# KirillKryukov/naf

Hardware: AMD Instinct MI355X
Metric: unnaf GB/s (uncompressed bases out) on 100 GB synthetic FASTA (higher is better)
Workload: dtype u8; 1 GPU; unnaf decode of a 100.0 GB synthetic-ACGT FASTA archive on one GPU (the size BASELINE.json's metric is quoted on; configs[1] at 10 GB rides along as cfg10_*), 100 records, 80-col lines; archive made in-run by the GPU ennaf; .naf 24739662224 B -> FASTA 99999995684 B, text + archive + decoded text resident in HBM; parallelism=one archive, one GPU, no data-path collective

## Files before the change

### naf_amd/csrc/ctx.h

```cpp
#pragma once
#include "common.h"
#include "../../include/naf_gpu.h"
#include <hip/hip_runtime.h>
#include <stdio.h>
#include <stdarg.h>
#include <string.h>
#include <vector>
#include <functional>
#include <string>

struct ArenaChunk { u8 *base; size_t cap, used; };

struct KTime { const char *name; hipEvent_t a, b; };

#define ZSPLIT_MAX 8
struct ZSplit { int parts; hipEvent_t ev[ZSPLIT_MAX]; u64 out_end[ZSPLIT_MAX]; int done; void *status; };
struct FlatStream { u64 q0, A; };
#define FLAT_DECODED (~0ull)
struct ZFlat { const u8 *src; const FlatStream *si; u64 nslots; const u8 *sym; void *status; bool ready;
               const u8 *tail; u64 tail_q; u32 tail_n;
               const u8 *cls; u32 n_decoded; u32 n_walk;
               struct naf_gpu_ctx *aux; hipEvent_t decoded_ev; void *later; };
struct CtxOpts { std::vector<std::pair<std::string, std::string>> kv; std::string trace; bool tracing = false; };
struct naf_gpu_ctx {
    int device = 0;
    CtxOpts *opts = nullptr;
    naf_gpu_ctx *root = nullptr;
    hipStream_t stream = nullptr;
    bool own_stream = false;
    std::vector<ArenaChunk> chunks;
    size_t high_water = 0;
    u8 *h_stage = nullptr;
    size_t h_stage_cap = 0;
    void *d_predef = nullptr;
    void *d_seqctab = nullptr;
    char err[512] = {0};
    bool timing = false;
    std::vector<KTime> ktimes;
    std::vector<hipEvent_t> ev_pool;
    size_t ev_used = 0;
    std::vector<std::string> agg_names; std::vector<float> agg_ms; std::vector<int> agg_n;
    float stream_ms[5] = { 0, 0, 0, 0, 0 };
    naf_gpu_ctx *side = nullptr;
    naf_gpu_ctx *side2 = nullptr;
    naf_gpu_ctx *side3 = nullptr;
    naf_gpu_ctx *side4 = nullptr;
    void *sides_thread = nullptr; int sides_rc = 0;
    hipEvent_t fork_ev = nullptr;
    struct ZSplit *zsplit = nullptr;
    hipEvent_t split_ev[ZSPLIT_MAX + 2] = {};
    struct ZFlat *zflat = nullptr;
    void *io_pool = nullptr;
    void *shard_state = nullptr;
    struct HostWorker *worker = nullptr;
};

void ctx_worker_start(naf_gpu_ctx *x, std::function<void()> job);
void ctx_worker_join(naf_gpu_ctx *x);
int  ctx_sides_ready(naf_gpu_ctx *c);

int  ctx_fail(naf_gpu_ctx *c, int code, const char *fmt, ...);
const char *ctx_opt(const naf_gpu_ctx *c, const char *name);
static inline bool ctx_opt_is(const naf_gpu_ctx *c, const char *name, char v) { const char *e = ctx_opt(c, name); return e && e[0] == v; }
bool ctx_tracing(const naf_gpu_ctx *c);
void ctx_trace(naf_gpu_ctx *c, const char *fmt, ...);
#define HIP_TRY(c, call) do { hipError_t e_ = (call); if (e_ != hipSuccess) return ctx_fail((c), NAF_GPU_EHIP, "%s: %s (%s:%d)", #call, hipGetErrorString(e_), __FILE__, __LINE__); } while (0)
static inline void ctx_take_error(naf_gpu_ctx *c, const char (&text)[512]) { memcpy(c->err, text, sizeof c->err); }
static inline void ctx_take_error(naf_gpu_ctx *c, const naf_gpu_ctx *from) { ctx_take_error(c, from->err); }
static inline hipError_t ctx_side_join(naf_gpu_ctx *x) { ctx_worker_join(x); return hipStreamSynchronize(x->stream); }
#define SIDE_SYNC_TRY(c, e, x) do { if ((e) != hipSuccess) return ctx_fail((c), NAF_GPU_EHIP, "%s: %s (%s:%d)", "hipStreamSynchronize(" #x "->stream)", hipGetErrorString(e), __FILE__, __LINE__); } while (0)
struct CtxJoinGuard { naf_gpu_ctx *x; ~CtxJoinGuard() { if (x) ctx_worker_join(x); } };

void  arena_reset(naf_gpu_ctx *c);
void *arena_alloc(naf_gpu_ctx *c, size_t bytes);
void  arena_settle(naf_gpu_ctx *c);
template <typename T> T *arena_new(naf_gpu_ctx *c, size_t n) { return (T *)arena_alloc(c, n * sizeof(T)); }
static inline std::vector<size_t> arena_mark(const naf_gpu_ctx *c) { std::vector<size_t> m; for (auto &ch : c->chunks) m.push_back(ch.used); return m; }
static inline void arena_release(naf_gpu_ctx *c, const std::vector<size_t> &m) { for (size_t k = 0; k < c->chunks.size(); k++) c->chunks[k].used = k < m.size() ? m[k] : 0; }

int ctx_readback(naf_gpu_ctx *c, void *h_dst, const void *d_src, size_t bytes);
int ctx_readback2(naf_gpu_ctx *c, void *h1, const void *d1, size_t n1, void *h2, const void *d2, size_t n2);
int ctx_readbackv(naf_gpu_ctx *c, int n, void *const *h, const void *const *d, const size_t *bytes);

void ktime_begin(naf_gpu_ctx *c, const char *name);
void ktime_end(naf_gpu_ctx *c);

#define LAUNCH(c, name, kern, grid, block, shmem, ...) do { \
    ktime_begin((c), name); \
    hipLaunchKernelGGL(kern, dim3(grid), dim3(block), (shmem), (c)->stream, __VA_ARGS__); \
    ktime_end((c)); } while (0)

static inline u32 cdiv(u64 a, u64 b) { return (u32)((a + b - 1) / b); }

int scan_exclusive_u64(naf_gpu_ctx *c, u64 *d_vals, size_t n, u64 *d_total);
int scan_inclusive_max_i32(naf_gpu_ctx *c, i32 *d_vals, size_t n);
int scan_inclusive_max_i64(naf_gpu_ctx *c, i64 *d_vals, size_t n);
int scan_exclusive_u64_multi(naf_gpu_ctx *c, u64 *const *arrs, int k, size_t n, u64 *const *totals);
int scan_inclusive_max_i64_multi(naf_gpu_ctx *c, i64 *const *arrs, int k, size_t n);

int zstd_decode(naf_gpu_ctx *c, const u8 *d_src, size_t src_len, int has_magic, u8 *d_dst, size_t dst_cap, size_t *out_len, const u8 *head = nullptr);
int zstd_init_tables(naf_gpu_ctx *c);
void ennaf_shard_state_free(naf_gpu_ctx *c);
void io_pool_free(naf_gpu_ctx *c);
struct EmitP;
int zstd_decode_fused_fasta(naf_gpu_ctx *c, const u8 *d_src, size_t src_len, int has_magic, size_t *out_len, const EmitP *P, u8 *text);
struct ZRange { u64 want_lo, want_hi, got_lo, got_hi; bool ranged; u8 *own_buf; };
int zstd_decode_range(naf_gpu_ctx *c, const u8 *d_src, size_t src_len, int has_magic, u8 *d_dst, size_t dst_cap, size_t *out_len, ZRange *rg, const u8 *head = nullptr);
int zstd_split_status(naf_gpu_ctx *c, const ZSplit *sp);
int zstd_flat_later(naf_gpu_ctx *c, ZFlat *zf);
void zstd_flat_drop(ZFlat *zf);
int zstd_small_batch(naf_gpu_ctx *c, int n, const u8 *const *src, const size_t *len, u8 *const *dst, const size_t *cap, bool *ok);
bool zstd_small_fits(size_t len, size_t cap);
int zstd_small_launch(naf_gpu_ctx *c, int n, const u8 *const *src, const size_t *len, u8 *const *dst, const size_t *cap, u32 **d_res_out);
enum { ZENC_PART = 16, ZENC_PART_FIRST = 32, ZENC_PART_LAST = 64, ZENC_PREFER_RAW = 128, ZENC_PREFER_FLAT = 256, ZENC_SHORT_CODES = 512, ZENC_FRAME_TREE = 1024, ZENC_LONG_LAST = 2048 };
int zenc_level_window(int level);
int zenc_repeat_probe(naf_gpu_ctx *c, const u8 *d_src, size_t n, u32 *share_1024);
static inline u32 zenc_probe_every(u64 n) { u32 e = 64; while (((n >> 20) / e) > 128) e <<= 1; return e; }
struct ZencPlace { u8 *(*fn)(void *ud, size_t frame_len); void *ud; };
struct ZencJob;
#define ZENC_LOC_BND 20
struct ZencLoc { const u8 *loc; const i32 *blk_bnd; const u32 *blk_t0; u64 tiles; };
int zstd_encode_begin(naf_gpu_ctx *c, const u8 *d_src, size_t n, int level, int with_magic, int lz, int block_log_hint, int window_log, ZencJob **job, const u8 *direct = nullptr, u32 nd = 0, const ZencLoc *dloc = nullptr);
int zstd_encode_finish(naf_gpu_ctx *c, ZencJob *job, u8 *d_dst, size_t cap, size_t *out_len, const ZencPlace *place);
void zstd_encode_drop(ZencJob *job);
int zstd_encode_size(naf_gpu_ctx *c, ZencJob *job, size_t *frame_len);
const u64 *zstd_encode_total_ptr(const ZencJob *job);
void zstd_encode_set_total(ZencJob *job, u64 total);
int zstd_encode(naf_gpu_ctx *c, const u8 *d_src, size_t n, int level, u8 *d_dst, size_t cap, size_t *out_len, int with_magic, int lz = 0, int block_log_hint = 0, int window_log = 0, const ZencPlace *place = nullptr);
```

### naf_amd/csrc/enc.hip

```cpp
#include "ctx.h"
#include <time.h>
#include "wgscan.h"
#include "enc_swar.h"

#define ET_BYTES 16
#define ET_TILE (256 * ET_BYTES)

struct OpMaxI64 { template <typename T> __device__ static T id() { return (T)(-1); } template <typename T> __device__ static T f(T a, T b) { return (i64)a > (i64)b ? a : b; } };
struct OpMaxU32 { template <typename T> __device__ static T id() { return (T)0; } template <typename T> __device__ static T f(T a, T b) { return a > b ? a : b; } };
struct OpMaxU64 { template <typename T> __device__ static T id() { return (T)0; } template <typename T> __device__ static T f(T a, T b) { return a > b ? a : b; } };

#define REG_ACGT 0x80000000u
#define REG_E(reg) (((reg) >> 24) & 0x7Fu)
struct EncP {
    const u8 *text; u64 n, p0;
    u32 expected[8];
    u8 replacement;
    u8 id_gt_unexpected;
    u8 strict, pad;
    u32 qlo, qhi;
    u32 plo, phi;
    u32 slo, shi;
    u32 nuc32[8];
    u32 *any_case;
// ... 704 lines not shown
    n = wg_reduce1<u64, OpAdd>(n, lds);
    if (threadIdx.x == 0 && n) atomicAdd(out, (unsigned long long)n);
}

struct EncOut {
    u8 *seq, *ids, *cmt;
    u8 *packed; u32 *casebits;
    u64 *rec_begin, *rec_end;
    u64 *unexpected;
    u64 *longest;
    u64 *lead;
    u64 *strict_first;
    const u64 *t_seq, *t_ids, *t_cmt, *t_rec; const u32 *t_tail; const i64 *tile_eol;
    const u32 *irr_list;
    const u32 *t_reg;
    const u8 *direct; u32 nd;
    u32 loc_mode;
    const u32 *sparse_list; const u32 *n_sparse;
};


__device__ __forceinline__ void flush_tile(u8 *dst, const u8 *stage, u32 n)
{
    u32 head = (u32)((8 - ((uintptr_t)dst & 7)) & 7); if (head > n) head = n;
    if (threadIdx.x < head) dst[threadIdx.x] = stage[threadIdx.x];
    u32 words = (n - head) >> 3;
    const u64 *s64 = (const u64 *)stage;
    for (u32 w = threadIdx.x; w < words; w += blockDim.x) {
        u32 off = head + 8 * w, sh = (off & 7) * 8;
        u64 a = s64[off >> 3], b = s64[(off >> 3) + 1];
        *(u64 *)(dst + off) = sh ? (a >> sh) | (b << (64 - sh)) : a;
    }
    u32 done = head + 8 * words;
    if (threadIdx.x < n - done) dst[done + threadIdx.x] = stage[done + threadIdx.x];
}

__device__ __forceinline__ u32 nuc4x4(u32 x, const u32 *t)
{
    const u32 sel = x & 0x07070707u;
    const u32 r0 = swar_perm(t[1], t[0], sel), r1 = swar_perm(t[3], t[2], sel), r2 = swar_perm(t[5], t[4], sel), r3 = swar_perm(t[7], t[6], sel);
    const u32 m3 = ((x >> 3) & 0x01010101u) * 0xFFu, m4 = ((x >> 4) & 0x01010101u) * 0xFFu, m6 = ((x >> 6) & 0x01010101u) * 0xFFu;
    const u32 lo = (r0 & ~m3) | (r1 & m3), hi = (r2 & ~m3) | (r3 & m3);
    const u32 tab = (lo & ~m4) | (hi & m4);
    return (tab & m6) | (m4 & 0x0F0F0F0Fu & ~m6);
}
__device__ __forceinline__ u32 nuc4x4_quick(u32 x) { return swar_perm(0x0F0F0F0Fu, 0x02010408u, (x >> 1) & 0x07070707u); }
__device__ __forceinline__ u32 pack_codes8(u32 c0, u32 c1)
{
    const u32 t0 = c0 | (c0 >> 4), t1 = c1 | (c1 >> 4);
    return swar_perm(t1, t0, 0x06040200u);
}
__device__ __forceinline__ bool all_quick16(const u32 w[4], u32 qlo, u32 qhi)
{
    const u32 L = 0x7F7F7F7Fu; u32 bad = 0;
#pragma unroll
    for (int i = 0; i < 4; i++) { u32 x = w[i], r = swar_perm(qhi, qlo, (x >> 1) & 0x07070707u), d = r ^ (x & 0xDFDFDFDFu); bad |= ((d & L) + L) | d; }
    return (bad & 0x80808080u) == 0;
}
template <bool KNOWN_QUICK>
__device__ __forceinline__ void flush_pack(const EncP &P, u8 *packed, u32 *casebits, u64 tbase, u32 n, const u8 *stage )
{
    if (!n) return;
    const u32 o = (u32)(tbase & 15), span = o + n, ng = (span + 15) >> 4;
    const u64 G0 = tbase >> 4;
    for (u32 j = threadIdx.x; j < ng; j += blockDim.x) {
        const uint4 v = *(const uint4 *)(stage + 16 * j);
        const u32 w[4] = { v.x, v.y, v.z, v.w };
        u32 cd[4];
        if (KNOWN_QUICK || all_quick16(w, P.qlo, P.qhi)) {
#pragma unroll
            for (int i = 0; i < 4; i++) cd[i] = nuc4x4_quick(w[i]);
        } else {
#pragma unroll
            for (int i = 0; i < 4; i++) cd[i] = nuc4x4(w[i], P.nuc32);
        }
        u64 pk = (u64)pack_codes8(cd[0], cd[1]) | ((u64)pack_codes8(cd[2], cd[3]) << 32);
        const u32 H = 0x80808080u;
        u32 cb = swar_movemask16((v.x | ((v.x << 1) & (v.x << 2))) & H, (v.y | ((v.y << 1) & (v.y << 2))) & H,
                                 (v.z | ((v.z << 1) & (v.z << 2))) & H, (v.w | ((v.w << 1) & (v.w << 2))) & H);
        const u32 a = j == 0 ? o : 0u, b = span - 16 * j < 16 ? span - 16 * j : 16u;
        if (a == 0 && b == 16) {
            *(u64 *)(packed + 8 * (G0 + j)) = pk;
            if (casebits) ((u16 *)casebits)[G0 + j] = (u16)cb;
        } else {
            const u64 nm = (b == 16 ? ~0ull : ((1ull << (4 * b)) - 1)) & ~((1ull << (4 * a)) - 1);
            cb &= ((1u << b) - 1) & ~((1u << a) - 1);
            atomicOr((unsigned long long *)(packed + 8 * (G0 + j)), (unsigned long long)(pk & nm));
            if (casebits) atomicOr(casebits + ((G0 + j) >> 1), cb << (16 * (u32)((G0 + j) & 1)));
        }
    }
}
#define DIRECT_PROBE_BLOCKS_LOG 5
__global__ __launch_bounds__(256) void k_direct_blocks(const u8 *text, const u64 *t_seq, const u32 *t_reg, u64 tiles, u32 nd, u32 prefer_flat, int probed, u8 *direct, const u32 *blk_t0 = nullptr, i32 *blk_bnd = nullptr)
{
    __shared__ u32 bins[4][64];
    const u32 wv = threadIdx.x >> 6, lane = threadIdx.x & 63;
    const u32 b = blockIdx.x * 4 + wv;
    bins[wv][lane] = 0;
    __syncthreads();
    bool ok = b < nd;
    if (ok && probed && (((b >> DIRECT_PROBE_BLOCKS_LOG) & (u32)(probed - 1)) == 0)) ok = false;
    u64 t0 = 0, t1 = 0;
    if (ok) {
        const u64 B0 = (u64)b << 16, B1 = B0 + 65536;
        u64 lo = 0, hi = tiles;
        if (blk_t0) { lo = blk_t0[b]; hi = lo + 1; }
        while (hi - lo > 1) {
            const u64 step = (hi - lo + 63) / 64;
            const u64 p = lo + (u64)lane * step;
            const bool le = p < hi && t_seq[p] <= B0;
            const u32 cnt = (u32)__popcll(__ballot(le));
            const u64 nlo = lo + (u64)(cnt - 1) * step, nhi = nlo + step < hi ? nlo + step : hi;
            lo = nlo; hi = nhi;
        }
        t0 = lo;
        const u64 t = t0 + lane;
        const u64 ts = t <= tiles ? t_seq[t] : ~0ull;
        const bool in = t < tiles && ts < B1;
        if (blk_bnd && lane < ZENC_LOC_BND) { const i64 rel = (i64)ts - (i64)B0; blk_bnd[(u64)b * ZENC_LOC_BND + lane] = t <= tiles && rel < (1 << 30) ? (i32)rel : (i32)(1 << 30); }
        const u64 bal = __ballot(in);
        const bool good = !in || ((t_reg[t] & REG_ACGT) != 0);
        ok = __ballot(!good) == 0 && bal != ~0ull;
        t1 = t0 + (u64)__popcll(bal) - 1;
    }
    if (ok) {
        const u64 x0 = t0 * ET_TILE, span = (t1 + 1 - t0) * ET_TILE;
        const u8 *at = text + x0 + (((u64)lane * span) >> 6 & ~63ull);
        uint4 v[4]; __builtin_memcpy(v, at, 64);
        const u32 w[16] = { v[0].x, v[0].y, v[0].z, v[0].w, v[1].x, v[1].y, v[1].z, v[1].w, v[2].x, v[2].y, v[2].z, v[2].w, v[3].x, v[3].y, v[3].z, v[3].w };
        u32 *mybins = &bins[wv][(lane & 3) * 16];
#pragma unroll
        for (int i = 0; i < 16; i++) {
#pragma unroll
            for (int h = 0; h < 2; h++) {
                const u32 pr = (w[i] >> (16 * h)) & 0xFFFFu, c0 = pr & 0xFF, c1 = pr >> 8;
                if ((c0 & 0x40) && (c1 & 0x40)) atomicAdd(&mybins[((c0 >> 1) & 3) | (((c1 >> 1) & 3) << 2)], 1u);
            }
        }
    }
    __syncthreads();
    if (ok) {
        const u32 c = lane < 16 ? bins[wv][lane] + bins[wv][16 + lane] + bins[wv][32 + lane] + bins[wv][48 + lane] : 0u;
        u32 ns = c;
#pragma unroll
        for (u32 d = 1; d < 16; d <<= 1) ns += __shfl_xor((int)ns, d, 64);
        float h = c ? (float)c * __log2f((float)ns / (float)c) : 0.0f;
#pragma unroll
        for (u32 d = 1; d < 16; d <<= 1) h += __shfl_xor(h, d, 64);
        ns = (u32)__shfl((int)ns, 0, 64); h = __shfl(h, 0, 64);
        ok = ns >= 1024 && h * (float)prefer_flat > 4.0f * (float)ns * (float)(prefer_flat - 1);
    }
    if (b < nd && lane == 0) direct[b] = ok ? 1 : 0;
}
__global__ __launch_bounds__(256) void k_direct_verdict(const u64 *t_seq, const u32 *t_reg, const u8 *t_hist, u64 tiles, u32 nd, u32 prefer_flat, int probed, const u32 *blk_t0, u8 *direct, i32 *blk_bnd)
{
    const u32 b = blockIdx.x * 256 + threadIdx.x;
    if (b >= nd) return;
    const u64 B0 = (u64)b << 16, B1 = B0 + 65536, t0 = blk_t0[b];
    bool ok = !(probed && (((b >> DIRECT_PROBE_BLOCKS_LOG) & (u32)(probed - 1)) == 0));
    u64 ts[ZENC_LOC_BND];
#pragma unroll
    for (u32 i = 0; i < ZENC_LOC_BND; i++) ts[i] = t0 + i <= tiles ? t_seq[t0 + i] : ~0ull;
#pragma unroll
    for (u32 i = 0; i < ZENC_LOC_BND; i++) { const i64 rel = (i64)ts[i] - (i64)B0; blk_bnd[(u64)b * ZENC_LOC_BND + i] = ts[i] != ~0ull && rel < (1 << 30) ? (i32)rel : (i32)(1 << 30); }
    u32 acc[8] = { 0, 0, 0, 0, 0, 0, 0, 0 };
    bool end = false;
#pragma unroll
    for (u32 i = 0; i < ZENC_LOC_BND - 1; i++) {
        if (!end && ok) {
            if (t0 + i >= tiles || ts[i] >= B1) end = true;
            else if (!(t_reg[t0 + i] & REG_ACGT)) ok = false;
            else {
                const uint4 h = *(const uint4 *)(t_hist + (t0 + i) * 16);
                acc[0] += h.x & 0x00FF00FFu; acc[1] += (h.x >> 8) & 0x00FF00FFu; acc[2] += h.y & 0x00FF00FFu; acc[3] += (h.y >> 8) & 0x00FF00FFu;
                acc[4] += h.z & 0x00FF00FFu; acc[5] += (h.z >> 8) & 0x00FF00FFu; acc[6] += h.w & 0x00FF00FFu; acc[7] += (h.w >> 8) & 0x00FF00FFu;
            }
        }
    }
    ok = ok && end;
    if (ok) {
        u32 ns = 0;
#pragma unroll
        for (int k = 0; k < 8; k++) ns += (acc[k] & 0xFFFFu) + (acc[k] >> 16);
        float h = 0.0f;
#pragma unroll
        for (int k = 0; k < 8; k++) {
            const u32 c0 = acc[k] & 0xFFFFu, c1 = acc[k] >> 16;
            if (c0) h += (float)c0 * __log2f((float)ns / (float)c0);
            if (c1) h += (float)c1 * __log2f((float)ns / (float)c1);
        }
        ok = ns >= 1024 && h * (float)prefer_flat > 4.0f * (float)ns * (float)(prefer_flat - 1);
    }
    direct[b] = ok ? 1 : 0;
}
__global__ __launch_bounds__(256) void k_case_gather(const u8 *direct, u32 nd, const u32 *blk_t0, const i32 *blk_bnd, const u8 *locc, const u8 *t_lower, u64 *casebits)
{
    __shared__ i32 s_bnd[ZENC_LOC_BND]; __shared__ u8 s_low[ZENC_LOC_BND];
    const u32 b = blockIdx.x;
    if (b >= nd || !direct[b]) return;
    const u64 t0 = blk_t0[b];
    if (threadIdx.x < ZENC_LOC_BND) { s_bnd[threadIdx.x] = blk_bnd[(u64)b * ZENC_LOC_BND + threadIdx.x]; s_low[threadIdx.x] = t_lower[t0 + threadIdx.x]; }
    __syncthreads();
    u32 a[4], c[4], e[4], sh[4], av[4], kk[4]; u64 nx[4];
#pragma unroll
    for (u32 r = 0; r < 4; r++) {
        const u32 W = r * 256u + threadIdx.x;
        const i32 r0 = (i32)(64u * W);
        u32 k = (u32)(r0 - s_bnd[0]) >> 12;
        if (s_bnd[k + 1] <= r0) k++;
        if (s_bnd[k + 1] <= r0) k++;
        const u32 i = (u32)(r0 - s_bnd[k]);
        av[r] = (u32)(s_bnd[k + 1] - r0); kk[r] = k; sh[r] = i & 31u;
        const u32 *p = (const u32 *)(locc + (t0 + k) * (LOC_TILE / 2)) + (i >> 5);
        a[r] = p[0]; c[r] = p[1]; e[r] = p[2];
        nx[r] = av[r] < 64u ? ld64(locc + (t0 + k + 1) * (LOC_TILE / 2)) : 0ull;
    }
#pragma unroll
    for (u32 r = 0; r < 4; r++) {
        u64 w = s_low[kk[r]] ? (u64)__builtin_amdgcn_alignbit(c[r], a[r], sh[r]) | ((u64)__builtin_amdgcn_alignbit(e[r], c[r], sh[r]) << 32) : 0ull;
        if (av[r] < 64u) {
            w &= (1ull << av[r]) - 1;
            if (s_low[kk[r] + 1]) w |= nx[r] << av[r];
        }
        casebits[((u64)b << 10) + r * 256u + threadIdx.x] = w;
    }
}
__global__ void k_irregular_list(const u32 *t_reg, const u64 *pre, u64 tiles, u32 *list, const u64 *t_seq = nullptr, u32 *blk_t0 = nullptr)
{
    const u64 t = (u64)blockIdx.x * blockDim.x + threadIdx.x;
    if (t >= tiles) return;
    if (!t_reg[t]) list[pre[t]] = (u32)t;
    if (blk_t0) {
        const u64 lo = t_seq[t], hi = t_seq[t + 1];
        for (u64 b = (lo + 65535) >> 16; (b << 16) < hi; b++) blk_t0[b] = (u32)t;
    }
}
__global__ void k_pack_edges_zero(const u64 *t_seq, u64 tiles, u64 T, u8 *packed, u32 *casebits, const u8 *direct, u32 nd, u32 loc_mode = 0)
{
    const u64 t = (u64)blockIdx.x * blockDim.x + threadIdx.x;
    if (t >= tiles) return;
    const u64 b0 = t_seq[t], b1 = t + 1 < tiles ? t_seq[t + 1] : T;
    if (b1 <= b0) return;
    const u64 g0 = b0 >> 4, g1 = (b1 - 1) >> 4;
    const bool d0 = direct && (g0 >> 12) < nd && direct[g0 >> 12], d1 = direct && (g1 >> 12) < nd && direct[g1 >> 12];
    if (loc_mode) {
        if (!d0) { *(u64 *)(packed + 8 * g0) = 0; if (casebits) ((u16 *)casebits)[g0] = 0; }
        if (!d1) { *(u64 *)(packed + 8 * g1) = 0; if (casebits) ((u16 *)casebits)[g1] = 0; }
        return;
    }
    if (d0) *((u32 *)(packed + ((g0 >> 12) << 15) + (((g0 >> 10) & 3) << 12)) + (1023u - (u32)(g0 & 1023u))) = 0; else *(u64 *)(packed + 8 * g0) = 0;
    if (d1) *((u32 *)(packed + ((g1 >> 12) << 15) + (((g1 >> 10) & 3) << 12)) + (1023u - (u32)(g1 & 1023u))) = 0; else *(u64 *)(packed + 8 * g1) = 0;
    if (casebits) { ((u16 *)casebits)[g0] = 0; ((u16 *)casebits)[g1] = 0; }
}

__device__ __forceinline__ u64 low_bytes(u32 n) { return n >= 8 ? ~0ull : ((1ull << (8 * n)) - 1); }
__device__ __forceinline__ void lds_store_n(u8 *p, u64 lo, u64 hi, u32 n)
{
    if (n >= 16) { __builtin_memcpy(p, &lo, 8); __builtin_memcpy(p + 8, &hi, 8); return; }
    if (n & 8) { __builtin_memcpy(p, &lo, 8); p += 8; lo = hi; }
    if (n & 4) { u32 v = (u32)lo; __builtin_memcpy(p, &v, 4); p += 4; lo >>= 32; }
    if (n & 2) { u16 v = (u16)lo; __builtin_memcpy(p, &v, 2); p += 2; lo >>= 16; }
    if (n & 1) *p = (u8)lo;
}

__device__ __forceinline__ u32 piece_run_compact(const Piece &pc, u32 a, u32 b, u32 sp, u64 &lo, u64 &hi)
{
    piece_from(pc, a, lo, hi);
    u32 d = (sp >> a) & ((1u << (b - a)) - 1);
    const u32 n = (b - a) - (u32)__popc(d);
    while (d) {
        u32 k = 31 - __clz((int)d); d &= ~(1u << k);
        u64 slo = (lo >> 8) | (hi << 56), shi = hi >> 8;
        if (k < 8) { u64 m = low_bytes(k); lo = (lo & m) | (slo & ~m); hi = shi; }
        else { u64 m = low_bytes(k - 8); hi = (hi & m) | (shi & ~m); }
    }
    return n;
}
__device__ __forceinline__ void global_store_n(u8 *p, u64 lo, u64 hi, u32 n)
{
    if (n >= 16) { st64(p, lo); st64(p + 8, hi); return; }
    if (n & 8) { st64(p, lo); p += 8; lo = hi; }
    if (n & 4) { st32(p, (u32)lo); p += 4; lo >>= 32; }
    if (n & 2) { p[0] = (u8)lo; p[1] = (u8)(lo >> 8); p += 2; lo >>= 16; }
    if (n & 1) p[0] = (u8)lo;
}

struct WriteSink {
    const EncOut &O; u64 bseq, bids, bcmt, rec; u64 line_b; u64 best; bool line_valid; u8 *stage; u64 tbase;
    __device__ WriteSink(const EncOut &o) : O(o) {}
    __device__ void emit(int s, u32 ch) { if (s == EV_SEQ) stage[bseq++ - tbase] = (u8)ch; else if (s == EV_IDS) O.ids[bids++] = (u8)ch; else O.cmt[bcmt++] = (u8)ch; }
    __device__ void header_start(u64) { if (rec > 0) O.rec_end[rec - 1] = bseq; else *O.lead = bseq; rec++; }
    __device__ void header_end(u64) { O.rec_begin[rec - 1] = bseq; line_b = bseq; }
    __device__ void line_end(u64) { u64 len = bseq - line_b; if (len > best) best = len; line_b = bseq; }
    __device__ void unexpected(int kind, u32 ch, u64 pos) { atomicAdd((unsigned long long *)&O.unexpected[kind * 257 + ch], 1ull); if (O.strict_first) atomicMin((unsigned long long *)O.strict_first, strict_key(pos, kind, ch)); }
    __device__ void ids_range(const Piece &pc, u32 a, u32 b) { u64 lo, hi; piece_from(pc, a, lo, hi); global_store_n(O.ids + bids, lo, hi, b - a); bids += b - a; }
    __device__ void cmt_range(const Piece &pc, u32 a, u32 b) { u64 lo, hi; piece_from(pc, a, lo, hi); global_store_n(O.cmt + bcmt, lo, hi, b - a); bcmt += b - a; }
    __device__ void seq_range(const Piece &pc, u32 a, u32 b, u32 sp) { u64 lo, hi; u32 n = piece_run_compact(pc, a, b, sp, lo, hi); lds_store_n(stage + (bseq - tbase), lo, hi, n); bseq += n; }
    __device__ void term(int st) { emit(st, 0); }
};

__device__ __forceinline__ u64 tile_line_base(const EncP &P, const EncOut &O, const i64 *tile_eol, u64 tile)
{
    const i64 le = tile ? tile_eol[tile - 1] : -1;
    if (le < 0 || (u64)(le + 1) <= P.p0) return 0;
    const u64 tp = (u64)le / ET_TILE;
    return O.t_seq[tp + 1] - (O.t_tail[tp] & 0x7FFFFFFFu);
}

#define REG_TPW 4
static bool enc_wave_wg(const naf_gpu_ctx *c) { const char *e = ctx_opt(c, "ENC_WAVE"); return !(e && e[0] == '0'); }
struct RegGroup { u32 ga, gb, e, nb; };
__device__ __forceinline__ void reg_group_geometry(u32 j, u32 o, u32 span, u32 p1, u32 W, float rW, RegGroup &g, u32 &x)
{
    g.ga = j == 0 ? o : 0u; g.gb = span - 16 * j < 16 ? span - 16 * j : 16u;
    const u32 b_lo = 16 * j + g.ga - o; g.nb = g.gb - g.ga;
    if (b_lo < p1) { x = b_lo; g.e = p1 - b_lo; }
    else {
        const u32 d = b_lo - p1;
        u32 k = (u32)((float)d * rW);
        if (k * W > d) k--; else if ((k + 1) * W <= d) k++;
        x = b_lo + 1 + k; g.e = W - (d - k * W);
    }
}
__device__ __forceinline__ void reg_group_pack(const RegGroup &g, u64 lo, u64 hi, u32 c16, u64 &pk, u32 &cb)
{
    if (g.e < g.nb) {
        const u64 slo = (lo >> 8) | (hi << 56), shi = (hi >> 8) | ((u64)c16 << 56);
        if (g.e < 8) { const u64 m = low_bytes(g.e); lo = (lo & m) | (slo & ~m); hi = shi; }
        else { const u64 m = low_bytes(g.e - 8); hi = (hi & m) | (shi & ~m); }
    }
    if (g.ga) {
        const u32 sh = 8 * g.ga;
        if (sh < 64) { hi = (hi << sh) | (lo >> (64 - sh)); lo <<= sh; } else { hi = lo << (sh - 64); lo = 0; }
    }
    const u32 gw[4] = { (u32)lo, (u32)(lo >> 32), (u32)hi, (u32)(hi >> 32) };
    u32 cd[4];
#pragma unroll
    for (int i = 0; i < 4; i++) cd[i] = nuc4x4_quick(gw[i]);
    pk = (u64)pack_codes8(cd[0], cd[1]) | ((u64)pack_codes8(cd[2], cd[3]) << 32);
    const u32 H = 0x80808080u;
    cb = swar_movemask16((gw[0] | ((gw[0] << 1) & (gw[0] << 2))) & H, (gw[1] | ((gw[1] << 1) & (gw[1] << 2))) & H,
                         (gw[2] | ((gw[2] << 1) & (gw[2] << 2))) & H, (gw[3] | ((gw[3] << 1) & (gw[3] << 2))) & H);
}
__device__ __forceinline__ u32 direct_code32(u64 pk)
{
    const u64 lg = ((pk >> 1) & 0x7777777777777777ull) - ((pk >> 3) & 0x1111111111111111ull);
// ... 1570 lines not shown
            if (ctx_tracing(c)) ctx_trace(c, "[fq reg] tiles %llu, not regular %llu\n", (unsigned long long)tiles, (unsigned long long)n_need);
        }
        if (n_need) LAUNCH(c, "ennaf_fq_count", k_encq_count, n_need, 256, 0, P, (const i64 *)t_eol, (const i64 *)t_sp, (const u64 *)t_ls, t_seq, t_ids, t_cmt, t_qual, piece_cnt, (const u32 *)need_list, 0);
        { u64 *const a4[4] = { t_seq, t_ids, t_cmt, t_qual }, *const t4[4] = { tot + 0, tot + 1, tot + 2, tot + 3 }; if ((rc = scan_exclusive_u64_multi(c, a4, 4, tiles, t4))) return rc; }
        u64 h[5]; u8 lastb = 0x0A;
        if (n) { if ((rc = ctx_readback2(c, h, tot, 40, &lastb, d_text + n - 1, 1))) return rc; }
        else if ((rc = ctx_readback(c, h, tot, 40))) return rc;
        T = h[0]; n_ids = h[1]; n_cmt = h[2]; n_qual = h[3];
        u64 nlines = h[4]; N = (nlines + 3) / 4;
        const bool noseq = nlines % 4 == 1 && !(lastb >= 0x0A && lastb <= 0x0D);
        if ((rc = alloc_bases(c, S))) return rc;
        s_ids = (u8 *)arena_alloc(c, n_ids + 16); s_cmt = (u8 *)arena_alloc(c, n_cmt + 16); s_qual = (u8 *)arena_alloc(c, n_qual + 16);
        rec_begin = arena_new<u64>(c, N + 1); rec_end = arena_new<u64>(c, N + 1);
        u64 *q_begin = arena_new<u64>(c, N + 1), *q_end = arena_new<u64>(c, N + 1);
        const size_t NU = 4 * 257 + 3;
        u64 *d_unexp = arena_new<u64>(c, NU);
        if (!s_ids || !s_cmt || !s_qual || !rec_begin || !rec_end || !q_begin || !q_end || !d_unexp) return NAF_GPU_ENOMEM;
        HIP_TRY(c, hipMemsetAsync(d_unexp, 0, NU * 8, c->stream));
        HIP_TRY(c, hipMemsetAsync(d_unexp + 4 * 257, 0xFF, 8, c->stream));
        HIP_TRY(c, hipMemsetAsync(d_unexp + 4 * 257 + 2, 0xFF, 8, c->stream));
        HIP_TRY(c, hipMemsetAsync(rec_begin, 0, (N + 1) * 8, c->stream)); HIP_TRY(c, hipMemsetAsync(rec_end, 0, (N + 1) * 8, c->stream));
        HIP_TRY(c, hipMemsetAsync(q_begin, 0, (N + 1) * 8, c->stream)); HIP_TRY(c, hipMemsetAsync(q_end, 0, (N + 1) * 8, c->stream));
        FqOut O; O.seq = bases; O.packed = S.packed; O.casebits = (u32 *)S.casebits; O.ids = s_ids; O.cmt = s_cmt; O.qual = s_qual; O.rec_begin = rec_begin; O.rec_end = rec_end; O.q_begin = q_begin; O.q_end = q_end;
        O.unexpected = d_unexp; O.first_error = d_unexp + 4 * 257; O.strict_first = o->strict ? d_unexp + 4 * 257 + 2 : nullptr;
        O.t_seq = t_seq; O.t_ids = t_ids; O.t_cmt = t_cmt; O.t_qual = t_qual; O.t_ls = t_ls; O.piece_cnt = piece_cnt; O.list = need_list; O.t_reg = t_reg; O.redo_list = redo_list; O.n_redo = n_redo;
        if (S.fourbit) {
            if (T) LAUNCH(c, "ennaf_pack_edges", k_pack_edges_zero, cdiv(tiles, 256), 256, 0, (const u64 *)t_seq, tiles, T, S.packed, (u32 *)S.casebits, (const u8 *)nullptr, 0u);
            O.reg_kind = fq_wave ? 2u : 1u;
            if (t_reg && fq_wave) LAUNCH(c, "ennaf_fq_scatter_wave", k_fq_scatter_wave<true>, tiles, 64, 0, P, (const i64 *)t_eol, (const i64 *)t_sp, O);
            if (t_reg && (!fq_wave || n_wide)) LAUNCH(c, "ennaf_fq_scatter_reg", k_encq_scatter_reg<true>, tiles, 256, 0, P, (const i64 *)t_eol, (const i64 *)t_sp, O);
            if (n_need) LAUNCH(c, "ennaf_fq_scatter", k_encq_scatter<true>, n_need, 256, 0, P, (const i64 *)t_eol, (const i64 *)t_sp, O);
            if (t_reg) {
                u32 nr = 0;
                if ((rc = ctx_readback(c, &nr, n_redo, 4))) return rc;
                if (ctx_tracing(c)) ctx_trace(c, "[fq reg] handed back %u\n", nr);
                if (nr) {
                    LAUNCH(c, "ennaf_fq_count", k_encq_count, nr, 256, 0, P, (const i64 *)t_eol, (const i64 *)t_sp, (const u64 *)t_ls, t_seq, t_ids, t_cmt, t_qual, piece_cnt, (const u32 *)redo_list, 1);
                    O.list = redo_list;
                    LAUNCH(c, "ennaf_fq_scatter", k_encq_scatter<true>, nr, 256, 0, P, (const i64 *)t_eol, (const i64 *)t_sp, O);
                }
            }
        } else LAUNCH(c, "ennaf_fq_scatter", k_encq_scatter<false>, tiles, 256, 0, P, (const i64 *)t_eol, (const i64 *)t_sp, O);
        if (nlines / 4) LAUNCH(c, "ennaf_fq_check", k_fq_check, cdiv(nlines / 4, 256), 256, 0, (const u64 *)rec_begin, (const u64 *)rec_end, (const u64 *)q_begin, (const u64 *)q_end, nlines / 4, O.first_error, d_unexp + 4 * 257 + 1);
        std::vector<u64> hu(NU);
        if ((rc = ctx_readback(c, hu.data(), d_unexp, NU * 8))) return rc;
        u64 fe = hu[4 * 257];
        u64 trunc_rec = nlines % 4 ? nlines / 4 : ~0ull;
        u64 best_rec = ~0ull; int best_stage = 99, best_kind = SE_NONE;
        if (fe != ~0ull && (fe >> 2) <= trunc_rec) {
            int kind = (int)(fe & 3);
            best_rec = fe >> 2; best_stage = kind == FQ_E_AT ? 0 : kind == FQ_E_PLUS ? 3 : 5;
            best_kind = kind == FQ_E_AT ? SE_AT : kind == FQ_E_PLUS ? SE_PLUS : SE_QLEN;
        }
        const u64 sk = hu[4 * 257 + 2];
        if (o->strict && sk != ~0ull) {
            const u64 pos = sk >> 11; const int skind = (int)((sk >> 9) & 3);
            unsigned long long *d_cnt = arena_new<unsigned long long>(c, 1); if (!d_cnt) return NAF_GPU_ENOMEM;
            HIP_TRY(c, hipMemsetAsync(d_cnt, 0, 8, c->stream));
            LAUNCH(c, "ennaf_count_starts", k_count_starts, (u32)((pos - p0) / 65536 + 1 < 1024 ? (pos - p0) / 65536 + 1 : 1024), 256, 0, d_text, p0, pos, 1, d_cnt);
            u64 cnt = 0; if ((rc = ctx_readback(c, &cnt, d_cnt, 8))) return rc;
            const u64 ord = cnt ? cnt - 1 : 0, srec = ord >> 2; const int sstage = skind <= 1 ? 1 : skind == 2 ? 2 : 4;
            if (srec <= trunc_rec && (srec < best_rec || (srec == best_rec && sstage < best_stage))) {
                S.err_kind = SE_STRICT; S.err_char = (u32)(sk & 0x1FF); S.err_rec = srec + 1; S.err_a = (u64)skind;
                return 0;
            }
        }
        if (best_kind != SE_NONE) {
            S.err_kind = best_kind; S.err_rec = best_rec;
            if (best_kind == SE_QLEN) {
                u64 v[4]; const u64 r = best_rec;
                if ((rc = ctx_readback2(c, &v[0], rec_begin + r, 8, &v[1], rec_end + r, 8)) || (rc = ctx_readback2(c, &v[2], q_begin + r, 8, &v[3], q_end + r, 8))) return rc;
                S.err_a = v[3] - v[2]; S.err_b = v[1] - v[0];
            }
            return 0;
        }
        if (noseq) { S.err_kind = SE_NOSEQ; return 0; }
        if (nlines % 4) { S.err_kind = SE_NOQUAL; return 0; }
        for (int k = 0; k < 4; k++) for (int i = 0; i < 257; i++) S.unexpected[k][i] = hu[k * 257 + i];
        longest = hu[4 * 257 + 1];
        S.all_ends = 1;
    }
    if (format == NAF_FMT_FASTA) {
        EncP P; memset(&P, 0, sizeof P);
        P.text = d_text; P.n = n; P.p0 = p0;
        set_expected(P, seq_type, true);
        u64 tiles = n / ET_TILE + 1;
        i64 *t_eol = arena_new<i64>(c, tiles + 1), *t_sp = arena_new<i64>(c, tiles + 1);
        u64 *t_seq = arena_new<u64>(c, tiles + 2), *t_ids = arena_new<u64>(c, tiles + 2), *t_cmt = arena_new<u64>(c, tiles + 2), *t_rec = arena_new<u64>(c, tiles + 2);
        u32 *t_tail = arena_new<u32>(c, tiles + 1), *t_reg = arena_new<u32>(c, tiles + 1), *irr_list = arena_new<u32>(c, tiles + 1);
        u64 *t_irr = arena_new<u64>(c, tiles + 2);
        u64 *tot = arena_new<u64>(c, 8);
        if (!t_eol || !t_sp || !t_seq || !t_ids || !t_cmt || !t_rec || !t_tail || !t_reg || !irr_list || !t_irr || !tot) return NAF_GPU_ENOMEM;
        HIP_TRY(c, hipMemsetAsync(tot + 6, 0, 8, c->stream));
        P.any_case = (u32 *)(tot + 6);
        const char *e_ed = ctx_opt(c, "DIRECT"), *e_epf = ctx_opt(c, "PREFER_FLAT"), *e_ebl = ctx_opt(c, "BLOCK_LOG"), *e_epr = ctx_opt(c, "PROBE"), *e_elz = ctx_opt(c, "LZ"), *e_op = ctx_opt(c, "ONEPASS");
        const u32 e_prefer_flat = e_epf && e_epf[0] ? (u32)atoi(e_epf) : 16u;
        const bool direct_opts = allow_direct && S.fourbit && o->level <= 1 && !o->long_log && !(e_ed && e_ed[0] == '0') && e_prefer_flat >= 2 && !(e_ebl && atoi(e_ebl) != 15) && !(e_epr && e_epr[0] == '1')
                                 && !(e_elz && !strcmp(e_elz, "all")) && n >= 16 * ET_TILE;
        const bool fused = direct_opts && enc_wave_wg(c) && !(e_op && e_op[0] == '0') && (n >> 17) >= ((e_ed && e_ed[0] == '2') || (e_op && e_op[0] == '2') ? 2u : 256u);
        u8 *loc = nullptr, *t_hist = nullptr, *locc = nullptr, *t_lower = nullptr; u32 *t_needf0 = nullptr; u64 *t_need0 = nullptr;
        if (fused) {
            loc = (u8 *)arena_alloc(c, (tiles + 1) * LOC_TILE + 64); t_hist = (u8 *)arena_alloc(c, (tiles + 1) * 16);
            locc = (u8 *)arena_alloc(c, (tiles + 1) * (LOC_TILE / 2) + 64); t_lower = (u8 *)arena_alloc(c, tiles + ZENC_LOC_BND + 2);
            if (!locc || !t_lower) return NAF_GPU_ENOMEM;
            HIP_TRY(c, hipMemsetAsync(t_lower, 0, tiles + ZENC_LOC_BND + 2, c->stream));
            t_needf0 = arena_new<u32>(c, tiles + 1); t_need0 = arena_new<u64>(c, tiles + 2);
            if (!loc || !t_hist || !t_needf0 || !t_need0) return NAF_GPU_ENOMEM;
            LAUNCH(c, "ennaf_split_once", (k_enc_fused<true, 1>), (u32)tiles, 64, 0, P, t_eol, t_sp, t_seq, t_ids, t_cmt, t_rec, t_tail, t_reg, t_irr, t_needf0, t_need0, tiles, loc, t_hist, locc, t_lower);
        } else
        LAUNCH(c, "ennaf_last", k_enc_last_fa, cdiv(tiles, 4 * LAST_TPW), 256, 0, P, t_eol, t_sp, tiles);
        { i64 *const a2[2] = { t_eol, t_sp }; if ((rc = scan_inclusive_max_i64_multi(c, a2, 2, tiles))) return rc; }
        if (S.fourbit && n >= 16 * ET_TILE) {
            u32 *t_needf = fused ? t_needf0 : arena_new<u32>(c, tiles + 1), *need_list = arena_new<u32>(c, tiles + 1); u64 *t_need = fused ? t_need0 : arena_new<u64>(c, tiles + 2);
            if (!t_needf || !need_list || !t_need) return NAF_GPU_ENOMEM;
            if (fused) LAUNCH(c, "ennaf_pure_check", k_pure_check, cdiv(tiles, 256), 256, 0, P, (const i64 *)t_eol, tiles, t_needf, t_need, t_reg, t_irr, (const u32 *)t_tail);
            else if (enc_wave_wg(c)) LAUNCH(c, "ennaf_count_pure", (k_enc_count_pure<1, 1>), (u32)tiles, 64, 0, P, (const i64 *)t_eol, t_seq, t_ids, t_cmt, t_rec, t_tail, t_reg, t_irr, t_needf, t_need, tiles);
            else LAUNCH(c, "ennaf_count_pure", (k_enc_count_pure<4, 1>), cdiv(tiles, 4), 256, 0, P, (const i64 *)t_eol, t_seq, t_ids, t_cmt, t_rec, t_tail, t_reg, t_irr, t_needf, t_need, tiles);
            if ((rc = scan_exclusive_u64(c, t_need, tiles, tot + 5))) return rc;
            LAUNCH(c, "ennaf_need_list", k_need_list, cdiv(tiles, 256), 256, 0, (const u32 *)t_needf, (const u64 *)t_need, tiles, need_list, (const u32 *)nullptr);
            u64 n_need = 0;
            if ((rc = ctx_readback(c, &n_need, tot + 5, 8))) return rc;
            if (ctx_tracing(c)) {
                std::vector<u32> hr(tiles); hipMemcpy(hr.data(), t_reg, tiles * 4, hipMemcpyDeviceToHost);
                u64 nz = 0; for (u64 i = 0; i < tiles; i++) nz += hr[i] != 0;
                ctx_trace(c, "[reg] tiles %llu need %llu regular %llu; reg[1..4] = %08x %08x %08x %08x\n", (unsigned long long)tiles, (unsigned long long)n_need, (unsigned long long)nz, hr[1], hr[2], hr[3], hr[4]);
            }
            if (n_need) LAUNCH(c, "ennaf_count", k_enc_count, n_need, 256, 0, P, (const i64 *)t_eol, (const i64 *)t_sp, t_seq, t_ids, t_cmt, t_rec, t_tail, t_reg, t_irr, (const u32 *)need_list);
        } else
        LAUNCH(c, "ennaf_count", k_enc_count, tiles, 256, 0, P, (const i64 *)t_eol, (const i64 *)t_sp, t_seq, t_ids, t_cmt, t_rec, t_tail, t_reg, t_irr, (const u32 *)nullptr);
        { u64 *const a5[5] = { t_seq, t_ids, t_cmt, t_rec, t_irr }, *const t5[5] = { tot + 0, tot + 1, tot + 2, tot + 3, tot + 4 }; if ((rc = scan_exclusive_u64_multi(c, a5, 5, tiles, t5))) return rc; }
        HIP_TRY(c, hipMemcpyAsync(t_seq + tiles, tot + 0, 8, hipMemcpyDeviceToDevice, c->stream));
        u32 *blk_t0 = fused ? arena_new<u32>(c, (size_t)(n >> 16) + 2) : nullptr;
        if (fused && !blk_t0) return NAF_GPU_ENOMEM;
        LAUNCH(c, "ennaf_irregular_list", k_irregular_list, cdiv(tiles, 256), 256, 0, (const u32 *)t_reg, (const u64 *)t_irr, tiles, irr_list, (const u64 *)t_seq, blk_t0);
        u64 h[7];
        if ((rc = ctx_readback(c, h, tot, 56))) return rc;
        T = h[0]; n_ids = h[1]; n_cmt = h[2]; N = h[3];
        S.no_case = (u32)h[6] == 0 && !(ctx_opt(c, "CASE_CENSUS") && ctx_opt(c, "CASE_CENSUS")[0] == '0');
        P.any_case = nullptr;
        const u64 n_irregular = h[4];
        if ((rc = alloc_bases(c, S, !(allow_direct && S.no_case)))) return rc;
        s_ids = (u8 *)arena_alloc(c, n_ids + 16); s_cmt = (u8 *)arena_alloc(c, n_cmt + 16);
        rec_begin = arena_new<u64>(c, N + 1); rec_end = arena_new<u64>(c, N + 1);
        const size_t NU = 3 * 257 + 3;
        u64 *d_unexp = arena_new<u64>(c, NU);
        if (!s_ids || !s_cmt || !rec_begin || !rec_end || !d_unexp) return NAF_GPU_ENOMEM;
        HIP_TRY(c, hipMemsetAsync(d_unexp, 0, NU * 8, c->stream));
        HIP_TRY(c, hipMemsetAsync(d_unexp + 3 * 257 + 1, 0xFF, 8, c->stream));
        HIP_TRY(c, hipMemsetAsync(rec_begin, 0, (N + 1) * 8, c->stream));
        EncOut O; O.seq = bases; O.packed = S.packed; O.casebits = (u32 *)S.casebits; O.ids = s_ids; O.cmt = s_cmt; O.rec_begin = rec_begin; O.rec_end = rec_end;
        O.unexpected = d_unexp; O.longest = d_unexp + 3 * 257; O.strict_first = o->strict ? d_unexp + 3 * 257 + 1 : nullptr; O.lead = d_unexp + 3 * 257 + 2;
        O.t_seq = t_seq; O.t_ids = t_ids; O.t_cmt = t_cmt; O.t_rec = t_rec; O.t_tail = t_tail; O.tile_eol = t_eol; O.t_reg = t_reg; O.irr_list = S.fourbit ? irr_list : nullptr;
        O.direct = nullptr; O.nd = 0; O.loc_mode = 0; O.sparse_list = nullptr; O.n_sparse = nullptr;
        if (S.fourbit) {
            const u64 n_seqb = (T + 1) / 2;
            const char *ed = e_ed, *epr = e_epr;
            const u32 prefer_flat = e_prefer_flat;
            const u64 nd64 = n_seqb >> 15;
            O.loc_mode = 0; O.sparse_list = nullptr; O.n_sparse = nullptr;
            if (direct_opts && nd64 >= ((ed && ed[0] == '2') || (fused && e_op && e_op[0] == '2') ? 2u : 256u) && nd64 < 0x7FFFFFFFull && !((T & 1) && (n_seqb & 32767) == 0)) {
                S.nd = (u32)nd64; S.direct = (u8 *)arena_alloc(c, S.nd); if (!S.direct) return NAF_GPU_ENOMEM;
                const bool use_loc = fused && !(e_op && e_op[0] == '3' && !S.no_case);
                i32 *blk_bnd = use_loc ? arena_new<i32>(c, (size_t)S.nd * ZENC_LOC_BND + 1) : nullptr;
                if (use_loc && !blk_bnd) return NAF_GPU_ENOMEM;
                if (use_loc) LAUNCH(c, "ennaf_direct_blocks", k_direct_verdict, cdiv(S.nd, 256), 256, 0, (const u64 *)t_seq, (const u32 *)t_reg, (const u8 *)t_hist, tiles, S.nd, prefer_flat, (epr && epr[0] == '0') ? 0 : (int)zenc_probe_every(n_seqb), (const u32 *)blk_t0, S.direct, blk_bnd);
                else LAUNCH(c, "ennaf_direct_blocks", k_direct_blocks, cdiv(S.nd, 4), 256, 0, d_text, (const u64 *)t_seq, (const u32 *)t_reg, tiles, S.nd, prefer_flat, (epr && epr[0] == '0') ? 0 : (int)zenc_probe_every(n_seqb), S.direct, (const u32 *)blk_t0, blk_bnd);
                O.direct = S.direct; O.nd = S.nd;
                if (use_loc) {
                    u32 *sparse_list = arena_new<u32>(c, tiles + 1), *n_sparse = arena_new<u32>(c, 2);
                    if (!sparse_list || !n_sparse) return NAF_GPU_ENOMEM;
                    HIP_TRY(c, hipMemsetAsync(n_sparse, 0, 8, c->stream));
                    O.loc_mode = 1; O.sparse_list = sparse_list; O.n_sparse = n_sparse;
                    LAUNCH(c, "ennaf_sparse_list", k_sparse_list, cdiv(tiles, 256), 256, 0, P, (const i64 *)t_eol, O, tiles, sparse_list, n_sparse);
                    S.dloc.loc = loc; S.dloc.blk_bnd = blk_bnd; S.dloc.blk_t0 = blk_t0; S.dloc.tiles = tiles;
                    if (S.casebits) LAUNCH(c, "ennaf_case_gather", k_case_gather, S.nd, 256, 0, (const u8 *)S.direct, S.nd, (const u32 *)blk_t0, (const i32 *)blk_bnd, (const u8 *)locc, (const u8 *)t_lower, S.casebits);
                }
                if (ctx_tracing(c)) {
                    std::vector<u8> hd(S.nd); hipStreamSynchronize(c->stream); hipMemcpy(hd.data(), S.direct, S.nd, hipMemcpyDeviceToHost);
                    u64 k = 0; for (u8 v : hd) k += v;
                    ctx_trace(c, "[direct] %llu of %u blocks\n", (unsigned long long)k, S.nd);
                }
            }
            S.sc4.P = P; S.sc4.O = O; S.sc4.t_eol = t_eol; S.sc4.t_sp = t_sp; S.sc4.t_seq = t_seq; S.sc4.tiles = tiles; S.sc4.T = T; S.sc4.n = n; S.sc4.n_irregular = n_irregular;
            if ((rc = ennaf_scatter4(c, S.sc4, S.packed, S.casebits))) return rc;
        } else LAUNCH(c, "ennaf_scatter", k_enc_scatter<false>, tiles, 256, 0, P, (const i64 *)t_eol, (const i64 *)t_sp, O);
        std::vector<u64> hu(NU);
        if ((rc = ctx_readback(c, hu.data(), d_unexp, NU * 8))) return rc;
        const u64 sk = hu[3 * 257 + 1];
        if (o->strict && sk != ~0ull) {
            const u64 pos = sk >> 11;
            unsigned long long *d_cnt = arena_new<unsigned long long>(c, 1); if (!d_cnt) return NAF_GPU_ENOMEM;
            HIP_TRY(c, hipMemsetAsync(d_cnt, 0, 8, c->stream));
            LAUNCH(c, "ennaf_count_starts", k_count_starts, (u32)((pos - p0) / 65536 + 1 < 1024 ? (pos - p0) / 65536 + 1 : 1024), 256, 0, d_text, p0, pos, 0, d_cnt);
            u64 cnt = 0; if ((rc = ctx_readback(c, &cnt, d_cnt, 8))) return rc;
            S.err_kind = SE_STRICT; S.err_char = (u32)(sk & 0x1FF); S.err_rec = cnt; S.err_a = (sk >> 9) & 3;
            return 0;
        }
        for (int k = 0; k < 3; k++) for (int i = 0; i < 257; i++) S.unexpected[k][i] = hu[k * 257 + i];
        longest = hu[3 * 257];
        S.lead = N ? hu[3 * 257 + 2] : T;
    }
    return 0;
}

struct EnnafCarry {
    u64 tail_extra;
    u32 skip_first;
    u32 tail_hi;
    int prev_masked;
    int skip_run0;
    u64 run_ext;
};
struct EnnafStreams { const u8 *ptr[6]; u64 len[6], orig[6]; int lz[6], block_log[6], window_log[6]; bool present[6];
                      u32 tail[6]; int flags[6];
                      const u8 *direct; u32 nd, tail_packed; const ZencLoc *dloc; };

static int ennaf_streams(naf_gpu_ctx *c, EnnafSplit &S, const EnnafCarry &K, EnnafStreams &X, int part = 3)
{
    if (part & 1) memset(&X, 0, sizeof X);
    int rc; const u64 T = S.T, N = S.N;
    u32 *s_len = nullptr; u8 *s_seq = nullptr, *s_mask = nullptr;
    u64 n_lenb = 0, n_seqb = 0, n_mask = 0; int mask_block_log = 15; u32 seq_tail = 0;
    if (S.format != 0) {
        if (N && (part & 2)) {
            u64 *lu = arena_new<u64>(c, N + 2); if (!lu) return NAF_GPU_ENOMEM;
            const u64 total = T + K.tail_extra;
            LAUNCH(c, "ennaf_len_count", k_len_unit_count, cdiv(N, 256), 256, 0, (const u64 *)S.rec_begin, (const u64 *)S.rec_end, N, total, lu, S.all_ends);
            if ((rc = scan_exclusive_u64(c, lu, N, lu + N + 1))) return rc;
            u64 nu = 0; if ((rc = ctx_readback(c, &nu, lu + N + 1, 8))) return rc;
            s_len = arena_new<u32>(c, nu + 1); if (!s_len) return NAF_GPU_ENOMEM;
            LAUNCH(c, "ennaf_len_write", k_len_unit_write, cdiv(N, 256), 256, 0, (const u64 *)S.rec_begin, (const u64 *)S.rec_end, N, total, (const u64 *)lu, s_len, S.all_ends);
            n_lenb = nu * 4;
        }
        const u64 mt = (T + MBB_TILE - 1) / MBB_TILE;
        u64 *tc = S.tc;
        if (!(part & 1)) { }
        else if (S.fourbit) {
            const u64 Tp = T > K.skip_first ? T - K.skip_first : 0;
            n_seqb = (Tp + 1) / 2;
            if (K.skip_first && n_seqb) {
                s_seq = (u8 *)arena_alloc(c, n_seqb + 16); if (!s_seq) return NAF_GPU_ENOMEM;
                LAUNCH(c, "ennaf_nibble_shift", k_nibble_shift, cdiv(cdiv(n_seqb, 8), 256), 256, 0, (const u8 *)S.packed, (T + 1) / 2, s_seq, n_seqb);
            } else s_seq = S.packed;
            if ((Tp & 1) && K.tail_hi) LAUNCH(c, "ennaf_tail_nibble", k_set_high_nibble, 1, 64, 0, s_seq + n_seqb - 1, K.tail_hi);
            if ((Tp & 1) && !K.tail_hi && n_seqb >= 2 && !S.store_qual) seq_tail = 1;
        } else {
            if (S.no_mask && T) LAUNCH(c, "ennaf_toupper", k_toupper, cdiv(T, 256), 256, 0, S.bases, T);
            s_seq = S.bases; n_seqb = T;
        }
        if (S.store_mask && T && (part & 2)) {
            u64 nb = 0; i64 *tile_last = S.census ? S.census_last : nullptr;
            const bool one_run = !S.census && S.no_case && !K.skip_run0 && !K.prev_masked;
            if (!one_run) {
            if (!S.census) {
                tc = arena_new<u64>(c, mt + 2); tile_last = arena_new<i64>(c, mt + 1); if (!tc || !tile_last) return NAF_GPU_ENOMEM;
                LAUNCH(c, "ennaf_mask_count", k_maskb_count, mt, 256, 0, (const u64 *)S.casebits, T, tc, 0, tile_last);
                if ((rc = scan_inclusive_max_i64(c, tile_last, mt))) return rc;
            }
            const int b0 = S.census ? ((S.first_base >= 96) != (K.prev_masked != 0)) : 0;
            if (b0) LAUNCH(c, "ennaf_mask_b0", k_add_u64, 1, 64, 0, tc, (u64)1);
            if ((rc = scan_exclusive_u64(c, tc, mt, tc + mt + 1))) return rc;
            if ((rc = ctx_readback(c, &nb, tc + mt + 1, 8))) return rc;
            }
            u64 nu = 0;
            if (nb == 0 && !K.skip_run0) {
                const u64 len = T + K.run_ext;
                nu = len / 255 + 1;
                s_mask = (u8 *)arena_alloc(c, nu + 16); if (!s_mask) return NAF_GPU_ENOMEM;
                HIP_TRY(c, hipMemsetAsync(s_mask, 0xFF, nu, c->stream));
                SmallBytes lb; memset(&lb, 0, sizeof lb); lb.b[0] = (u8)(len % 255); lb.n = 1;
                LAUNCH(c, "ennaf_mask_units", k_put_bytes, 1, 64, 0, s_mask + (nu - 1), lb);
            } else {
            u64 *any_long = arena_new<u64>(c, 1), *bnd = nullptr;
            if (!any_long) return NAF_GPU_ENOMEM;
            u64 longs = 1;
            const char *ms = ctx_opt(c, "MASK_SHORT");
            if (tile_last && nb >= (1u << 16) && nb * 64 >= T && !(ms && (ms[0] == '0' || ms[0] == '1'))) {
                nu = nb + 1 - (K.skip_run0 ? 1 : 0);
                s_mask = (u8 *)arena_alloc(c, nu + 16); if (!s_mask) return NAF_GPU_ENOMEM;
                HIP_TRY(c, hipMemsetAsync(any_long, 0, 8, c->stream));
                LAUNCH(c, "ennaf_mask_units", k_maskb_units_direct, mt, 256, 0, (const u64 *)S.casebits, T, (const u64 *)tc, (const i64 *)tile_last, nb, s_mask, K.run_ext, K.skip_run0, K.prev_masked, any_long);
                if ((rc = ctx_readback(c, &longs, any_long, 8))) return rc;
            }
            if (longs) {
            bnd = arena_new<u64>(c, nb + 1); if (!bnd) return NAF_GPU_ENOMEM;
            if (nb) LAUNCH(c, "ennaf_mask_bscatter", k_maskb_scatter, mt, 256, 0, (const u64 *)S.casebits, T, (const u64 *)tc, nb, bnd, K.prev_masked);
            { 
              if (!(ms && ms[0] == '0') && (nb + 1) * 255 > T + K.run_ext) {
                  nu = nb + 1 - (K.skip_run0 ? 1 : 0);
                  s_mask = (u8 *)arena_alloc(c, nu + 16); if (!s_mask) return NAF_GPU_ENOMEM;
                  HIP_TRY(c, hipMemsetAsync(any_long, 0, 8, c->stream));
                  LAUNCH(c, "ennaf_mask_units", k_mask_units_short, cdiv(nb + 1, 256), 256, 0, (const u64 *)bnd, nb, T, s_mask, K.run_ext, K.skip_run0, any_long);
                  if ((rc = ctx_readback(c, &longs, any_long, 8))) return rc;
              } }
            }
            if (longs) {
                u64 *ru = arena_new<u64>(c, nb + 3); if (!ru) return NAF_GPU_ENOMEM;
                LAUNCH(c, "ennaf_mask_runs", k_mask_run_units, cdiv(nb + 1, 256), 256, 0, (const u64 *)bnd, nb, T, ru, K.run_ext, K.skip_run0);
                if ((rc = scan_exclusive_u64(c, ru, nb + 1, ru + nb + 2))) return rc;
                if ((rc = ctx_readback(c, &nu, ru + nb + 2, 8))) return rc;
                s_mask = (u8 *)arena_alloc(c, nu + 16); if (!s_mask) return NAF_GPU_ENOMEM;
                if (nu) HIP_TRY(c, hipMemsetAsync(s_mask, 0xFF, nu, c->stream));
                LAUNCH(c, "ennaf_mask_units", k_mask_units_write, cdiv(nb + 1, 256), 256, 0, (const u64 *)bnd, nb, T, (const u64 *)ru, s_mask, K.run_ext, K.skip_run0);
            }
            }
            mask_block_log = 13;
            { const char *mb = ctx_opt(c, "MASK_BLOCK_LOG"); if (mb && atoi(mb) >= 10 && atoi(mb) <= 17) mask_block_log = atoi(mb); else if (nu >= (64ull << 20)) mask_block_log = 15; }
            n_mask = nu;
        }
    }
    if (part & 1) {
        X.ptr[0] = S.s_ids; X.len[0] = X.orig[0] = S.n_ids; X.lz[0] = 1; X.present[0] = true;
        X.ptr[1] = S.s_cmt; X.len[1] = X.orig[1] = S.n_cmt; X.lz[1] = 1; X.present[1] = true;
        { const char *sb_ = ctx_opt(c, "NAMES_BLOCK_LOG"); const int v = sb_ ? atoi(sb_) : 0; if (v >= 10 && v <= 15) X.block_log[1] = v; else if (S.n_cmt >= (16u << 20)) X.block_log[1] = 15; }
        X.tail_packed = seq_tail; X.direct = nullptr; X.nd = 0;
        X.dloc = nullptr;
        if (S.direct && (part & 1)) { X.direct = S.direct; X.nd = S.nd; seq_tail = (u32)(n_seqb & 32767); X.dloc = S.dloc.loc ? &S.dloc : nullptr; }
        X.ptr[4] = s_seq; X.len[4] = n_seqb; X.orig[4] = T; X.present[4] = true; X.tail[4] = seq_tail;
        if (S.store_qual) X.flags[4] |= ZENC_LONG_LAST;
        X.ptr[5] = S.s_qual; X.len[5] = X.orig[5] = S.n_qual; X.present[5] = S.store_qual;
    }
    if (part & 2) {
        X.ptr[2] = (const u8 *)s_len; X.len[2] = X.orig[2] = n_lenb; X.lz[2] = 1; X.present[2] = true;
        { const char *sb_ = ctx_opt(c, "SIDE_BLOCK_LOG"); const int v = sb_ ? atoi(sb_) : 0; if (v >= 10 && v <= 15) X.block_log[2] = v; else if (n_lenb >= (16u << 20)) X.block_log[2] = 15; }
        X.ptr[3] = s_mask; X.len[3] = X.orig[3] = n_mask; X.block_log[3] = mask_block_log; X.present[3] = S.store_mask; X.flags[3] = ZENC_PREFER_RAW;
    }
    return 0;
}

static void ennaf_probe_verdict(EnnafStreams &X, u32 share) { if (share >= 32) { X.window_log[4] = 19; X.lz[4] = 1; } }
static int ennaf_windows(naf_gpu_ctx *c, EnnafStreams &X, const naf_gpu_ennaf_opts *o, bool *defer = nullptr)
{
    const int wl = zenc_level_window(o->level);
    for (int i = 0; i < 6; i++) X.window_log[i] = wl;
    if (o->level <= 1) X.flags[4] |= ZENC_PREFER_FLAT;
    if (o->level <= 1) { X.flags[4] |= ZENC_SHORT_CODES; X.flags[5] |= ZENC_SHORT_CODES; }
    if (o->level <= 1) { X.flags[4] |= ZENC_FRAME_TREE; X.flags[5] |= ZENC_FRAME_TREE; }
    if (o->long_log) { X.window_log[4] = o->long_log < 10 ? 10 : o->long_log > 31 ? 31 : o->long_log; X.lz[4] = 1; }
    else if (!wl && X.present[4] && X.len[4]) {
// ... 620 lines not shown
```

### naf_amd/csrc/scan.hip

```cpp
#include "ctx.h"
#include "wgscan.h"

#define SCAN_ITEMS   8
#define SCAN_TILE    (SCAN_THREADS * SCAN_ITEMS)

template <typename T, typename Op>
__global__ __launch_bounds__(SCAN_THREADS) void k_scan_tile_reduce(const T *vals, size_t n, T *sums)
{
    __shared__ T lds[4];
    size_t base = (size_t)blockIdx.x * SCAN_TILE + threadIdx.x;
    T acc = Op::template id<T>();
#pragma unroll
    for (int i = 0; i < SCAN_ITEMS; i++) { size_t k = base + (size_t)i * SCAN_THREADS; if (k < n) acc = Op::template f<T>(acc, vals[k]); }
    T tot = wg_reduce1<T, Op>(acc, lds);
    if (threadIdx.x == 0) sums[blockIdx.x] = tot;
}

template <typename T, typename Op, bool EXCL>
__global__ __launch_bounds__(SCAN_THREADS) void k_scan_tile_apply(T *vals, size_t n, const T *tile_pre)
{
    __shared__ T lds[2][4];
    size_t base = (size_t)blockIdx.x * SCAN_TILE + threadIdx.x;
    T v[SCAN_ITEMS];
#pragma unroll
    for (int i = 0; i < SCAN_ITEMS; i++) { size_t k = base + (size_t)i * SCAN_THREADS; v[i] = k < n ? vals[k] : Op::template id<T>(); }
    T run = tile_pre ? tile_pre[blockIdx.x] : Op::template id<T>();
#pragma unroll
    for (int i = 0; i < SCAN_ITEMS; i++) {
        T pre, tot;
        T wi = wg_scan1<T, Op>(v[i], &pre, &tot, lds[i & 1]);
        T r = Op::template f<T>(run, Op::template f<T>(pre, EXCL ? wave_shift_up1<T, Op>(wi) : wi));
        size_t k = base + (size_t)i * SCAN_THREADS;
        if (k < n) vals[k] = r;
        run = Op::template f<T>(run, tot);
    }
}

#define SCAN_SMALL 4096
template <typename T, typename Op, bool EXCL>
__global__ __launch_bounds__(SCAN_THREADS) void k_scan_small(T *vals, size_t n, T *total)
{
    __shared__ T lds[4];
    const size_t per = (n + SCAN_THREADS - 1) / SCAN_THREADS, lo = threadIdx.x * per, hi = lo + per < n ? lo + per : n;
    T acc = Op::template id<T>();
    for (size_t k = lo; k < hi; k++) acc = Op::template f<T>(acc, vals[k]);
    T tot;
    const T incl = wg_scan_inclusive<T, Op>(acc, &tot, lds);
    T run = Op::template id<T>();
    {
        __shared__ T s_incl[SCAN_THREADS];
        s_incl[threadIdx.x] = incl;
        __syncthreads();
        if (threadIdx.x) run = s_incl[threadIdx.x - 1];
    }
    for (size_t k = lo; k < hi; k++) {
        const T v = vals[k];
        if (EXCL) { vals[k] = run; run = Op::template f<T>(run, v); }
        else { run = Op::template f<T>(run, v); vals[k] = run; }
    }
    if (total && threadIdx.x == 0) *total = tot;
}

template <typename T, typename Op, bool EXCL>
static int scan_rec(naf_gpu_ctx *c, T *vals, size_t n, T *d_total)
{
    if (n == 0) { if (d_total) HIP_TRY(c, hipMemsetAsync(d_total, 0, sizeof(T), c->stream)); return 0; }
    if (n <= SCAN_SMALL) { LAUNCH(c, "scan_small", (k_scan_small<T, Op, EXCL>), 1, SCAN_THREADS, 0, vals, n, d_total); return 0; }
    size_t ntiles = (n + SCAN_TILE - 1) / SCAN_TILE;
    T *sums = arena_new<T>(c, ntiles + 1);
    if (!sums) return ctx_fail(c, NAF_GPU_ENOMEM, "scan scratch");
    LAUNCH(c, "scan_reduce", (k_scan_tile_reduce<T, Op>), ntiles, SCAN_THREADS, 0, (const T *)vals, n, sums);
    int rc = scan_rec<T, Op, true>(c, sums, ntiles, d_total);
    if (rc) return rc;
    LAUNCH(c, "scan_apply", (k_scan_tile_apply<T, Op, EXCL>), ntiles, SCAN_THREADS, 0, vals, n, (const T *)sums);
    return 0;
}

int scan_exclusive_u64(naf_gpu_ctx *c, u64 *d_vals, size_t n, u64 *d_total)
{
    return scan_rec<u64, OpAdd, true>(c, d_vals, n, d_total);
}

int scan_inclusive_max_i32(naf_gpu_ctx *c, i32 *d_vals, size_t n)
{
    return scan_rec<i32, OpMax, false>(c, d_vals, n, (i32 *)nullptr);
}

int scan_inclusive_max_i64(naf_gpu_ctx *c, i64 *d_vals, size_t n)
{
    return scan_rec<i64, OpMax, false>(c, d_vals, n, (i64 *)nullptr);
}

#define SCAN_MULTI_MAX 8
template <typename T> struct ScanSet { T *v[SCAN_MULTI_MAX]; T *sums[SCAN_MULTI_MAX]; T *tot[SCAN_MULTI_MAX]; };
template <typename T, typename Op>
__global__ __launch_bounds__(SCAN_THREADS) void k_scan_tile_reduce_multi(ScanSet<T> S, size_t n)
{
    __shared__ T lds[4];
    const T *vals = S.v[blockIdx.y];
    size_t base = (size_t)blockIdx.x * SCAN_TILE + threadIdx.x;
    T acc = Op::template id<T>();
#pragma unroll
    for (int i = 0; i < SCAN_ITEMS; i++) { size_t k = base + (size_t)i * SCAN_THREADS; if (k < n) acc = Op::template f<T>(acc, vals[k]); }
    T tot = wg_reduce1<T, Op>(acc, lds);
    if (threadIdx.x == 0) S.sums[blockIdx.y][blockIdx.x] = tot;
}
template <typename T, typename Op>
__global__ __launch_bounds__(SCAN_THREADS) void k_scan_small_multi(ScanSet<T> S, size_t n)
{
    __shared__ T lds[4];
    __shared__ T s_incl[SCAN_THREADS];
    T *vals = S.sums[blockIdx.x];
    const size_t per = (n + SCAN_THREADS - 1) / SCAN_THREADS, lo = threadIdx.x * per, hi = lo + per < n ? lo + per : n;
    T acc = Op::template id<T>();
    for (size_t k = lo; k < hi; k++) acc = Op::template f<T>(acc, vals[k]);
    T tot;
    const T incl = wg_scan_inclusive<T, Op>(acc, &tot, lds);
    s_incl[threadIdx.x] = incl;
    __syncthreads();
    T run = threadIdx.x ? s_incl[threadIdx.x - 1] : Op::template id<T>();
    for (size_t k = lo; k < hi; k++) { const T v = vals[k]; vals[k] = run; run = Op::template f<T>(run, v); }
    if (S.tot[blockIdx.x] && threadIdx.x == 0) *S.tot[blockIdx.x] = tot;
}
template <typename T, typename Op, bool EXCL>
__global__ __launch_bounds__(SCAN_THREADS) void k_scan_tile_apply_multi(ScanSet<T> S, size_t n)
{
    __shared__ T lds[2][4];
    T *vals = S.v[blockIdx.y]; const T *tile_pre = S.sums[blockIdx.y];
    size_t base = (size_t)blockIdx.x * SCAN_TILE + threadIdx.x;
    T v[SCAN_ITEMS];
#pragma unroll
    for (int i = 0; i < SCAN_ITEMS; i++) { size_t k = base + (size_t)i * SCAN_THREADS; v[i] = k < n ? vals[k] : Op::template id<T>(); }
    T run = tile_pre[blockIdx.x];
#pragma unroll
    for (int i = 0; i < SCAN_ITEMS; i++) {
        T pre, tot;
        T wi = wg_scan1<T, Op>(v[i], &pre, &tot, lds[i & 1]);
        T r = Op::template f<T>(run, Op::template f<T>(pre, EXCL ? wave_shift_up1<T, Op>(wi) : wi));
        size_t k = base + (size_t)i * SCAN_THREADS;
        if (k < n) vals[k] = r;
        run = Op::template f<T>(run, tot);
    }
}
template <typename T, typename Op, bool EXCL>
static int scan_multi(naf_gpu_ctx *c, T *const *arrs, int k, size_t n, T *const *totals)
{
    const size_t ntiles = (n + SCAN_TILE - 1) / SCAN_TILE;
    if (k < 2 || k > SCAN_MULTI_MAX || n <= SCAN_SMALL || ntiles > SCAN_SMALL) {
        for (int i = 0; i < k; i++) { int rc = scan_rec<T, Op, EXCL>(c, arrs[i], n, totals ? totals[i] : (T *)nullptr); if (rc) return rc; }
        return 0;
    }
    ScanSet<T> S; memset(&S, 0, sizeof S);
    for (int i = 0; i < k; i++) {
        S.v[i] = arrs[i]; S.tot[i] = totals ? totals[i] : nullptr;
        S.sums[i] = arena_new<T>(c, ntiles + 1); if (!S.sums[i]) return ctx_fail(c, NAF_GPU_ENOMEM, "scan scratch");
    }
    LAUNCH(c, "scan_reduce", (k_scan_tile_reduce_multi<T, Op>), dim3((unsigned)ntiles, (unsigned)k), SCAN_THREADS, 0, S, n);
    LAUNCH(c, "scan_small", (k_scan_small_multi<T, Op>), (unsigned)k, SCAN_THREADS, 0, S, ntiles);
    LAUNCH(c, "scan_apply", (k_scan_tile_apply_multi<T, Op, EXCL>), dim3((unsigned)ntiles, (unsigned)k), SCAN_THREADS, 0, S, n);
    return 0;
}
int scan_exclusive_u64_multi(naf_gpu_ctx *c, u64 *const *arrs, int k, size_t n, u64 *const *totals) { return scan_multi<u64, OpAdd, true>(c, arrs, k, n, totals); }
int scan_inclusive_max_i64_multi(naf_gpu_ctx *c, i64 *const *arrs, int k, size_t n) { return scan_multi<i64, OpMax, false>(c, arrs, k, n, (i64 *const *)nullptr); }
```

### naf_amd/csrc/zstd_enc.hip

```cpp
#include "ctx.h"
#include <vector>
#include "zstd_enc_core.h"

#define ZENC_TREE_SLOT 192
#include "wgscan.h"
#include "enc_swar.h"
struct OpMaxU64 { template <typename T> __device__ static T id() { return (T)0; } template <typename T> __device__ static T f(T a, T b) { return a > b ? a : b; } };
#define ZENC_HCOPIES 4
#define ZENC_CACHE_ENTRIES 256
struct ZTreeEntry { u64 key; u32 tb, pad; u8 wt[256]; u8 tree[ZENC_TREE_SLOT]; };
struct ZTreeCache { ZTreeEntry e[ZENC_CACHE_ENTRIES]; };
static_assert(ZENC_CACHE_ENTRIES == 256, "one entry per thread of the plan kernel");
struct ZPlanWS {
    u32 tot[256]; u32 w[512]; u16 order[256]; u16 parent[512]; u8 depth[512];
    u8 len[256], wt[256], tree[ZENC_TREE_SLOT], tmp[160];
    FseWS fse; u32 log, tb;
};

struct ZFlat16 { u32 tb; u8 tree[ZENC_TREE_SLOT]; };
static const ZFlat16 &zenc_flat16()
{
    static const ZFlat16 T = [] {
        ZFlat16 t; memset(&t, 0, sizeof t);
        u8 wt[256]; memset(wt, 0, sizeof wt);
        for (u32 s = 0; s < 256; s++) if (__builtin_popcount(s & 15u) == 1 && __builtin_popcount(s >> 4) == 1) wt[s] = 1;
        static FseWS ws; u8 tmp[160];
        t.tb = huf_write_tree_w(t.tree, wt, 0x88u, tmp, ws, true);
        return t;
    }();
    return T;
}
__host__ __device__ static inline u64 zenc_block_lo(u64 n, u32 nblk, u32 b) { u64 q = n / nblk, r = n % nblk; return (u64)b * q + (b < r ? b : r); }

#define ZENC_FLATSCAN_WAVES 4
__global__ __launch_bounds__(64 * ZENC_FLATSCAN_WAVES) void k_zenc_flat_scan(const u8 *src, u64 n, u32 nblk, ZEncPlan *plan, u16 *codes, u8 *trees, u64 *csize, u8 *done, u32 min_gain, u32 prefer_flat, ZFlat16 f16, const u8 *planned, const u8 *direct)
{
    __shared__ u32 bins[ZENC_FLATSCAN_WAVES][64];
    const u32 wv = threadIdx.x >> 6, lane = threadIdx.x & 63;
    for (u32 bq = blockIdx.x; bq * ZENC_FLATSCAN_WAVES < nblk; bq += gridDim.x) {
    const u32 b = bq * ZENC_FLATSCAN_WAVES + wv;
    if (planned && bq * ZENC_FLATSCAN_WAVES + ZENC_FLATSCAN_WAVES <= nblk && *(const u32 *)(planned + bq * ZENC_FLATSCAN_WAVES) == 0x01010101u) continue;
    bins[wv][lane] = 0;
    __syncthreads();
    bool ok = b < nblk;
    u32 bn = 0; const u8 *s = src;
    if (ok) {
        const u64 lo = zenc_block_lo(n, nblk, b), hi = zenc_block_lo(n, nblk, b + 1);
        bn = (u32)(hi - lo); s = src + lo;
        ok = bn >= 2048;
    }
    const bool dir = ok && direct && direct[b];
    if (ok && !dir) {
        u64 bad = 0;
        const bool sampler = (lane & 3) == 0;
        u32 *mybins = &bins[wv][((lane >> 2) & 3) * 16];
        const u64 M5 = 0x5555555555555555ull, M3 = 0x3333333333333333ull, ONE = 0x1111111111111111ull;
#pragma unroll 8
        for (u32 i = lane * 16; i + 16 <= bn; i += 1024) {
            const u64 w0 = ld64(s + i), w1 = ld64(s + i + 8);
            u64 c0 = w0 - ((w0 >> 1) & M5), c1 = w1 - ((w1 >> 1) & M5);
            c0 = (c0 & M3) + ((c0 >> 2) & M3); c1 = (c1 & M3) + ((c1 >> 2) & M3);
            bad |= (c0 ^ ONE) | (c1 ^ ONE);
            if (sampler) {
                const u64 lg = ((w0 >> 1) & 0x7777777777777777ull) - ((w0 >> 3) & 0x1111111111111111ull);
                const u64 rk = ((lg >> 2) & 0x0C0C0C0C0C0C0C0Cull) | (lg & 0x0303030303030303ull);
#pragma unroll
                for (u32 k = 0; k < 8; k++) atomicAdd(&mybins[(u32)(rk >> (8 * k)) & 15u], 1u);
            }
        }
        if (lane == 0) for (u32 k = bn & ~15u; k < bn; k++) { const u32 v = s[k]; if (__popc(v & 15u) != 1 || __popc(v >> 4) != 1) bad = 1; }
        ok = __ballot(bad != 0) == 0;
    }
    __syncthreads();
    bool fast = dir;
    if (ok && !dir) {
        const u32 c = lane < 16 ? bins[wv][lane] + bins[wv][16 + lane] + bins[wv][32 + lane] + bins[wv][48 + lane] : 0u;
        u32 ns = c;
#pragma unroll
        for (u32 d = 1; d < 16; d <<= 1) ns += __shfl_xor((int)ns, d, 64);
        float h = c ? (float)c * __log2f((float)ns / (float)c) : 0.0f;
#pragma unroll
        for (u32 d = 1; d < 16; d <<= 1) h += __shfl_xor(h, d, 64);
        ns = (u32)__shfl((int)ns, 0, 64); h = __shfl(h, 0, 64);
        fast = ns > 0 && h * (float)prefer_flat > 4.0f * (float)ns * (float)(prefer_flat - 1);
    }
    if (fast) {
        const u32 perq = (bn + 3) / 4;
        ZEncPlan p; p.n = bn; p.kind = ZK_RAW; p.csize = 3 + bn; p.log = 0; p.tree_bytes = 0; p.lhdr = 0; p.pad = 0; p.frame = 0; p.pad2 = 0;
        for (u32 k = 0; k < 4; k++) p.ssz[k] = ((k < 3 ? perq : bn - 3 * perq) * 4 + 8) >> 3;
        zenc_plan_finish(p, bn, 4, f16.tb, min_gain);
        fast = p.kind == ZK_HUF;
        if (fast) {
            p.pad = dir ? 2 : 1;
            if (lane == 0) { plan[b] = p; if (csize) csize[b] = p.csize; }
            if (!dir)
            for (u32 sym = lane; sym < 256; sym += 64) {
                const bool is16 = __popc(sym & 15u) == 1 && __popc(sym >> 4) == 1;
                const u32 hn = sym >> 4, ln = sym & 15u, rank = 4 * ((hn >> 1) - (hn >> 3)) + ((ln >> 1) - (ln >> 3));
                codes[(u64)b * 256 + sym] = is16 ? (u16)(rank | (4u << 12)) : (u16)0;
            }
            for (u32 k = lane; k < p.tree_bytes; k += 64) trees[(u64)b * ZENC_TREE_SLOT + k] = f16.tree[k];
        }
    }
    if (b < nblk && lane == 0) done[b] = fast ? 1 : 0;
    }
}

__global__ void k_zenc_direct_plans(const u8 *direct, u32 nblk, ZEncPlan pd, ZFlat16 f16, ZEncPlan *plan, u8 *trees, u64 *csize, u8 *done)
{
    const u32 b = blockIdx.x * blockDim.x + threadIdx.x;
    if (b >= nblk || !direct[b]) return;
    plan[b] = pd; if (csize) csize[b] = pd.csize; done[b] = 1;
    for (u32 k = 0; k < pd.tree_bytes; k++) trees[(u64)b * ZENC_TREE_SLOT + k] = f16.tree[k];
}

__global__ __launch_bounds__(256) void k_zenc_plan(const u8 *src, u64 n, u32 nblk, ZEncPlan *plan, u16 *codes, u8 *trees, u64 *csize, const u32 *blk_len, u64 slot, ZTreeCache *cache, u32 sample_stride, u32 try_fse, u32 min_gain, u32 maxbits, u32 prefer_flat, const u8 *done, u8 *wt_defer,
                                                    u32 *fhist = nullptr, const ZEncPlan *fplan = nullptr, const u16 *fcodes = nullptr, const u32 *fratio = nullptr, u32 long_last = 0)
{
    __shared__ u32 hist[ZENC_HCOPIES * 1024];
    u32 b = sample_stride ? blockIdx.x * sample_stride : blockIdx.x;
    if (done && done[b]) return;
    u64 lo = zenc_block_lo(n, nblk, b), hi = zenc_block_lo(n, nblk, b + 1);
    if (blk_len) { lo = (u64)b * slot; hi = lo + blk_len[b]; }
    u32 bn = (u32)(hi - lo);
    for (u32 i = threadIdx.x; i < ZENC_HCOPIES * 1024; i += 256) hist[i] = 0;
    __syncthreads();
    u32 per = (bn + 3) / 4; if (!per) per = 1;
    const u8 *s = src + lo;
    const u32 cpy = threadIdx.x & (ZENC_HCOPIES - 1), rot = 8 * cpy;
    u32 *my = hist + cpy * 1024;
    const u64 rot8 = 0x0101010101010101ull * rot;
#ifdef ZPLAN_NOHIST
    if (threadIdx.x < 16) for (u32 q = 0; q < 4; q++) hist[q * 256 + threadIdx.x * 17] = bn / 64;
    if (0)
#endif
    for (u32 i0 = threadIdx.x * 8; i0 < bn; i0 += 8 * 2048) {
        u64 wv[8];
#pragma unroll
        for (u32 j = 0; j < 8; j++) { const u32 i = i0 + j * 2048; wv[j] = i + 8 <= bn ? ld64(s + i) : 0; }
#pragma unroll
        for (u32 j = 0; j < 8; j++) {
            const u32 i = i0 + j * 2048;
            if (i >= bn) break;
            if (i + 8 <= bn) {
                const u64 w = wv[j];
                const u32 q0 = (i >= per) + (i >= 2 * per) + (i >= 3 * per), q7 = (i + 7 >= per) + (i + 7 >= 2 * per) + (i + 7 >= 3 * per);
                if (q0 == q7) {
                    const u64 H = 0x8080808080808080ull;
                    const u64 wr = ((w & ~H) + rot8) ^ (w & H);
                    u32 *hq = my + q0 * 256;
                    const u32 lo = (u32)wr, hi = (u32)(wr >> 32);
#pragma unroll
                    for (u32 k = 0; k < 4; k++) { atomicAdd(&hq[(lo >> (8 * k)) & 0xFF], 1u); atomicAdd(&hq[(hi >> (8 * k)) & 0xFF], 1u); }
                } else {
#pragma unroll
                    for (u32 k = 0; k < 8; k++) { u32 pos = i + k, q = (pos >= per) + (pos >= 2 * per) + (pos >= 3 * per); atomicAdd(&my[q * 256 + (((u32)(w >> (8 * k)) + rot) & 0xFF)], 1u); }
                }
            } else {
                for (u32 k = 0; i + k < bn; k++) { u32 pos = i + k, q = (pos >= per) + (pos >= 2 * per) + (pos >= 3 * per); atomicAdd(&my[q * 256 + ((s[pos] + rot) & 0xFF)], 1u); }
            }
        }
    }
    __syncthreads();
    u32 red4[4];
    for (u32 q = 0; q < 4; q++) { u32 v = 0; for (u32 k = 0; k < ZENC_HCOPIES; k++) v += hist[k * 1024 + q * 256 + ((threadIdx.x + 8 * k) & 0xFF)]; red4[q] = v; }
    __syncthreads();
    for (u32 q = 0; q < 4; q++) hist[q * 256 + threadIdx.x] = red4[q];
    __syncthreads();
    static_assert(sizeof(ZPlanWS) <= (ZENC_HCOPIES - 1) * 4096, "plan workspace must fit the dead histogram copies");
    ZPlanWS &ws = *(ZPlanWS *)(hist + 1024);
    __shared__ u64 red[4];
    const u32 sym = threadIdx.x;
    u32 mine = hist[sym] + hist[256 + sym] + hist[512 + sym] + hist[768 + sym];
    ws.tot[sym] = mine; ws.len[sym] = 0;
    u32 distinct = (u32)__syncthreads_count(mine != 0);
    __shared__ u16 plist[256]; __shared__ u32 wave_n[4];
    u64 bal = __ballot(mine != 0);
    u32 myidx = (u32)__popcll(bal & ((1ull << (threadIdx.x & 63)) - 1));
    if ((threadIdx.x & 63) == 0) wave_n[threadIdx.x >> 6] = (u32)__popcll(bal);
    __syncthreads();
    for (u32 w = 0; w < (threadIdx.x >> 6); w++) myidx += wave_n[w];
    if (mine) plist[myidx] = (u16)sym;
    __syncthreads();
    ZEncPlan p; p.n = bn; p.kind = ZK_RAW; p.csize = 3 + bn; p.log = 0; p.tree_bytes = 0; p.lhdr = 0; p.pad = 0; p.frame = 0; p.pad2 = 0;
    p.ssz[0] = p.ssz[1] = p.ssz[2] = p.ssz[3] = 0;
    if (fhist && sample_stride && mine) atomicAdd(&fhist[sym], mine);
    if (fcodes && !sample_stride && fplan->kind == ZK_HUF && bn >= 64 && distinct >= 2) {
        __shared__ u64 fred[4];
        const u32 fl = (u32)fcodes[sym] >> 12;
        if (__syncthreads_and(mine == 0 || fl != 0)) {
            const float ent = mine ? (float)mine * __log2f((float)bn / (float)mine) : 0.f;
            u64 both; wg_scan_inclusive<u64, OpAdd>(((u64)(mine * fl) << 32) | (u64)(u32)(ent + 0.5f), &both, fred);
            const u64 fbits = both >> 32, ebits = both & 0xFFFFFFFFull;
            if (fbits * 1024 * 100 <= ebits * fratio[0] * 103 + 6400ull * 1024) {
                for (u32 k = 0; k < 4; k++) { u64 bits; wg_scan_inclusive<u64, OpAdd>((u64)hist[256 * k + sym] * fl, &bits, fred); p.ssz[k] = (u32)((bits + 1 + 7) / 8); }
                zenc_plan_finish(p, bn, fplan->log, 0, min_gain);
                if (p.kind == ZK_HUF && p.csize + fplan->tree_bytes <= 3 + bn) {
                    p.frame = 1; codes[(u64)b * 256 + sym] = fcodes[sym];
                    if (threadIdx.x == 0) { plan[b] = p; if (csize) csize[b] = p.csize; }
                    return;
                }
                if (p.kind != ZK_HUF) {
                    if (threadIdx.x == 0) { plan[b] = p; if (csize) csize[b] = p.csize; }
                    return;
                }
                p.kind = ZK_RAW; p.csize = 3 + bn; p.log = 0; p.tree_bytes = 0; p.lhdr = 0; p.pad = 0; p.frame = 0; p.pad2 = 0;
                p.ssz[0] = p.ssz[1] = p.ssz[2] = p.ssz[3] = 0;
            }
        }
    }
    bool huf = false, defer = false;
    if (bn && distinct == 1 && long_last && b + 1 == nblk && bn > 4) { }
    else if (bn && distinct == 1) { p.kind = ZK_RLE; p.csize = 4; }
    else if (min_gain && bn >= 64 && __syncthreads_or(mine + 16 >= bn)) { }
    else if (bn >= 64 && distinct >= 2) {
        __shared__ u32 s_flat_log, s_mm[4][3];
        {
            const u32 v = mine ? mine : 0xFFFFFFFFu;
            u32 m1 = v, mx = mine;
            for (int d = 32; d; d >>= 1) { const u32 o = (u32)__shfl_xor((int)m1, d, 64); m1 = o < m1 ? o : m1; const u32 q = (u32)__shfl_xor((int)mx, d, 64); mx = q > mx ? q : mx; }
            const bool twice = __popcll(__ballot(v == m1)) >= 2;
            u32 m2 = (v == m1) ? 0xFFFFFFFFu : v;
            for (int d = 32; d; d >>= 1) { const u32 o = (u32)__shfl_xor((int)m2, d, 64); m2 = o < m2 ? o : m2; }
            if (twice) m2 = m1;
            if ((threadIdx.x & 63) == 0) { s_mm[threadIdx.x >> 6][0] = m1; s_mm[threadIdx.x >> 6][1] = m2; s_mm[threadIdx.x >> 6][2] = mx; }
            __syncthreads();
            if (threadIdx.x == 0) {
                u32 a = 0xFFFFFFFFu, b = 0xFFFFFFFFu, top = 0;
                for (int w = 0; w < 4; w++) {
                    for (int k = 0; k < 2; k++) { const u32 x = s_mm[w][k]; if (x < a) { b = a; a = x; } else if (x < b) b = x; }
                    if (s_mm[w][2] > top) top = s_mm[w][2];
                }
                const bool pow2 = (distinct & (distinct - 1)) == 0;
                s_flat_log = (pow2 && distinct >= 2 && b != 0xFFFFFFFFu && (u64)a + b > top) ? (u32)(31 - __clz((int)distinct)) : 0u;
            }
            __syncthreads();
        }
        u32 flat_log = s_flat_log;
        if (flat_log) {
            if (mine) ws.len[sym] = (u8)flat_log;
            if (threadIdx.x == 0) ws.log = flat_log;
        }
        else if (mine) {
            u32 r = 0;
            for (u32 j = 0; j < distinct; j++) { u32 t = plist[j], c = ws.tot[t]; r += (c < mine || (c == mine && t < sym)); }
            ws.order[r] = (u16)sym;
        }
        __syncthreads();
        if (flat_log) { }
        else if (distinct <= 64) {
            if (threadIdx.x < 64) {
                const u32 lane = threadIdx.x, n = distinct;
                u32 wl = lane < n ? ws.tot[ws.order[lane]] : 0xFFFFFFFFu;
                u32 wi = 0xFFFFFFFFu, pl = 0, pi = 0;
                u32 leaf = 0, inode = 0, next = 0;
                for (u32 step = 0; step + 1 < n; step++) {
                    u32 sum = 0;
#pragma unroll
                    for (int pick = 0; pick < 2; pick++) {
                        const u32 lw = leaf < n ? (u32)__builtin_amdgcn_readlane((int)wl, (int)__builtin_amdgcn_readfirstlane((int)(leaf < 64 ? leaf : 63))) : 0xFFFFFFFFu;
                        const u32 iw = inode < next ? (u32)__builtin_amdgcn_readlane((int)wi, (int)__builtin_amdgcn_readfirstlane((int)inode)) : 0xFFFFFFFFu;
                        if (leaf < n && (inode >= next || lw <= iw)) { sum += lw; if (lane == leaf) pl = next; leaf++; }
                        else { sum += iw; if (lane == inode) pi = next; inode++; }
                    }
                    if (lane == next) wi = sum;
                    next++;
                }
                u32 di = 0;
                for (u32 k = n - 2; k-- > 0;) {
                    const u32 par = (u32)__builtin_amdgcn_readlane((int)pi, (int)__builtin_amdgcn_readfirstlane((int)k));
                    const u32 dpar = (u32)__builtin_amdgcn_readlane((int)di, (int)__builtin_amdgcn_readfirstlane((int)par));
                    if (lane == k) di = dpar + 1;
                }
// ... 99 lines not shown
    } else
    if (huf) {
        __shared__ u32 wcnt[16], wstart[16];
        if (sym < 16) wcnt[sym] = 0;
        __syncthreads();
        u32 l = ws.len[sym], wgt = l ? p.log + 1 - l : 0, rank = 0;
        if (l) { atomicAdd(&wcnt[wgt], 1u); for (u32 j = 0; j < myidx; j++) rank += ws.len[plist[j]] == l; }
        __syncthreads();
        if (sym == 0) { u32 pos = 0; for (u32 w = 1; w <= p.log; w++) { wstart[w] = pos; pos += wcnt[w] << (w - 1); } }
        __syncthreads();
        codes[(u64)b * 256 + sym] = l ? (u16)(((wstart[wgt] >> (wgt - 1)) + rank) | (l << 12)) : (u16)0;
        if (!defer && sym < p.tree_bytes) trees[(u64)b * ZENC_TREE_SLOT + sym] = ws.tree[sym];
    }
}

#define ZENC_FRAME_BLOCK 32768u
__global__ __launch_bounds__(256) void k_zenc_frame_block(const u32 *fhist, u8 *blockbuf, u32 *blen)
{
    __shared__ u64 red[4];
    const u32 sym = threadIdx.x, h = fhist[sym];
    u64 tot; wg_scan_inclusive<u64, OpAdd>((u64)h, &tot, red);
    u32 cnt = 0;
    if (h && tot) { cnt = (u32)(((u64)h * (ZENC_FRAME_BLOCK - 256)) / tot); if (!cnt) cnt = 1; }
    u64 all; const u64 inc = wg_scan_inclusive<u64, OpAdd>((u64)cnt, &all, red);
    u8 *o = blockbuf + (inc - cnt);
    for (u32 k = 0; k < cnt; k++) o[k] = (u8)sym;
    if (sym == 0) *blen = (u32)all;
}
__global__ __launch_bounds__(256) void k_zenc_frame_ratio(u32 *fhist, const u16 *fcodes)
{
    __shared__ u64 red[4];
    const u32 h = fhist[threadIdx.x], l = (u32)fcodes[threadIdx.x] >> 12;
    u64 tot = wg_reduce1<u64, OpAdd>((u64)h, red);
    __syncthreads();
    const float ent = (h && tot) ? (float)h * __log2f((float)tot / (float)h) : 0.f;
    const u64 both = wg_reduce1<u64, OpAdd>(((u64)h * l) << 0 | 0ull, red);
    __syncthreads();
    const u64 e = wg_reduce1<u64, OpAdd>((u64)(ent + 0.5f), red);
    if (threadIdx.x == 0) { u64 r = e ? both * 1024 / e : 1024; fhist[257] = (u32)(r < 1024 ? 1024 : r > 1229 ? 1229 : r); }
}
#define ZQ_MISSING 0x80u
__device__ __forceinline__ u32 zq_hash4(u32 x) { return (x ^ (x >> 4)) & 0x0F0F0F0Fu; }
__global__ __launch_bounds__(256) void k_zenc_frame_stats(const u32 *fhist, const u16 *fcodes, float *fstat)
{
    __shared__ u64 red[4];
    const u32 sym = threadIdx.x, h = fhist[sym], l = (u32)fcodes[sym] >> 12, x[3] = { l, l * l, (sym ^ (sym >> 4)) & 15u };
    const u64 N = wg_reduce1<u64, OpAdd>((u64)h, red);
    __syncthreads();
    for (u32 k = 0; k < 3; k++) {
        const u64 a = wg_reduce1<u64, OpAdd>((u64)h * x[k], red);
        __syncthreads();
        const u64 b2 = wg_reduce1<u64, OpAdd>((u64)h * x[k] * x[k], red);
        __syncthreads();
        if (sym == 0) {
            const double mu = N ? (double)a / (double)N : 0.0, var = N ? (double)b2 / (double)N - mu * mu : 0.0;
            fstat[2 * k] = (float)mu; fstat[2 * k + 1] = var > 0.0 ? (float)sqrt(var) : 0.f;
        }
    }
}
__global__ __launch_bounds__(256) void k_zenc_frame_quick(const u8 *src, u64 n, u32 nblk, ZEncPlan *plan, u16 *codes, u64 *csize, u8 *done,
                                                           const ZEncPlan *fplan, const u16 *fcodes, const float *fstat, u32 min_gain, u32 stride, u32 *tally, const u32 *gate)
{
    __shared__ __attribute__((aligned(16))) u8 tab[256 * 64];
    __shared__ u32 s_q[4][4], s_accept;
    const u32 b = stride ? blockIdx.x * stride : blockIdx.x, tid = threadIdx.x, lane = tid & 63, q = tid >> 6;
    if (!stride && gate && gate[0] * 2 < gate[1]) return;
    if (b >= nblk || done[b] || fplan->kind != ZK_HUF) return;
    const u64 lo = zenc_block_lo(n, nblk, b), hi = zenc_block_lo(n, nblk, b + 1);
    const u32 bn = (u32)(hi - lo);
    if (bn < 64) return;
    const u16 fc = fcodes[tid];
    {
        const u32 l = (u32)fc >> 12, v = (l ? l : ZQ_MISSING) * 0x01010101u;
        uint4 r; r.x = r.y = r.z = r.w = v;
        uint4 *row = (uint4 *)(tab + 64 * tid);
        row[0] = r; row[1] = r; row[2] = r; row[3] = r;
    }
    __syncthreads();
    const u32 per = (bn + 3) / 4;
    const u32 qlo = q * per < bn ? q * per : bn, qhi = q == 3 ? bn : (qlo + per < bn ? qlo + per : bn);
    const u8 *s = src + lo, *my = tab + lane;
    u32 s1 = 0, s2 = 0, orr = 0, sh = 0;
    for (u32 i0 = qlo + lane * 8; i0 < qhi; i0 += 8 * 512) {
        u64 wv[8];
#pragma unroll
        for (u32 j = 0; j < 8; j++) { const u32 i = i0 + j * 512; wv[j] = i + 8 <= qhi ? ld64(s + i) : 0; }
#pragma unroll
        for (u32 j = 0; j < 8; j++) {
            const u32 i = i0 + j * 512;
            if (i >= qhi) break;
            if (i + 8 <= qhi) {
                const u32 x0 = (u32)wv[j], x1 = (u32)(wv[j] >> 32);
#pragma unroll
                for (u32 k = 0; k < 4; k++) {
                    const u32 t0 = my[((x0 >> (8 * k)) & 0xFF) << 6], t1 = my[((x1 >> (8 * k)) & 0xFF) << 6];
                    s1 += t0 + t1; s2 += t0 * t0; s2 += t1 * t1; orr |= t0 | t1;
                }
                sh = swar_dot4(zq_hash4(x0), 0x01010101u, sh); sh = swar_dot4(zq_hash4(x1), 0x01010101u, sh);
            } else for (u32 k = 0; i + k < qhi; k++) {
                const u32 c = s[i + k], t = my[c << 6];
                s1 += t; s2 += t * t; orr |= t; sh += (c ^ (c >> 4)) & 15u;
            }
        }
    }
#pragma unroll
    for (int d = 32; d; d >>= 1) { s1 += (u32)__shfl_xor((int)s1, d, 64); s2 += (u32)__shfl_xor((int)s2, d, 64); sh += (u32)__shfl_xor((int)sh, d, 64); orr |= (u32)__shfl_xor((int)orr, d, 64); }
    if (lane == 0) { s_q[q][0] = s1; s_q[q][1] = s2; s_q[q][2] = sh; s_q[q][3] = orr; }
    __syncthreads();
    ZEncPlan p;
    if (tid == 0) {
        u32 accept = 0;
        const u32 S[3] = { s_q[0][0] + s_q[1][0] + s_q[2][0] + s_q[3][0], s_q[0][1] + s_q[1][1] + s_q[2][1] + s_q[3][1], s_q[0][2] + s_q[1][2] + s_q[2][2] + s_q[3][2] };
        bool like = !((s_q[0][3] | s_q[1][3] | s_q[2][3] | s_q[3][3]) & ZQ_MISSING);
        const float fb = (float)bn, rt = sqrtf(fb);
        for (u32 k = 0; k < 3 && like; k++) {
            const float want = fb * fstat[2 * k], d = fabsf((float)S[k] - want);
            if (d > 6.f * rt * fstat[2 * k + 1] + 0.005f * want) like = false;
        }
        if (like) {
            p.n = bn; p.kind = ZK_RAW; p.csize = 3 + bn; p.log = 0; p.tree_bytes = 0; p.lhdr = 0; p.pad = 0; p.frame = 0; p.pad2 = 0;
            for (u32 k = 0; k < 4; k++) p.ssz[k] = (s_q[k][0] + 1 + 7) / 8;
            zenc_plan_finish(p, bn, fplan->log, 0, min_gain);
            if (p.kind == ZK_HUF && p.csize + fplan->tree_bytes <= 3 + bn) { p.frame = 1; accept = 1; }
            else if (p.kind != ZK_HUF) accept = 2;
        }
        if (stride) { atomicAdd(&tally[1], 1u); if (accept) atomicAdd(&tally[0], 1u); accept = 0; }
        if (accept) { plan[b] = p; if (csize) csize[b] = p.csize; done[b] = 1; }
        s_accept = accept;
    }
    __syncthreads();
    if (s_accept == 1) codes[(u64)b * 256 + tid] = fc;
}

__global__ void k_zenc_frame_class(const ZEncPlan *plan, u32 nblk, i32 *v)
{
    const u32 b = blockIdx.x * blockDim.x + threadIdx.x;
    if (b < nblk) v[b] = plan[b].kind == ZK_HUF ? (i32)(2 * b + (plan[b].frame ? 0u : 1u)) : -1;
}
__global__ void k_zenc_frame_fix(ZEncPlan *plan, u32 nblk, const i32 *v, const ZEncPlan *fplan, const u8 *ftree, u8 *trees, u64 *csize)
{
    const u32 b = blockIdx.x * blockDim.x + threadIdx.x;
    if (b >= nblk || plan[b].kind != ZK_HUF || !plan[b].frame) return;
    const i32 prev = b ? v[b - 1] : -1;
    if (prev >= 0 && !(prev & 1)) return;
    ZEncPlan p = plan[b];
    const u32 tb = fplan->tree_bytes;
    zenc_plan_force(p, tb);
    for (u32 k = 0; k < tb; k++) trees[(u64)b * ZENC_TREE_SLOT + k] = ftree[k];
    plan[b] = p; if (csize) csize[b] = p.csize;
}

struct ZTreeLane { FseWS fse; u8 tmp[160]; u8 w[256]; u32 odd; };
static_assert((sizeof(ZTreeLane) / 4) % 2 == 1, "odd word stride: the lanes' workspaces start in different LDS banks");
__global__ __launch_bounds__(64) void k_zenc_tree(u32 nblk, ZEncPlan *plan, u8 *trees, u64 *csize, const u8 *wt_defer, u32 min_gain)
{
    __builtin_amdgcn_s_setprio(3);
    extern __shared__ __attribute__((aligned(16))) u8 tree_lds[];
    const u32 b = blockIdx.x * 64 + threadIdx.x;
    const bool pending = b < nblk && (plan[b].pad & 0x80u);
    if (!__ballot(pending)) return;
    if (!pending) return;
    ZTreeLane &L = ((ZTreeLane *)tree_lds)[threadIdx.x];
    ZEncPlan p = plan[b];
    const u32 lastw = p.tree_bytes, log = p.log, try_fse = p.lhdr, flat16 = p.pad & 1u;
    for (u32 k = 0; k < 256; k += 4) *(u32 *)(L.w + k) = *(const u32 *)(wt_defer + (u64)b * 256 + k);
    u8 *tree = trees + (u64)b * ZENC_TREE_SLOT;
    const u32 tb = huf_write_tree_w(tree, L.w, lastw, L.tmp, L.fse, try_fse != 0);
    p.kind = ZK_RAW; p.csize = 3 + p.n; p.log = 0; p.tree_bytes = 0; p.lhdr = 0; p.pad = 0; p.frame = 0; p.pad2 = 0;
    if (tb) { zenc_plan_finish(p, p.n, log, tb, min_gain); if (p.kind == ZK_HUF && flat16) p.pad = 1; }
    plan[b] = p;
    if (csize) csize[b] = p.csize;
}

#define LZ_MINMATCH 5
__device__ __forceinline__ u32 rdlane(u32 v, u32 l) { return (u32)__builtin_amdgcn_readlane((int)v, (int)l); }
#define LZ_HASH_LOG 12
#define LZ_BLOCK_MAX 32768
#define LZ_LANE_EXT 32
struct LzBufs {
    u8 *lits; u64 slot;
    u16 *ll, *ml, *of; u64 seq_slot;
    u32 *ofv;
    u32 *nseq, *nlit;
    u8 *seqbuf; u32 *seq_bytes;
};
__global__ __launch_bounds__(64) void k_lz_parse(const u8 *src, u64 n, u32 nblk, LzBufs B, u32 buf_bytes, u32 hash_log, const u8 *fallback = nullptr)
{
    if (fallback && !fallback[blockIdx.x]) return;

    __builtin_amdgcn_s_setprio(3);
    extern __shared__ __attribute__((aligned(16))) u8 lz_lds[];
    u8 *buf = lz_lds;
    u16 *tab = (u16 *)(lz_lds + buf_bytes);
    const u32 b = blockIdx.x, lane = threadIdx.x;
    const u64 lo = zenc_block_lo(n, nblk, b);
    const u32 bn = (u32)(zenc_block_lo(n, nblk, b + 1) - lo);
    for (u32 i = lane * 16; i < bn; i += 64 * 16) {
        if (i + 16 <= bn) { uint4 v; __builtin_memcpy(&v, src + lo + i, 16); *(uint4 *)(buf + i) = v; }
        else for (u32 k = i; k < bn; k++) buf[k] = src[lo + k];
    }
    for (u32 i = lane; i < (1u << hash_log); i += 64) tab[i] = 0;
    for (u32 i = bn + lane; i < bn + 320 && i < buf_bytes; i += 64) buf[i] = 0;
    __syncthreads();
    u8 *lits = B.lits + (u64)b * B.slot;
    u16 *sll = B.ll + (u64)b * B.seq_slot, *sml = B.ml + (u64)b * B.seq_slot, *sof = B.of + (u64)b * B.seq_slot;
    u32 cur = 0, anchor = 0, ns = 0, nl = 0;
    while (cur + LZ_MINMATCH <= bn) {
        u32 p = cur + lane; bool valid = p + LZ_MINMATCH <= bn;
        u32 v = 0, h = 0, c = 0, m = 0;
        if (valid) {
            __builtin_memcpy(&v, buf + p, 4);
            h = (v * 2654435761u) >> (32 - hash_log);
            c = tab[h];
            if (c) {
                u32 q = c - 1, cv; __builtin_memcpy(&cv, buf + q, 4);
                if (cv == v) {
                    m = 4;
                    for (;;) {
                        u64 x, y; __builtin_memcpy(&x, buf + q + m, 8); __builtin_memcpy(&y, buf + p + m, 8);
                        const u64 d = x ^ y;
                        if (d) { m += (u32)(__ffsll((long long)d) - 1) >> 3; break; }
                        m += 8;
                        if (p + m >= bn || m >= LZ_LANE_EXT) break;
                    }
                    if (p + m > bn) m = bn - p;
                }
            }
        }
        u64 win = __ballot(m >= LZ_MINMATCH);
        if (valid) tab[h] = (u16)(p + 1);
        u32 next = cur < anchor ? anchor : cur;
        while (next < cur + 64) {
            u64 w2 = win & ~((1ull << (next - cur)) - 1);
            if (!w2) break;
            u32 f = (u32)__ffsll((long long)w2) - 1;
            u32 pf = cur + f, mf = rdlane(m, f), cf = rdlane(c, f) - 1;
            while (mf >= LZ_LANE_EXT && pf + mf < bn) {
                u32 x, y; __builtin_memcpy(&x, buf + cf + mf + 4 * lane, 4); __builtin_memcpy(&y, buf + pf + mf + 4 * lane, 4);
                u32 d = x ^ y;
                u64 ne = __ballot(d != 0);
                if (!ne) { mf += 256; continue; }
                u32 l0 = (u32)__ffsll((long long)ne) - 1;
                u32 d0 = rdlane(d, l0);
                mf += 4 * l0 + (((u32)__ffs((int)d0) - 1) >> 3);
                break;
            }
            if (pf + mf > bn) mf = bn - pf;
            u32 ll = pf - anchor;
            for (u32 k = lane; k < ll; k += 64) lits[nl + k] = buf[anchor + k];
            if (lane == 0) { sll[ns] = (u16)ll; sml[ns] = (u16)mf; sof[ns] = (u16)(pf - cf); }
            nl += ll; ns++;
            anchor = next = pf + mf;
        }
        cur += 64;
        if (cur < anchor) cur = anchor;
    }
    for (u32 k = lane; k < bn - anchor; k += 64) lits[nl + k] = buf[anchor + k];
    nl += bn - anchor;
    if (lane == 0) { B.nseq[b] = ns; B.nlit[b] = nl; }
}

__device__ __forceinline__ u64 zero_bytes64(u64 w) { const u64 L = 0x7F7F7F7F7F7F7F7Full; return ~(((w & L) + L) | w) & ~L; }
__global__ __launch_bounds__(64) void k_lz_parse_lines(const u8 *src, u64 n, u32 nblk, LzBufs B, u32 buf_bytes, u8 *fallback, ZEncPlan *plan, u64 *csize, u8 *done, u32 line_div, u32 ml_slots)
{
    extern __shared__ __attribute__((aligned(16))) u8 lz_lds[];
    u8 *buf = lz_lds;
    u32 *s_ml = (u32 *)(lz_lds + buf_bytes);
    u16 *ends = (u16 *)(lz_lds + buf_bytes + 4 * (size_t)ml_slots);
    const u32 b = blockIdx.x, lane = threadIdx.x;
    const u64 lo = zenc_block_lo(n, nblk, b);
    const u32 bn = (u32)(zenc_block_lo(n, nblk, b + 1) - lo);
    const u32 max_lines = bn / line_div;
    for (u32 i = lane * 16; i < bn; i += 64 * 16) {
        if (i + 16 <= bn) { uint4 v; __builtin_memcpy(&v, src + lo + i, 16); *(uint4 *)(buf + i) = v; }
        else for (u32 k = i; k < bn; k++) buf[k] = src[lo + k];
    }
    for (u32 i = bn + lane; i < bn + 64 && i < buf_bytes; i += 64) buf[i] = 0xFF;
    __syncthreads();
    const u32 per = (((bn + 63) / 64) + 7) & ~7u, c0 = lane * per < bn ? lane * per : bn, c1 = c0 + per < bn ? c0 + per : bn;
    u32 cnt = 0;
    for (u32 i = c0; i < c1; i += 8) { u64 z = zero_bytes64(*(const u64 *)(buf + i)); if (i + 8 > c1) z &= (1ull << (8 * (c1 - i))) - 1; cnt += (u32)__popcll(z); }
    const u32 incl = wave_scan_inclusive<u32, OpAdd>(cnt), L = (u32)__shfl((int)incl, 63, 64);
    if (L < 2 || L > max_lines || L * 128 < bn) { if (lane == 0) fallback[b] = 1; return; }
    {
        u32 idx = incl - cnt;
        for (u32 i = c0; i < c1; i += 8) {
            u64 z = zero_bytes64(*(const u64 *)(buf + i)); if (i + 8 > c1) z &= (1ull << (8 * (c1 - i))) - 1;
            while (z) { ends[idx++] = (u16)(i + (((u32)__ffsll((long long)z) - 1) >> 3)); z &= z - 1; }
        }
    }
    __syncthreads();
    const u32 last_end = (u32)ends[L - 1] + 1, NL = L + (last_end < bn ? 1u : 0u);
    u16 *sll = B.ll + (u64)b * B.seq_slot, *sml = B.ml + (u64)b * B.seq_slot, *sof = B.of + (u64)b * B.seq_slot;
    u8 *lits = B.lits + (u64)b * B.slot;
    u32 seq_base = 0, matched_base = 0, anchor = 0;
    u32 c_open = 0xFFFFFFFFu, c_of = 0; bool c_tail = false;
    for (u32 r = 0; r < NL; r += 64) {
        const u32 i = r + lane;
        u32 s = 0, e = 0, of = 0, m1 = 0, k2 = 0, m2 = 0, len = 0;
        if (i < NL) {
            s = i ? (u32)ends[i - 1] + 1 : 0u; e = i < L ? (u32)ends[i] + 1 : bn; len = e - s;
            if (i >= 1) {
                of = s - (i >= 2 ? (u32)ends[i - 2] + 1 : 0u);
                const u32 lim = len < 256 ? len : 256u;
                u32 k = 0;
                for (; k < lim; k += 8) { u64 x, y; __builtin_memcpy(&x, buf + s + k, 8); __builtin_memcpy(&y, buf + s + k - of, 8); const u64 d = x ^ y; if (d) { k += ((u32)__ffsll((long long)d) - 1) >> 3; break; } }
                m1 = k < lim ? k : lim;
                if (m1 < len) {
                    const u32 plen = of;
                    u32 maxs = len - m1; if (maxs > plen) maxs = plen; if (maxs > 256) maxs = 256;
                    u32 ks = 0; bool stop = false;
// ... 210 lines not shown
                            }
                            if (m2 > m) { m = m2; c = (i64)q - (i64)lo; }
                        }
                    }
                }
            }
            if (p + m > bn) m = bn - p;
        }
        const u64 win = __ballot(m >= LZ_MINMATCH);
        if (valid) tab[h] = (u16)(p + 1);
        u32 next = cur < anchor ? anchor : cur;
        while (next < cur + 64 && ns + 8 < max_seq) {
            const u64 w2 = win & ~((1ull << (next - cur)) - 1);
            if (!w2) break;
            const u32 f = (u32)__ffsll((long long)w2) - 1;
            u32 pf = cur + f, mf = rdlane(m, f);
            const u32 clo = rdlane((u32)(u64)c, f), chi = rdlane((u32)((u64)c >> 32), f);
            i64 cf = (i64)(((u64)chi << 32) | clo);
            if (mf >= LZ_LANE_EXT) mf = lzx_wave_match(buf, gblk, n - lo, bn, pf, cf, mf);
            const u32 back = lzx_wave_back(buf, gblk, lo, pf, cf, anchor);
            pf -= back; cf -= back; mf += back;
            const u32 d = (u32)((i64)pf - cf);
            emit(pf, mf, d);
            for (;;) {
                bool again = false;
                for (u32 skip = 1; skip <= 3 && !again; skip++) {
                    const u32 t = anchor + skip;
                    if (t + 4 > bn) break;
                    const u32 mr = lzx_wave_match(buf, gblk, n - lo, bn, t, (i64)t - (i64)d, 0);
                    if (mr >= 4 && ns + 8 < max_seq) { emit(t, mr, d); again = true; }
                }
                if (!again) break;
            }
            next = anchor;
        }
        cur += 64;
        if (cur < anchor) cur = anchor;
    }
    for (u32 k = lane; k < bn - anchor; k += 64) lits[nl + k] = buf[anchor + k];
    nl += bn - anchor;
    if (lane == 0) { B.nseq[b] = ns; B.nlit[b] = nl; }
}

__global__ __launch_bounds__(64) void k_lzx_seqenc(u32 nblk, LzBufs B, const SeqCTabs *tabs)
{
    __builtin_amdgcn_s_setprio(3);
    __shared__ SeqCTabs T; __shared__ SeqWS ws;
    for (u32 i = threadIdx.x; i < sizeof(SeqCTabs) / 4; i += 64) ((u32 *)&T)[i] = ((const u32 *)tabs)[i];
    __syncthreads();
    const u32 b = blockIdx.x;
    if (threadIdx.x) return;
    const u32 ns = B.nseq[b]; u32 bytes = 1;
    u8 *out = B.seqbuf + (u64)b * B.slot;
    if (ns == 0) out[0] = 0;
    else bytes = zenc_write_sequences_x(out, (u32)B.slot, B.ll + (u64)b * B.seq_slot, B.ml + (u64)b * B.seq_slot, B.ofv + (u64)b * B.seq_slot, ns, T, ws);
    B.seq_bytes[b] = bytes;
}

__host__ __device__ static inline u32 lz_lit_section_bytes(const ZEncPlan &p)
{
    if (p.kind == ZK_HUF) return p.csize - 3 - 1;
    u32 hdr = p.n < 32 ? 1 : (p.n < 4096 ? 2 : 3);
    return p.kind == ZK_RLE ? hdr + 1 : hdr + p.n;
}
__global__ void k_lz_choose(u32 nblk, const ZEncPlan *plan0, const ZEncPlan *plan1, const u32 *nseq, const u32 *seq_bytes, u8 *mode, u64 *csize)
{
    u32 b = blockIdx.x * blockDim.x + threadIdx.x;
    if (b >= nblk) return;
    u32 s0 = plan0[b].csize, s1 = 3 + lz_lit_section_bytes(plan1[b]) + seq_bytes[b];
    bool lz = nseq[b] > 0 && seq_bytes[b] > 0 && s1 < s0;
    mode[b] = lz ? 1 : 0; csize[b] = lz ? s1 : s0;
}

#define ZENC_BLOCKS_PER_WG 16
#define ZENC_OROW 80
template <int GROUP>
__device__ __forceinline__ void huf_encode_stream_staged(u8 *out, const u8 *src, u32 n, const u16 *codes, u8 *orow)
{
    u64 acc = 0; u32 nb = 0;
    u32 lo = (u32)((uintptr_t)out & 63), fill = lo;
    u8 *seg = out - lo;
    auto flush_group = [&]() {
        __builtin_memcpy(orow + fill, &acc, 8);
        fill += nb >> 3; acc >>= (nb & ~7u); nb &= 7;
        if (fill >= 64) {
            if (lo == 0) { const uint4 *r = (const uint4 *)orow; uint4 *g = (uint4 *)seg; g[0] = r[0]; g[1] = r[1]; g[2] = r[2]; g[3] = r[3]; }
            else { for (u32 k = lo; k < 64; k++) seg[k] = orow[k]; lo = 0; }
            u64 t0, t1; __builtin_memcpy(&t0, orow + 64, 8); __builtin_memcpy(&t1, orow + 72, 8);
            __builtin_memcpy(orow, &t0, 8); __builtin_memcpy(orow + 8, &t1, 8);
            seg += 64; fill -= 64;
        }
    };
    auto put_e = [&](u32 e) { acc |= (u64)(e & 0xFFF) << nb; nb += e >> 12; };
    u32 i = n;
    while (i >= 64) {
        i -= 64;
        uint4 q[4]; __builtin_memcpy(q, src + i, 64);
#pragma unroll
        for (int wdx = 7; wdx >= 0; wdx--) {
            const uint4 &qq = q[wdx >> 1];
            u64 w = (wdx & 1) ? ((u64)qq.z | ((u64)qq.w << 32)) : ((u64)qq.x | ((u64)qq.y << 32));
            u32 e[8];
#pragma unroll
            for (int k = 0; k < 8; k++) e[k] = codes[(u32)(w >> (8 * k)) & 0xFF];
            if (GROUP == 8) {
#pragma unroll
                for (int k = 7; k >= 0; k--) put_e(e[k]);
                flush_group();
            } else {
                put_e(e[7]); put_e(e[6]); put_e(e[5]); put_e(e[4]); flush_group();
                put_e(e[3]); put_e(e[2]); put_e(e[1]); put_e(e[0]); flush_group();
            }
        }
    }
    while (i > 0) {
        u32 g = i < 4 ? i : 4;
        for (u32 k = 0; k < g; k++) put_e(codes[src[--i]]);
        flush_group();
    }
    acc |= 1ull << nb; nb++;
    __builtin_memcpy(orow + fill, &acc, 8); fill += (nb + 7) >> 3;
    for (u32 k = lo; k < fill; k++) seg[k] = orow[k];
}

__device__ __forceinline__ void zenc_flat4_stream(u8 *out, const u8 *s, u32 n, const u16 *codes, u32 lane)
{
    const u32 B = (4 * n + 8) >> 3;
    for (u32 t0 = lane * 16; t0 < B; t0 += 64 * 16) {
        const u32 q0 = 2 * t0;
        if (q0 + 32 <= n) {
            uint4 v0, v1; __builtin_memcpy(&v0, s + (n - 32 - q0), 16); __builtin_memcpy(&v1, s + (n - 16 - q0), 16);
            const u32 wd[8] = { v0.x, v0.y, v0.z, v0.w, v1.x, v1.y, v1.z, v1.w };
            u64 lo = 0, hi = 0;
#pragma unroll
            for (int i = 0; i < 16; i++) {
                const u32 a = (wd[(31 - i) >> 2] >> (8 * ((31 - i) & 3))) & 0xFFu, b2 = (wd[(15 - i) >> 2] >> (8 * ((15 - i) & 3))) & 0xFFu;
                lo |= (u64)(codes[a] & 0xFu) << (4 * i);
                hi |= (u64)(codes[b2] & 0xFu) << (4 * i);
            }
            const uint4 o4 = make_uint4((u32)lo, (u32)(lo >> 32), (u32)hi, (u32)(hi >> 32));
            __builtin_memcpy(out + t0, &o4, 16);
        } else {
            const u32 t1 = t0 + 16 < B ? t0 + 16 : B;
            for (u32 t = t0; t < t1; t++) {
                const u32 qa = 2 * t, qb = qa + 1;
                const u32 na = qa < n ? (codes[s[n - 1 - qa]] & 0xFu) : (qa == n ? 1u : 0u), nbv = qb < n ? (codes[s[n - 1 - qb]] & 0xFu) : (qb == n ? 1u : 0u);
                out[t] = (u8)(na | (nbv << 4));
            }
        }
    }
}

struct ZWriteLz { const u8 *mode; const ZEncPlan *plan1; const u16 *codes1; const u8 *trees1; LzBufs B; u32 not_last; u32 wave_general; u32 frame_split; };
struct ZencJob { const u8 *src; size_t n; u32 nblk, frame_wlog; ZEncPlan *plan; u16 *codes; u8 *trees; u64 *offs; u64 hdr; int with_magic, empty; ZWriteLz L; bool direct; u32 block_bytes; ZencLoc dloc; u64 known_total; int have_total, own_sync; };
template <bool FRAME>
__global__ __launch_bounds__(64) void k_zenc_write(const u8 *src, u64 n, u32 nblk, const ZEncPlan *plan, const u16 *codes_g, const u8 *trees,
                                                    const u64 *offs, u8 *dst, u64 frame_hdr, ZWriteLz L)
{
    __shared__ __attribute__((aligned(16))) u16 codes[FRAME ? 1 : ZENC_BLOCKS_PER_WG][256];
    __shared__ __attribute__((aligned(16))) u8 orows[64 * ZENC_OROW];
    int lane = threadIdx.x;
    u32 b0 = blockIdx.x * ZENC_BLOCKS_PER_WG;
    auto framed = [&](u32 bb) { return plan[bb].kind == ZK_HUF && plan[bb].frame != 0 && !plan[bb].pad; };
    if (FRAME) {
        const u32 bb = b0 + (u32)lane;
        const u64 fr = __ballot(lane < ZENC_BLOCKS_PER_WG && bb < nblk && framed(bb));
        if (!fr) return;
        const uint4 *g = (const uint4 *)(codes_g + (u64)(b0 + (u32)__ffsll((long long)fr) - 1) * 256);
        if (lane < 32) ((uint4 *)codes[0])[lane] = g[lane];
    } else {
    {
        const u32 bb = b0 + (u32)lane;
        const bool other = lane < ZENC_BLOCKS_PER_WG && bb < nblk && !(plan[bb].kind == ZK_HUF && (plan[bb].pad == 2 || L.wave_general) && !(L.mode && L.mode[bb])) && !(L.frame_split && framed(bb));
        if (__ballot(other) == 0) return;
    }
    for (u32 jj = 0; jj < ZENC_BLOCKS_PER_WG; jj++) {
        u32 bb = b0 + jj;
        if (bb >= nblk) break;
        const bool lzb = L.mode && L.mode[bb];
        if ((lzb ? L.plan1[bb].kind : plan[bb].kind) != ZK_HUF || (!lzb && plan[bb].pad == 2)) continue;
        if (L.frame_split && framed(bb)) continue;
        const uint4 *g = (const uint4 *)((lzb ? L.codes1 : codes_g) + (u64)bb * 256);
        if (lane < 32) ((uint4 *)codes[FRAME ? 0 : jj])[lane] = g[lane];
    }
    }
    __syncthreads();
    if (!FRAME) for (u32 jj = 0; jj < ZENC_BLOCKS_PER_WG; jj++) {
        const u32 bb = b0 + jj;
        if (bb >= nblk) break;
        if (L.mode && L.mode[bb]) continue;
        const ZEncPlan p = plan[bb];
        if (p.kind != ZK_HUF || !p.pad || L.wave_general) continue;
        if (p.pad == 2) continue;
        u8 *out = dst + frame_hdr + offs[bb];
        const u64 lo = zenc_block_lo(n, nblk, bb);
        if (lane == 0) { zenc_write_block_prefix(out, p, trees + (u64)bb * ZENC_TREE_SLOT, bb + 1 == nblk && !L.not_last, src[lo]); out[p.csize - 1] = 0; }
        const u32 per = (p.n + 3) / 4;
        u32 o = 3 + p.lhdr + p.tree_bytes + 6;
        for (u32 q = 0; q < 4; q++) { zenc_flat4_stream(out + o, src + lo + (u64)q * per, q < 3 ? per : p.n - 3 * per, codes[FRAME ? 0 : jj], (u32)lane); o += p.ssz[q]; }
    }
    u32 j = lane >> 2, k = lane & 3, b = b0 + j;
    if (b < nblk && (FRAME ? framed(b) : !(L.frame_split && framed(b)))) {
        const bool lzb = L.mode && L.mode[b];
        const u16 *ct = codes[FRAME ? 0 : j];
        u8 *out = dst + frame_hdr + offs[b];
        if (!lzb && plan[b].kind == ZK_HUF && (plan[b].pad || L.wave_general)) { }
        else if (!lzb) {
            const ZEncPlan p = plan[b];
            u64 lo = zenc_block_lo(n, nblk, b);
            if (k == 0) zenc_write_block_prefix(out, p, trees + (u64)b * ZENC_TREE_SLOT, b + 1 == nblk && !L.not_last, p.n ? src[lo] : 0);
            if (p.kind == ZK_HUF) {
                u32 per = (p.n + 3) / 4;
                u32 cnt = k < 3 ? per : p.n - 3 * per;
                const u32 o = 3 + p.lhdr + p.tree_bytes + 6 + (k > 0 ? p.ssz[0] : 0u) + (k > 1 ? p.ssz[1] : 0u) + (k > 2 ? p.ssz[2] : 0u);
                if (p.log <= 7) huf_encode_stream_staged<8>(out + o, src + lo + (u64)k * per, cnt, ct, orows + lane * ZENC_OROW);
                else huf_encode_stream_staged<4>(out + o, src + lo + (u64)k * per, cnt, ct, orows + lane * ZENC_OROW);
                if (k == 3) out[p.csize - 1] = 0;
            }
        } else {
            const ZEncPlan p = L.plan1[b];
            const u8 *lits = L.B.lits + (u64)b * L.B.slot;
            const u32 lsec = lz_lit_section_bytes(p), sbytes = L.B.seq_bytes[b];
            if (k == 0) zenc_write_block_header(out, 2, lsec + sbytes, b + 1 == nblk && !L.not_last);
            if (p.kind == ZK_HUF) {
                if (k == 0) zenc_write_huf_lit_prefix(out + 3, p, L.trees1 + (u64)b * ZENC_TREE_SLOT);
                u32 per = (p.n + 3) / 4;
                u32 cnt = k < 3 ? per : p.n - 3 * per;
                const u32 o = 3 + p.lhdr + p.tree_bytes + 6 + (k > 0 ? p.ssz[0] : 0u) + (k > 1 ? p.ssz[1] : 0u) + (k > 2 ? p.ssz[2] : 0u);
                if (p.log <= 7) huf_encode_stream_staged<8>(out + o, lits + (u64)k * per, cnt, ct, orows + lane * ZENC_OROW);
                else huf_encode_stream_staged<4>(out + o, lits + (u64)k * per, cnt, ct, orows + lane * ZENC_OROW);
            } else if (k == 0) {
                u32 h = zenc_lit_header_raw(out + 3, p.kind == ZK_RLE ? 1u : 0u, p.n);
                if (p.kind == ZK_RLE) out[3 + h] = lits[0];
                else for (u32 i = 0; i < p.n; i++) out[3 + h + i] = lits[i];
            }
            const u8 *sq = L.B.seqbuf + (u64)b * L.B.slot;
            for (u32 i = k; i < sbytes; i += 4) out[3 + lsec + i] = sq[i];
        }
    }
    if (!FRAME) for (u32 jj = 0; jj < ZENC_BLOCKS_PER_WG; jj++) {
        u32 bb = b0 + jj;
        if (bb >= nblk) break;
        if ((L.mode && L.mode[bb]) || plan[bb].kind != ZK_RAW) continue;
        u64 lo = zenc_block_lo(n, nblk, bb);
        u32 bn = plan[bb].n;
        const u8 *s = src + lo; u8 *o = dst + frame_hdr + offs[bb] + 3;
        for (u32 i = lane * 8; i + 8 <= bn; i += 64 * 8) st64(o + i, ld64(s + i));
        for (u32 i = (bn & ~7u) + lane; i < bn; i += 64) o[i] = s[i];
    }
}

#define ZWW_OBUF 12288u
#define ZWW_BLOCKS 64u
__global__ __launch_bounds__(256) void k_zenc_write_wave(const u8 *src, u64 n, u32 nblk, const ZEncPlan *plan, const u16 *codes_g, const u8 *trees,
                                                         const u64 *offs, u8 *dst, u64 frame_hdr, u32 not_last)
{
    extern __shared__ __attribute__((aligned(16))) u8 zww[];
    __shared__ u64 s_general;
    if (threadIdx.x < 64) {
        const u64 bb = (u64)blockIdx.x + (u64)threadIdx.x * gridDim.x;
        const u64 m = __ballot(bb < nblk && plan[bb].kind == ZK_HUF && plan[bb].pad != 2);
        if (threadIdx.x == 0) s_general = m;
    }
    __syncthreads();
    for (u64 todo = s_general; todo; todo &= todo - 1) {
    const u32 b = blockIdx.x + (u32)(__ffsll((long long)todo) - 1) * gridDim.x;
    const ZEncPlan p = plan[b];
    __syncthreads();
    u16 *codes = (u16 *)zww;
    if (threadIdx.x < 32) ((uint4 *)codes)[threadIdx.x] = ((const uint4 *)(codes_g + (u64)b * 256))[threadIdx.x];
    const u32 k = threadIdx.x >> 6, lane = threadIdx.x & 63;
    u32 *ob = (u32 *)(zww + 512 + k * ZWW_OBUF);
    const u32 per = (p.n + 3) / 4, cnt = k < 3 ? per : p.n - 3 * per, sbytes = k == 0 ? p.ssz[0] : k == 1 ? p.ssz[1] : k == 2 ? p.ssz[2] : p.ssz[3];
    for (u32 i = lane; i < (sbytes + 11) / 4; i += 64) ob[i] = 0;
    __syncthreads();
    const u64 lo_b = zenc_block_lo(n, nblk, b);
    const u8 *s = src + lo_b + (u64)k * per;
    u8 *out = dst + frame_hdr + offs[b];
    const u32 o = 3 + p.lhdr + p.tree_bytes + 6 + (k > 0 ? p.ssz[0] : 0u) + (k > 1 ? p.ssz[1] : 0u) + (k > 2 ? p.ssz[2] : 0u);
    if (p.pad == 1) {
        zenc_flat4_stream(out + o, s, cnt, codes, lane);
        if (threadIdx.x == 0) zenc_write_block_prefix(out, p, trees + (u64)b * ZENC_TREE_SLOT, b + 1 == nblk && !not_last, 0);
        if (threadIdx.x == 255) out[p.csize - 1] = 0;
        continue;
    }
    const u32 chunk = (cnt + 63) / 64, lo = lane * chunk < cnt ? lane * chunk : cnt, hi = lo + chunk < cnt ? lo + chunk : cnt;
    u32 bits = 0;
    {
        u32 i = lo;
        for (; i + 8 <= hi; i += 8) { const u64 v = ld64(s + i);
#pragma unroll
            for (u32 q = 0; q < 8; q++) bits += codes[(u32)(v >> (8 * q)) & 0xFFu] >> 12; }
        for (; i < hi; i++) bits += codes[s[i]] >> 12;
    }
    const u32 incl = wave_scan_inclusive<u32, OpAdd>(bits);
    const u32 total = (u32)__builtin_amdgcn_readlane((int)incl, 63);
    u32 pos = total - incl;
    u64 acc = 0; u32 nb = pos & 31, w = pos >> 5;
    {
        u32 i = hi;
        for (; i >= lo + 8; i -= 8) { const u64 v = ld64(s + i - 8);
#pragma unroll
            for (int q = 7; q >= 0; q--) {
                const u32 e = codes[(u32)(v >> (8 * q)) & 0xFFu];
                acc |= (u64)(e & 0xFFFu) << nb; nb += e >> 12;
                if (nb >= 32) { atomicOr(&ob[w], (u32)acc); w++; acc >>= 32; nb -= 32; }
            } }
        for (; i-- > lo;) {
            const u32 e = codes[s[i]];
            acc |= (u64)(e & 0xFFFu) << nb; nb += e >> 12;
            if (nb >= 32) { atomicOr(&ob[w], (u32)acc); w++; acc >>= 32; nb -= 32; }
        }
    }
    if (nb) atomicOr(&ob[w], (u32)acc);
    if (lane == 0) atomicOr(&ob[total >> 5], 1u << (total & 31));
    __syncthreads();
    const u8 *img = (const u8 *)ob;
    for (u32 i = lane * 8; i + 8 <= sbytes; i += 64 * 8) st64(out + o + i, ld64(img + i));
    for (u32 i = (sbytes & ~7u) + lane; i < sbytes; i += 64) out[o + i] = img[i];
    if (threadIdx.x == 0) zenc_write_block_prefix(out, p, trees + (u64)b * ZENC_TREE_SLOT, b + 1 == nblk && !not_last, 0);
    if (threadIdx.x == 255) out[p.csize - 1] = 0;
    }
}

__global__ __launch_bounds__(256) void k_zenc_write_direct(const u8 *src, u32 nblk, const ZEncPlan *plan, const u8 *trees, const u64 *offs, u8 *dst, u64 frame_hdr, u32 not_last)
{
    const u32 b = blockIdx.x, q = threadIdx.x >> 6, lane = threadIdx.x & 63;
    const ZEncPlan p = plan[b];
    if (p.kind != ZK_HUF || p.pad != 2) return;
    const u32 o = 3 + p.lhdr + p.tree_bytes + 6 + (q > 0 ? p.ssz[0] : 0u) + (q > 1 ? p.ssz[1] : 0u) + (q > 2 ? p.ssz[2] : 0u);
    const uint4 *in = (const uint4 *)(src + ((u64)b << 15) + 4096u * q);
    u8 *out = dst + frame_hdr + offs[b], *so = out + o;
    if (threadIdx.x == 255) { zenc_write_block_prefix(out, p, trees + (u64)b * ZENC_TREE_SLOT, b + 1 == nblk && !not_last, 0); out[p.csize - 1] = 0; }
    uint4 v[4];
#pragma unroll
    for (u32 r = 0; r < 4; r++) v[r] = in[r * 64 + lane];
#pragma unroll
    for (u32 r = 0; r < 4; r++) __builtin_memcpy(so + 16u * (r * 64 + lane), &v[r], 16);
    if (lane == 0) so[4096] = 1;
}

__device__ __forceinline__ u32 nibble_rev32(u32 x) { const u32 r = __builtin_bswap32(x); return ((r & 0x0F0F0F0Fu) << 4) | ((r >> 4) & 0x0F0F0F0Fu); }
__global__ __launch_bounds__(256) void k_zenc_write_direct_loc(ZencLoc D, u32 nblk, const ZEncPlan *plan, const u8 *trees, const u64 *offs, u8 *dst, u64 frame_hdr, u32 not_last)
{
    __shared__ i32 s_bnd[4][ZENC_LOC_BND];
    const u32 b = blockIdx.x, q = threadIdx.x >> 6, lane = threadIdx.x & 63;
    const u64 t0 = D.blk_t0[b];
    const i32 mine = lane < ZENC_LOC_BND ? D.blk_bnd[(u64)b * ZENC_LOC_BND + lane] : 0;
    const ZEncPlan p = plan[b];
    if (p.kind != ZK_HUF || p.pad != 2) return;
    if (lane < ZENC_LOC_BND) s_bnd[q][lane] = mine;
    __builtin_amdgcn_fence(__ATOMIC_RELEASE, "wavefront"); __builtin_amdgcn_wave_barrier(); __builtin_amdgcn_fence(__ATOMIC_ACQUIRE, "wavefront");
    const i32 *bnd = s_bnd[q];
    const i32 b0rel = bnd[0];
    uint4 A[4]; u32 E[4], sh[4], avail[4]; u64 N0[4], N1[4];
#pragma unroll
    for (u32 r = 0; r < 4; r++) {
        const u32 cidx = r * 64 + lane, Q = 255u - cidx;
        const i32 r0 = (i32)(16384u * q + 64u * Q);
        u32 k = (u32)(r0 - b0rel) >> 12;
        if (bnd[k + 1] <= r0) k++;
        if (bnd[k + 1] <= r0) k++;
        const u32 i = (u32)(r0 - bnd[k]);
        const u32 *pw = (const u32 *)(D.loc + (t0 + k) * 1024) + (i >> 4);
        __builtin_memcpy(&A[r], pw, 16); E[r] = pw[4];
        sh[r] = 2u * (i & 15u);
        const u32 av = (u32)(bnd[k + 1] - r0);
        avail[r] = av < 64u ? av : 64u;
        N0[r] = N1[r] = 0;
        if (av < 64u) { const u8 *nx = D.loc + (t0 + k + 1) * 1024; N0[r] = ld64(nx); N1[r] = ld64(nx + 8); }
    }
    const u32 o = 3 + p.lhdr + p.tree_bytes + 6 + (q > 0 ? p.ssz[0] : 0u) + (q > 1 ? p.ssz[1] : 0u) + (q > 2 ? p.ssz[2] : 0u);
    u8 *out = dst + frame_hdr + offs[b], *so = out + o;
    if (threadIdx.x == 255) { zenc_write_block_prefix(out, p, trees + (u64)b * ZENC_TREE_SLOT, b + 1 == nblk && !not_last, 0); out[p.csize - 1] = 0; }
    uint4 v[4];
#pragma unroll
    for (u32 r = 0; r < 4; r++) {
        const u32 w0 = __builtin_amdgcn_alignbit(A[r].y, A[r].x, sh[r]), w1 = __builtin_amdgcn_alignbit(A[r].z, A[r].y, sh[r]),
                  w2 = __builtin_amdgcn_alignbit(A[r].w, A[r].z, sh[r]), w3 = __builtin_amdgcn_alignbit(E[r], A[r].w, sh[r]);
        u64 a = (u64)w0 | ((u64)w1 << 32), c = (u64)w2 | ((u64)w3 << 32);
        if (avail[r] < 64u) {
            const u64 n0 = N0[r], n1 = N1[r];
            const u32 s = 2u * avail[r];
            if (s < 64) { const u64 m = (1ull << s) - 1; a = (a & m) | (n0 << s); c = (n1 << s) | (n0 >> (64 - s)); }
            else if (s == 64) { c = n0; }
            else { const u64 m = (1ull << (s - 64)) - 1; c = (c & m) | (n0 << (s - 64)); }
        }
        v[r] = make_uint4(nibble_rev32((u32)(c >> 32)), nibble_rev32((u32)c), nibble_rev32((u32)(a >> 32)), nibble_rev32((u32)a));
    }
#pragma unroll
    for (u32 r = 0; r < 4; r++) __builtin_memcpy(so + 16u * (r * 64 + lane), &v[r], 16);
    if (lane == 0) so[4096] = 1;
}

__global__ void k_zenc_frame_header(u8 *dst, int with_magic, u32 wlog)
{
    if (threadIdx.x || blockIdx.x) return;
    u32 p = 0;
    if (with_magic) { dst[p++] = 0x28; dst[p++] = 0xB5; dst[p++] = 0x2F; dst[p++] = 0xFD; }
    dst[p++] = 0x00;
    dst[p++] = (u8)((wlog - 10) << 3);
}

#define PROBE_REGION_LOG 20
#define PROBE_TLOG 16
__global__ __launch_bounds__(256) void k_ldm_probe(const u8 *src, u64 n, u32 *tab, u32 *counts , int pass, u32 every)
{
    const u64 region = (u64)(blockIdx.x >> 9) * every, rbase = region << PROBE_REGION_LOG;
    const u64 p0 = rbase + ((u64)(blockIdx.x & 511) * 256 + threadIdx.x) * 8;
    u32 anchors = 0, hits = 0;
    if (p0 + 24 <= n) {
        const u64 w0 = ld64(src + p0), w1 = ld64(src + p0 + 8), w2 = ld64(src + p0 + 16);
        u32 *t = tab + ((u64)(blockIdx.x >> 9) << PROBE_TLOG);
#pragma unroll
        for (u32 k = 0; k < 8; k++) {
            const u64 a = k ? (w0 >> (8 * k)) | (w1 << (64 - 8 * k)) : w0, b = k ? (w1 >> (8 * k)) | (w2 << (64 - 8 * k)) : w1;
            u32 idx;
            if (!ldm_key(a, b, PROBE_TLOG, idx) || (ldm_mix(a) >> 58) != 0) continue;
            const u32 rel = (u32)(p0 + k - rbase);
            if (pass == 0) atomicMin(&t[idx], rel);
            else {
                anchors++;
                const u32 q = t[idx];
                if (q < rel && rel - q < (1u << 19) && ld64(src + rbase + q) == a && ld64(src + rbase + q + 8) == b) hits++;
            }
        }
    }
    if (pass) {
        __shared__ u32 s_c[4];
        const u32 tot = wg_reduce1<u32, OpAdd>(anchors | (hits << 16), s_c);
        if (threadIdx.x == 0) counts[blockIdx.x] = tot;
    }
}
int zenc_repeat_probe(naf_gpu_ctx *c, const u8 *d_src, size_t n, u32 *share_1024)
{
    *share_1024 = 0;
    if (n < 65536) return 0;
    if (n < (4u << PROBE_REGION_LOG)) { *share_1024 = 1024; return 0; }
    const u32 every = zenc_probe_every(n);
    const u64 regions = ((n >> PROBE_REGION_LOG) + every - 1) / every;
    const u32 nwg = (u32)(regions * 512);
    u32 *tab = arena_new<u32>(c, regions << PROBE_TLOG), *cnt = arena_new<u32>(c, nwg);
    if (!tab || !cnt) return NAF_GPU_ENOMEM;
    HIP_TRY(c, hipMemsetAsync(tab, 0xFF, (regions << PROBE_TLOG) * 4, c->stream));
    LAUNCH(c, "zenc_probe_insert", k_ldm_probe, nwg, 256, 0, d_src, (u64)n, tab, cnt, 0, every);
    LAUNCH(c, "zenc_probe_count", k_ldm_probe, nwg, 256, 0, d_src, (u64)n, tab, cnt, 1, every);
    std::vector<u32> hc(nwg);
    int rc = ctx_readback(c, hc.data(), cnt, (size_t)nwg * 4); if (rc) return rc;
    u64 h[2] = { 0, 0 };
    for (u32 v : hc) { h[0] += v & 0xFFFF; h[1] += v >> 16; }
    if (h[0]) *share_1024 = (u32)(h[1] * 1024 / h[0]);
    return 0;
}

int zenc_level_window(int level)
{
    static const unsigned char w[23] = { 0, 0, 20, 21, 21, 21, 21, 21, 21, 21, 22, 22, 22, 22, 22, 22, 22, 23, 23, 23, 25, 26, 27 };
    if (level < 2) return 0;
    return w[level > 22 ? 22 : level];
}

extern "C" size_t naf_gpu_zstd_compress_bound(size_t n)
{
    return n + 3 * (n / 1024 + 2) + 64;
}

struct ZencOpts {
    bool part, part_first, part_last;
    int with_magic;
    int window_log;
    u32 min_gain, maxbits, prefer_flat, long_last, try_fse;
    u32 block_log;
    bool use_lz;
    bool frame_tree_allowed, frame_quick, lz_lines, tree_defer, frame_write;
};
struct ZencFrame {
    naf_gpu_ctx *c; const u8 *src; size_t n; ZencJob *J;
    ZencOpts O;
    const u8 *direct; u32 nd; const ZencLoc *dloc;
    u32 block_log, window_log, frame_wlog, nblk, lz_buf; u64 bs, hdr; bool use_lz, lzx, lz_on;
    ZEncPlan *plan; u16 *codes; u8 *trees; u64 *offs; ZTreeCache *cache; u32 sample_stride;
    u8 *done;
    bool frame_tree; u32 *fhist; ZEncPlan *fplan; u16 *fcodes; u8 *ftree;
    LzBufs B; u8 *lz_fallback, *wt_defer;
};
#define ZENC_EMPTY_PART 1

static void zenc_options(const naf_gpu_ctx *c, int level, int with_magic, int lz, int block_log_hint, int window_log, ZencOpts &O)
{
    O.part = (with_magic & ZENC_PART) != 0; O.part_first = (with_magic & ZENC_PART_FIRST) != 0; O.part_last = (with_magic & ZENC_PART_LAST) != 0;
    O.min_gain = (with_magic & ZENC_PREFER_RAW) ? 32u : 0u;
    O.maxbits = (with_magic & ZENC_PREFER_RAW) ? 9u : (with_magic & ZENC_SHORT_CODES) ? 7u : (u32)ZENC_HUF_MAXBITS;
    O.prefer_flat = (with_magic & ZENC_PREFER_FLAT) ? 16u : 0u;
    const char *pf = ctx_opt(c, "PREFER_FLAT");
    if (O.prefer_flat && pf && pf[0]) O.prefer_flat = (u32)atoi(pf);
    O.long_last = ((with_magic & ZENC_LONG_LAST) && (!O.part || O.part_last)) ? 1u : 0u;
    O.with_magic = O.part ? 0 : with_magic & ~(ZENC_PREFER_RAW | ZENC_PREFER_FLAT | ZENC_SHORT_CODES | ZENC_FRAME_TREE | ZENC_LONG_LAST);
    O.window_log = window_log;
    O.block_log = 15;
    if (block_log_hint >= 10 && block_log_hint <= 17) O.block_log = (u32)block_log_hint;
    const char *e = ctx_opt(c, "BLOCK_LOG");
    if (e) { int v = atoi(e); if (v >= 10 && v <= 17) O.block_log = (u32)v; }
    const char *el = ctx_opt(c, "LZ");
    O.use_lz = lz || level >= 2;
    if (el && !strcmp(el, "0")) O.use_lz = false;
    if (el && !strcmp(el, "all")) O.use_lz = true;
    if (O.use_lz && !e) O.block_log = (lz && block_log_hint >= 10 && block_log_hint <= 15) ? (u32)block_log_hint : 13u;
    if (O.use_lz && O.block_log > 15) O.block_log = 15;
    O.try_fse = level >= 2;
    const char *eft = ctx_opt(c, "FRAME_TREE");
    O.frame_tree_allowed = level <= 1 && (with_magic & ZENC_FRAME_TREE) != 0 && !(eft && eft[0] == '0');
    const char *fq = ctx_opt(c, "FRAME_QUICK");
    O.frame_quick = !(fq && fq[0] == '0');
    const char *ll = ctx_opt(c, "LZ_LINES");
    O.lz_lines = !(ll && ll[0] == '0');
    const char *td = ctx_opt(c, "TREE_DEFER");
    O.tree_defer = !(td && td[0] == '0');
    const char *fs = ctx_opt(c, "FRAME_WRITE");
    O.frame_write = !(fs && fs[0] == '0');
}

static int zenc_geometry(ZencFrame &F)
{
    naf_gpu_ctx *c = F.c; const ZencOpts &O = F.O; const size_t n = F.n;
    if (O.part && n == 0 && !O.part_last) {
        F.J->empty = 1; F.J->hdr = O.part_first ? 2 : 0; F.J->frame_wlog = (u32)(O.window_log >= 10 ? O.window_log : 19);
        return ZENC_EMPTY_PART;
    }
    F.use_lz = O.use_lz; F.lz_on = F.use_lz && n >= 64;
    F.lzx = F.lz_on && O.window_log >= 10;
    F.window_log = (u32)(O.window_log > 31 ? 31 : O.window_log);
    F.block_log = O.block_log;
    if (F.lzx) F.block_log = F.window_log < 16 ? F.window_log : 16u;
    F.frame_wlog = (F.use_lz && O.window_log >= 10) ? F.window_log : 19u;
    F.bs = 1ull << F.block_log;
    const u64 nblk64 = n ? (n + F.bs - 1) / F.bs : 1;
    if (nblk64 > 0x7FFFFFFFull) return ctx_fail(c, NAF_GPU_EARG, "stream too large");
    F.nblk = (u32)nblk64;
    F.hdr = O.with_magic ? 6 : (O.part && !O.part_first) ? 0 : 2;
    F.lz_buf = (u32)((F.bs + 1 + 320 + 15) & ~15ull);
    if (F.direct && (F.use_lz || F.block_log != 15 || F.nblk != F.nd || n != (size_t)F.nd << 15 || O.prefer_flat < 2 || !zenc_flat16().tb))
        return ctx_fail(c, NAF_GPU_EARG, "direct blocks: the stream must be %u blocks of 32 KiB coded without the match finder", F.nd);
    return 0;
}

struct PlanCall {
    const char *name; u32 grid;
    const u8 *src; u64 n; u32 nblk; ZEncPlan *plan; u16 *codes; u8 *trees; u64 *csize;
    const u32 *blk_len; u64 slot;
    ZTreeCache *cache; u32 sample_stride;
    u32 min_gain, prefer_flat;
    const u8 *done; u8 *wt_defer;
    u32 *fhist; const ZEncPlan *fplan; const u16 *fcodes; const u32 *fratio;
    u32 long_last;
};
static PlanCall plan_call(const char *name, u32 grid) { PlanCall p; memset(&p, 0, sizeof p); p.name = name; p.grid = grid; return p; }
static PlanCall plan_call_blocks(const ZencFrame &F, const char *name, u32 grid)
{
    PlanCall p = plan_call(name, grid);
    p.src = F.src; p.n = (u64)F.n; p.nblk = F.nblk; p.plan = F.plan; p.codes = F.codes; p.trees = F.trees; p.csize = F.offs;
    p.min_gain = F.O.min_gain; p.prefer_flat = F.O.prefer_flat; p.done = F.done;
    return p;
}
static void launch_plan(const ZencFrame &F, const PlanCall &p)
{
    LAUNCH(F.c, p.name, k_zenc_plan, p.grid, 256, 0, p.src, p.n, p.nblk, p.plan, p.codes, p.trees, p.csize, p.blk_len, p.slot, p.cache, p.sample_stride, F.O.try_fse, p.min_gain, F.O.maxbits, p.prefer_flat,
           p.done, p.wt_defer, p.fhist, p.fplan, p.fcodes, p.fratio, p.long_last);
}
static void launch_tree(naf_gpu_ctx *c, u32 nblk, ZEncPlan *plan, u8 *trees, u64 *csize, const u8 *wt_defer, u32 min_gain)
{
    LAUNCH(c, "zenc_tree", k_zenc_tree, cdiv(nblk, 64), 64, 64 * sizeof(ZTreeLane), nblk, plan, trees, csize, wt_defer, min_gain);
}
static int zenc_done_map(ZencFrame &F, bool zeroed)
{
    if (F.done) return 0;
    F.done = (u8 *)arena_alloc(F.c, F.nblk); if (!F.done) return NAF_GPU_ENOMEM;
    if (zeroed) HIP_TRY(F.c, hipMemsetAsync(F.done, 0, F.nblk, F.c->stream));
    return 0;
}

static int plan_buffers(ZencFrame &F)
{
    naf_gpu_ctx *c = F.c; const u32 nblk = F.nblk;
    F.plan = arena_new<ZEncPlan>(c, nblk);
    F.codes = arena_new<u16>(c, (size_t)nblk * 256); F.trees = (u8 *)arena_alloc(c, (size_t)nblk * ZENC_TREE_SLOT);
    F.offs = arena_new<u64>(c, (size_t)nblk + 2);
    F.sample_stride = nblk >= 16 * ZENC_CACHE_ENTRIES ? nblk / ZENC_CACHE_ENTRIES : 0;
    F.cache = F.sample_stride ? arena_new<ZTreeCache>(c, 1) : nullptr;
    if (!F.plan || !F.codes || !F.trees || !F.offs || (F.sample_stride && !F.cache)) return NAF_GPU_ENOMEM;
    if (F.cache) HIP_TRY(c, hipMemsetAsync(F.cache, 0, sizeof(ZTreeCache), c->stream));
    return 0;
}

static int flat_blocks(ZencFrame &F)
{
    naf_gpu_ctx *c = F.c; const u32 nblk = F.nblk; const u8 *direct = F.direct;
    if (!(F.O.prefer_flat >= 2 && F.n >= 2048 && zenc_flat16().tb)) return 0;
    int rc = zenc_done_map(F, false); if (rc) return rc;
    bool dplans = false;
    if (direct) {
        ZEncPlan pd; memset(&pd, 0, sizeof pd);
        const u32 bn = 32768, perq = bn / 4;
        pd.n = bn; pd.kind = ZK_RAW; pd.csize = 3 + bn;
        for (u32 k = 0; k < 4; k++) pd.ssz[k] = (perq * 4 + 8) >> 3;
        zenc_plan_finish(pd, bn, 4, zenc_flat16().tb, F.O.min_gain);
        if (pd.kind == ZK_HUF) {
            pd.pad = 2; dplans = true;
            LAUNCH(c, "zenc_direct_plans", k_zenc_direct_plans, cdiv(nblk, 256), 256, 0, direct, nblk, pd, zenc_flat16(), F.plan, F.trees, F.offs, F.done);
        }
    }
    LAUNCH(c, "zenc_flat_scan", k_zenc_flat_scan, (dplans && cdiv(nblk, ZENC_FLATSCAN_WAVES) > 16384u) ? 16384u : cdiv(nblk, ZENC_FLATSCAN_WAVES), 64 * ZENC_FLATSCAN_WAVES, 0, F.src, (u64)F.n, nblk, F.plan, F.codes, F.trees, F.offs, F.done, F.O.min_gain, F.O.prefer_flat, zenc_flat16(), dplans ? direct : (const u8 *)nullptr, direct);
    return 0;
}

static int frame_quick(ZencFrame &F)
{
    naf_gpu_ctx *c = F.c; const u32 nblk = F.nblk;
    float *fstat = arena_new<float>(c, 8); if (!fstat) return NAF_GPU_ENOMEM;
    int rc = zenc_done_map(F, true); if (rc) return rc;
    LAUNCH(c, "zenc_frame_stats", k_zenc_frame_stats, 1, 256, 0, (const u32 *)F.fhist, (const u16 *)F.fcodes, fstat);
    u32 *tally = arena_new<u32>(c, 2); if (!tally) return NAF_GPU_ENOMEM;
    HIP_TRY(c, hipMemsetAsync(tally, 0, 8, c->stream));
    const u32 qs = nblk / 512 ? nblk / 512 : 1u;
    LAUNCH(c, "zenc_frame_quick", k_zenc_frame_quick, cdiv(nblk, qs), 256, 0, F.src, (u64)F.n, nblk, F.plan, F.codes, F.offs, F.done, (const ZEncPlan *)F.fplan, (const u16 *)F.fcodes, (const float *)fstat, F.O.min_gain, qs, tally, (const u32 *)nullptr);
    LAUNCH(c, "zenc_frame_quick", k_zenc_frame_quick, nblk, 256, 0, F.src, (u64)F.n, nblk, F.plan, F.codes, F.offs, F.done, (const ZEncPlan *)F.fplan, (const u16 *)F.fcodes, (const float *)fstat, F.O.min_gain, 0u, (u32 *)nullptr, (const u32 *)tally);
    return 0;
}
static int frame_tree_build(ZencFrame &F)
{
    naf_gpu_ctx *c = F.c;
    F.frame_tree = F.O.frame_tree_allowed && F.cache && !F.use_lz && !F.direct;
    if (F.frame_tree) {
        F.fhist = arena_new<u32>(c, 256 + 2); F.fplan = arena_new<ZEncPlan>(c, 1); F.fcodes = arena_new<u16>(c, 256); F.ftree = (u8 *)arena_alloc(c, ZENC_TREE_SLOT);
        if (!F.fhist || !F.fplan || !F.fcodes || !F.ftree) return NAF_GPU_ENOMEM;
        HIP_TRY(c, hipMemsetAsync(F.fhist, 0, 258 * 4, c->stream));
        HIP_TRY(c, hipMemsetAsync(F.fplan, 0, sizeof(ZEncPlan), c->stream));
        HIP_TRY(c, hipMemsetAsync(F.fcodes, 0, 512, c->stream));
    }
    if (F.cache) {
        PlanCall p = plan_call_blocks(F, "zenc_plan_sample", ZENC_CACHE_ENTRIES);
        p.cache = F.cache; p.sample_stride = F.sample_stride; p.fhist = F.fhist;
        launch_plan(F, p);
    }
    if (!F.frame_tree) return 0;
    u8 *fblock = (u8 *)arena_alloc(c, ZENC_FRAME_BLOCK + 64); if (!fblock) return NAF_GPU_ENOMEM;
    LAUNCH(c, "zenc_frame_block", k_zenc_frame_block, 1, 256, 0, (const u32 *)F.fhist, fblock, F.fhist + 256);
    u8 *fwt = (u8 *)arena_alloc(c, 256); if (!fwt) return NAF_GPU_ENOMEM;
    PlanCall p = plan_call("zenc_plan_frame", 1);
    p.src = fblock; p.nblk = 1; p.plan = F.fplan; p.codes = F.fcodes; p.trees = F.ftree; p.blk_len = F.fhist + 256; p.wt_defer = fwt;
    launch_plan(F, p);
    launch_tree(c, 1, F.fplan, F.ftree, nullptr, fwt, 0);
    LAUNCH(c, "zenc_frame_ratio", k_zenc_frame_ratio, 1, 256, 0, F.fhist, (const u16 *)F.fcodes);
    return F.O.frame_quick ? frame_quick(F) : 0;
}

static int lz_buffers(ZencFrame &F)
{
    naf_gpu_ctx *c = F.c; const u32 nblk = F.nblk; const u64 bs = F.bs; LzBufs &B = F.B;
    if (!F.lz_on) return 0;
    B.slot = bs; B.seq_slot = bs / 4 + 2; B.of = nullptr; B.ofv = nullptr;
    B.lits = (u8 *)arena_alloc(c, (size_t)nblk * B.slot + 64); B.seqbuf = (u8 *)arena_alloc(c, (size_t)nblk * B.slot + 64);
    B.ll = arena_new<u16>(c, (size_t)nblk * B.seq_slot + 8); B.ml = arena_new<u16>(c, (size_t)nblk * B.seq_slot + 8);
    if (F.lzx) B.ofv = arena_new<u32>(c, (size_t)nblk * B.seq_slot + 8); else B.of = arena_new<u16>(c, (size_t)nblk * B.seq_slot + 8);
    B.nseq = arena_new<u32>(c, nblk); B.nlit = arena_new<u32>(c, nblk); B.seq_bytes = arena_new<u32>(c, nblk);
    if (!B.lits || !B.seqbuf || !B.ll || !B.ml || (!B.of && !B.ofv) || !B.nseq || !B.nlit || !B.seq_bytes) return NAF_GPU_ENOMEM;
    if (F.lzx || !F.O.lz_lines || bs > 32768 || nblk < 64) return 0;
    F.lz_fallback = (u8 *)arena_alloc(c, nblk); if (!F.lz_fallback) return NAF_GPU_ENOMEM;
    int rc = zenc_done_map(F, true); if (rc) return rc;
    const u32 line_div = bs > 16384 ? 16u : 8u, ml_slots = 2 * (u32)(bs / line_div) + 4;
    const u32 lines_lds = F.lz_buf + 4 * ml_slots + 2 * (u32)(bs / line_div + 2);
    LAUNCH(c, "zenc_lz_lines", k_lz_parse_lines, nblk, 64, lines_lds, F.src, (u64)F.n, nblk, B, F.lz_buf, F.lz_fallback, F.plan, F.offs, F.done, line_div, ml_slots);
    return 0;
}

static int plan_blocks(ZencFrame &F)
{
    F.wt_defer = (F.nblk >= 256 && F.O.tree_defer) ? (u8 *)arena_alloc(F.c, (size_t)F.nblk * 256) : nullptr;
    PlanCall p = plan_call_blocks(F, "zenc_plan", F.nblk);
    p.cache = F.cache; p.wt_defer = F.wt_defer; p.fplan = F.fplan; p.fcodes = F.fcodes; p.fratio = F.fhist ? F.fhist + 257 : nullptr; p.long_last = F.O.long_last;
    launch_plan(F, p);
    if (F.wt_defer) launch_tree(F.c, F.nblk, F.plan, F.trees, F.offs, F.wt_defer, F.O.min_gain);
    return 0;
}

static int frame_tree_fix(ZencFrame &F)
{
    naf_gpu_ctx *c = F.c; const u32 nblk = F.nblk;
    if (!F.frame_tree) return 0;
    i32 *fv = arena_new<i32>(c, (size_t)nblk + 1); if (!fv) return NAF_GPU_ENOMEM;
    LAUNCH(c, "zenc_frame_class", k_zenc_frame_class, cdiv(nblk, 256), 256, 0, (const ZEncPlan *)F.plan, nblk, fv);
    int rcs = scan_inclusive_max_i32(c, fv, nblk); if (rcs) return rcs;
    LAUNCH(c, "zenc_frame_fix", k_zenc_frame_fix, cdiv(nblk, 256), 256, 0, F.plan, nblk, (const i32 *)fv, (const ZEncPlan *)F.fplan, (const u8 *)F.ftree, F.trees, F.offs);
    return 0;
}

static int match_finder(ZencFrame &F)
{
    naf_gpu_ctx *c = F.c; const u32 nblk = F.nblk; const size_t n = F.n; const LzBufs &B = F.B; ZWriteLz &L = F.J->L;
    if (!F.lz_on) return 0;
    if (!c->d_seqctab) {
        SeqCTabs T; zenc_build_predefined(T);
        HIP_TRY(c, hipMalloc(&c->d_seqctab, sizeof T));
        HIP_TRY(c, hipMemcpy(c->d_seqctab, &T, sizeof T, hipMemcpyHostToDevice));
    }
    ZEncPlan *plan1 = arena_new<ZEncPlan>(c, nblk);
    u16 *codes1 = arena_new<u16>(c, (size_t)nblk * 256); u8 *trees1 = (u8 *)arena_alloc(c, (size_t)nblk * ZENC_TREE_SLOT);
    u8 *mode = (u8 *)arena_alloc(c, nblk);
    if (!plan1 || !codes1 || !trees1 || !mode) return NAF_GPU_ENOMEM;
    if (F.lzx) {
        LdmTab T; T.wlog = F.window_log; T.elog = T.wlog - 1; T.pad = 0;
        const u64 E = 1ull << T.elog, span = n < E ? n : E;
        u32 tl = 4; while ((1ull << tl) < span / 4 + 16) tl++;
        T.tlog = tl;
        const u64 n_ep = (n >> T.elog) + 1, entries = n_ep << T.tlog;
        T.tab = arena_new<u32>(c, entries); if (!T.tab) return NAF_GPU_ENOMEM;
        HIP_TRY(c, hipMemsetAsync(T.tab, 0xFF, entries * 4, c->stream));
        LAUNCH(c, "zenc_ldm_insert", k_ldm_insert, cdiv(cdiv(n, 8), 256), 256, 0, F.src, (u64)n, T);
        HIP_TRY(c, hipFuncSetAttribute((const void *)k_lzx_parse, hipFuncAttributeMaxDynamicSharedMemorySize, (int)(F.lz_buf + (2u << LZ_HASH_LOG))));
        LAUNCH(c, "zenc_lz_parse", k_lzx_parse, nblk, 64, F.lz_buf + (2u << LZ_HASH_LOG), F.src, (u64)n, nblk, B, F.lz_buf, T);
        LAUNCH(c, "zenc_lz_seqenc", k_lzx_seqenc, nblk, 64, 0, nblk, B, (const SeqCTabs *)c->d_seqctab);
    } else {
        const u32 hash_log = LZ_HASH_LOG;
        LAUNCH(c, "zenc_lz_parse", k_lz_parse, nblk, 64, F.lz_buf + (2u << hash_log), F.src, (u64)n, nblk, B, F.lz_buf, hash_log, (const u8 *)F.lz_fallback);
        LAUNCH(c, "zenc_lz_seqenc", k_lz_seqenc, cdiv(nblk, 64), 64, 0, nblk, B, (const SeqCTabs *)c->d_seqctab);
    }
    PlanCall p = plan_call("zenc_plan", nblk);
    p.src = B.lits; p.n = (u64)n; p.nblk = nblk; p.plan = plan1; p.codes = codes1; p.trees = trees1; p.blk_len = B.nlit; p.slot = B.slot; p.min_gain = F.O.min_gain; p.wt_defer = F.wt_defer;
    launch_plan(F, p);
    if (F.wt_defer) launch_tree(c, nblk, plan1, trees1, nullptr, F.wt_defer, F.O.min_gain);
    LAUNCH(c, "zenc_lz_choose", k_lz_choose, cdiv(nblk, 256), 256, 0, nblk, (const ZEncPlan *)F.plan, (const ZEncPlan *)plan1, (const u32 *)B.nseq, (const u32 *)B.seq_bytes, mode, F.offs);
    L.mode = mode; L.plan1 = plan1; L.codes1 = codes1; L.trees1 = trees1; L.B = B;
    return 0;
}

static int block_offsets(ZencFrame &F)
{
    ZencJob *J = F.J;
    int rc = scan_exclusive_u64(F.c, F.offs, F.nblk, F.offs + F.nblk + 1); if (rc) return rc;
    J->L.not_last = F.O.part && !F.O.part_last;
    J->L.frame_split = (F.frame_tree && F.O.frame_write) ? 1u : 0u;
    J->direct = F.direct != nullptr;
    if (F.direct && F.dloc) J->dloc = *F.dloc;
    J->block_bytes = (u32)F.bs; J->nblk = F.nblk; J->plan = F.plan; J->codes = F.codes; J->trees = F.trees; J->offs = F.offs; J->hdr = F.hdr; J->with_magic = F.O.with_magic; J->frame_wlog = F.frame_wlog;
    return 0;
}

int zstd_encode_begin(naf_gpu_ctx *c, const u8 *d_src, size_t n, int level, int with_magic, int lz, int block_log_hint, int window_log, ZencJob **job, const u8 *direct, u32 nd, const ZencLoc *dloc)
{
    ZencJob *J = new ZencJob; *job = J;
    memset(J, 0, sizeof *J);
    J->src = d_src; J->n = n;
    ZencFrame F; memset(&F, 0, sizeof F);
    F.c = c; F.src = d_src; F.n = n; F.J = J; F.direct = direct; F.nd = nd; F.dloc = dloc;
    zenc_options(c, level, with_magic, lz, block_log_hint, window_log, F.O);
    int rc = zenc_geometry(F);
    if (rc) return rc == ZENC_EMPTY_PART ? 0 : rc;
    if ((rc = plan_buffers(F))) return rc;
    if ((rc = flat_blocks(F))) return rc;
    if ((rc = frame_tree_build(F))) return rc;
    if ((rc = lz_buffers(F))) return rc;
    if ((rc = plan_blocks(F))) return rc;
    if ((rc = frame_tree_fix(F))) return rc;
    if ((rc = match_finder(F))) return rc;
    return block_offsets(F);
}

static int zenc_finish(naf_gpu_ctx *c, ZencJob *J, u8 *d_dst, size_t cap, size_t *out_len, const ZencPlace *place);
void zstd_encode_drop(ZencJob *J) { delete J; }
int zstd_encode_finish(naf_gpu_ctx *c, ZencJob *J, u8 *d_dst, size_t cap, size_t *out_len, const ZencPlace *place)
{
    if (!J) return NAF_GPU_EARG;
    int rc = zenc_finish(c, J, d_dst, cap, out_len, place);
    delete J;
    return rc;
}
static int finish_empty(naf_gpu_ctx *c, ZencJob *J, u8 *d_dst, size_t cap, size_t *out_len, const ZencPlace *place)
{
    const u64 hdr = J->hdr;
    if (place && !(d_dst = place->fn(place->ud, hdr))) return NAF_GPU_ECAP;
    if (!place && cap < hdr) return ctx_fail(c, NAF_GPU_ECAP, "zstd_compress capacity %zu too small", cap);
    if (hdr) LAUNCH(c, "zenc_frame_header", k_zenc_frame_header, 1, 64, 0, d_dst, 0, J->frame_wlog);
    *out_len = hdr;
    return 0;
}
static int zenc_total(naf_gpu_ctx *c, const ZencJob *J, u64 *total)
{
    if (J->have_total) { *total = J->known_total; return 0; }
    return ctx_readback(c, total, J->offs + J->nblk + 1, 8);
}
static int finish_place(naf_gpu_ctx *c, ZencJob *J, u8 **d_dst, size_t cap, const ZencPlace *place, u64 *total)
{
    const u64 bound = J->hdr + J->n + 3ull * J->nblk;
    if (!place) return cap < bound ? ctx_fail(c, NAF_GPU_ECAP, "zstd_compress capacity %zu too small (bound %llu)", cap, (unsigned long long)bound) : 0;
    int rc = zenc_total(c, J, total); if (rc) return rc;
    return (*d_dst = place->fn(place->ud, J->hdr + *total)) ? 0 : NAF_GPU_ECAP;
}
template <typename Kernel, typename Last>
static void launch_writer(naf_gpu_ctx *on, bool timed, const char *name, Kernel kern, u32 grid, u32 block, u32 lds, const ZencJob *J, u8 *d_dst, const Last &last)
{
    if (timed) ktime_begin(on, name);
    hipLaunchKernelGGL(kern, dim3(grid), dim3(block), lds, on->stream, J->src, (u64)J->n, J->nblk, (const ZEncPlan *)J->plan, (const u16 *)J->codes, (const u8 *)J->trees, (const u64 *)J->offs, d_dst, J->hdr, last);
    if (timed) ktime_end(on);
}
static void write_wave(naf_gpu_ctx *on, bool timed, const ZencJob *J, u8 *d_dst)
{
    launch_writer(on, timed, "zenc_write_wave", k_zenc_write_wave, cdiv(J->nblk, ZWW_BLOCKS), 256, 512u + 4u * ZWW_OBUF, J, d_dst, J->L.not_last);
}
static void write_blocks(naf_gpu_ctx *c, ZencJob *J, u8 *d_dst)
{
    J->L.wave_general = (!J->L.mode && J->block_bytes <= 32768u && (J->direct || J->nblk <= 2048u)) ? 1u : 0u;
    if (J->L.frame_split) launch_writer(c, true, "zenc_write", k_zenc_write<true>, cdiv(J->nblk, ZENC_BLOCKS_PER_WG), 64, 0, J, d_dst, J->L);
    launch_writer(c, true, "zenc_write", k_zenc_write<false>, cdiv(J->nblk, ZENC_BLOCKS_PER_WG), 64, 0, J, d_dst, J->L);
}
static int write_direct(naf_gpu_ctx *c, const ZencJob *J, u8 *d_dst)
{
    const u32 nblk = J->nblk;
    if (J->direct && J->dloc.loc) LAUNCH(c, "zenc_write_direct", k_zenc_write_direct_loc, nblk, 256, 0, J->dloc, nblk, (const ZEncPlan *)J->plan, (const u8 *)J->trees, (const u64 *)J->offs, d_dst, J->hdr, J->L.not_last);
    else if (J->direct) LAUNCH(c, "zenc_write_direct", k_zenc_write_direct, nblk, 256, 0, J->src, nblk, (const ZEncPlan *)J->plan, (const u8 *)J->trees, (const u64 *)J->offs, d_dst, J->hdr, J->L.not_last);
    return 0;
}
static naf_gpu_ctx *beside_stream(naf_gpu_ctx *c, const ZencJob *J)
{
    if (!(J->L.wave_general && J->direct && J->own_sync && c->side3 && c->split_ev[ZSPLIT_MAX - 1])) return nullptr;
    return hipStreamWaitEvent(c->side3->stream, c->fork_ev, 0) == hipSuccess ? c->side3 : nullptr;
}
static int write_beside(naf_gpu_ctx *c, naf_gpu_ctx *aux, const ZencJob *J, u8 *d_dst)
{
    write_wave(aux, false, J, d_dst);
    if (hipGetLastError() != hipSuccess || hipEventRecord(c->split_ev[ZSPLIT_MAX - 1], aux->stream) != hipSuccess) return ctx_fail(c, NAF_GPU_EHIP, "zenc_write_wave beside the gather: launch failed");
    const int rc = write_direct(c, J, d_dst);
    if (hipStreamWaitEvent(c->stream, c->split_ev[ZSPLIT_MAX - 1], 0) != hipSuccess && !rc) return ctx_fail(c, NAF_GPU_EHIP, "zenc_write_wave beside the gather: join failed");
    return rc;
}
static int zenc_finish(naf_gpu_ctx *c, ZencJob *J, u8 *d_dst, size_t cap, size_t *out_len, const ZencPlace *place)
{
    if (J->empty) return finish_empty(c, J, d_dst, cap, out_len, place);
    int rc;
    u64 total = 0;
    if ((rc = finish_place(c, J, &d_dst, cap, place, &total))) return rc;
    if (J->hdr) LAUNCH(c, "zenc_frame_header", k_zenc_frame_header, 1, 64, 0, d_dst, J->with_magic, J->frame_wlog);
    write_blocks(c, J, d_dst);
    naf_gpu_ctx *aux = beside_stream(c, J);
    if (aux) rc = write_beside(c, aux, J, d_dst);
    else {
        if (J->L.wave_general) write_wave(c, true, J, d_dst);
        rc = write_direct(c, J, d_dst);
    }
    if (rc) return rc;
    if (!place && (rc = zenc_total(c, J, &total))) return rc;
    *out_len = J->hdr + total;
    return 0;
}
const u64 *zstd_encode_total_ptr(const ZencJob *J) { return (!J || J->empty || J->have_total) ? nullptr : J->offs + J->nblk + 1; }
void zstd_encode_set_total(ZencJob *J, u64 total) { if (J && !J->empty) { J->known_total = total; J->have_total = 1; } }
int zstd_encode_size(naf_gpu_ctx *c, ZencJob *J, size_t *frame_len)
{
    if (!J || !frame_len) return NAF_GPU_EARG;
    if (J->empty) { *frame_len = J->hdr; return 0; }
    if (!J->have_total) {
        u64 t = 0; int rc = ctx_readback(c, &t, J->offs + J->nblk + 1, 8); if (rc) return rc;
        J->known_total = t; J->have_total = 1; J->own_sync = 1;
    }
    *frame_len = J->hdr + J->known_total;
    return 0;
}

int zstd_encode(naf_gpu_ctx *c, const u8 *d_src, size_t n, int level, u8 *d_dst, size_t cap, size_t *out_len, int with_magic, int lz, int block_log_hint, int window_log, const ZencPlace *place)
{
    ZencJob *J = nullptr;
    int rc = zstd_encode_begin(c, d_src, n, level, with_magic, lz, block_log_hint, window_log, &J);
    if (rc) { delete J; return rc; }
    return zstd_encode_finish(c, J, d_dst, cap, out_len, place);
}

extern "C" int naf_gpu_zstd_compress(naf_gpu_ctx *c, const void *d_src, size_t n, int level, void *d_dst, size_t cap, size_t *out_len)
{
    if (!c || !d_dst || !out_len || (!d_src && n)) return NAF_GPU_EARG;
    if (cap < naf_gpu_zstd_compress_bound(n)) return ctx_fail(c, NAF_GPU_ECAP, "zstd_compress capacity %zu is less than the bound %zu", cap, naf_gpu_zstd_compress_bound(n));
    arena_reset(c);
    return zstd_encode(c, (const u8 *)d_src, n, level, (u8 *)d_dst, cap, out_len, 1, 0, 0, zenc_level_window(level));
}
```

Before: 4378 GB/s.

## Plan and scan only non-direct blocks via compacted odd-block list in encoder

The direct-verdict kernel now stages tile sequence and histogram data in LDS per 64-block window and counts non-direct blocks with a ballot. A scan plus a compaction kernel builds a list of these odd blocks. The flat-scan, plan and tree kernels iterate only over that list instead of every block, and direct blocks share one tree buffer instead of per-block copies. A mid-size multi-scan path is also added. This cuts encoder work and memory traffic, at the cost of extra launches and a readback of the odd count.

```diff
diff --git a/naf_amd/csrc/ctx.h b/naf_amd/csrc/ctx.h
--- a/naf_amd/csrc/ctx.h
+++ b/naf_amd/csrc/ctx.h
@@ -119,7 +119,7 @@
 struct ZencPlace { u8 *(*fn)(void *ud, size_t frame_len); void *ud; };
 struct ZencJob;
 #define ZENC_LOC_BND 20
-struct ZencLoc { const u8 *loc; const i32 *blk_bnd; const u32 *blk_t0; u64 tiles; };
+struct ZencLoc { const u8 *loc; const i32 *blk_bnd; const u32 *blk_t0; u64 tiles; const u32 *odd_list; u32 n_odd; };
 int zstd_encode_begin(naf_gpu_ctx *c, const u8 *d_src, size_t n, int level, int with_magic, int lz, int block_log_hint, int window_log, ZencJob **job, const u8 *direct = nullptr, u32 nd = 0, const ZencLoc *dloc = nullptr);
 int zstd_encode_finish(naf_gpu_ctx *c, ZencJob *job, u8 *d_dst, size_t cap, size_t *out_len, const ZencPlace *place);
 void zstd_encode_drop(ZencJob *job);
diff --git a/naf_amd/csrc/enc.hip b/naf_amd/csrc/enc.hip
--- a/naf_amd/csrc/enc.hip
+++ b/naf_amd/csrc/enc.hip
@@ -880,26 +880,55 @@
     }
     if (b < nd && lane == 0) direct[b] = ok ? 1 : 0;
 }
-__global__ __launch_bounds__(256) void k_direct_verdict(const u64 *t_seq, const u32 *t_reg, const u8 *t_hist, u64 tiles, u32 nd, u32 prefer_flat, int probed, const u32 *blk_t0, u8 *direct, i32 *blk_bnd)
-{
-    const u32 b = blockIdx.x * 256 + threadIdx.x;
-    if (b >= nd) return;
-    const u64 B0 = (u64)b << 16, B1 = B0 + 65536, t0 = blk_t0[b];
+#define DV_BLOCKS 64
+#define DV_WINDOW (17 * DV_BLOCKS)
+#define DV_BEYOND 0x7FFFFFFFu
+static_assert((u64)DV_WINDOW * ET_TILE < (1u << 30), "a window's base counts fit 30 bits");
+static_assert(DV_WINDOW * 20 + DV_BLOCKS * 4 <= 65536, "two workgroups a CU");
+static_assert(DV_BLOCKS == 64, "k_direct_verdict counts, and k_odd_list numbers, a workgroup's blocks with a wavefront's ballot");
+__global__ __launch_bounds__(256) void k_direct_verdict(const u64 *t_seq, const u32 *t_reg, const u8 *t_hist, u64 tiles, u32 nd, u32 prefer_flat, int probed, const u32 *blk_t0, u8 *direct, i32 *blk_bnd, u64 *odd_cnt)
+{
+    __shared__ uint4 s_hist[DV_WINDOW];
+    __shared__ u32 s_rel[DV_WINDOW], s_t0[DV_BLOCKS];
+    const u32 bf = blockIdx.x * DV_BLOCKS, nb = nd - bf < DV_BLOCKS ? nd - bf : DV_BLOCKS;
+    const u64 w0 = blk_t0[bf];
+    const u64 wend = (u64)blk_t0[bf + nb - 1] + ZENC_LOC_BND;
+    const u32 wn = wend - w0 < DV_WINDOW ? (u32)(wend - w0) : (u32)DV_WINDOW;
+    const u64 base = t_seq[w0];
+    if (threadIdx.x < nb) s_t0[threadIdx.x] = blk_t0[bf + threadIdx.x];
+    for (u32 j = threadIdx.x; j < wn; j += 256) {
+        const u64 t = w0 + j;
+        u32 e = DV_BEYOND; uint4 h = make_uint4(0, 0, 0, 0);
+        if (t <= tiles) e = (u32)(t_seq[t] - base);
+        if (t < tiles) { e |= t_reg[t] & REG_ACGT; h = *(const uint4 *)(t_hist + t * 16); }
+        s_rel[j] = e; s_hist[j] = h;
+    }
+    __syncthreads();
+    auto seq_at = [&](u64 t) -> u64 {
+        const u64 j = t - w0;
+        if (j < wn) { const u32 e = s_rel[j]; return e == DV_BEYOND ? ~0ull : base + (e & 0x3FFFFFFFu); }
+        return t <= tiles ? t_seq[t] : ~0ull;
+    };
+    for (u32 x = threadIdx.x; x < nb * ZENC_LOC_BND; x += 256) {
+        const u32 bl = x / ZENC_LOC_BND, i = x - bl * ZENC_LOC_BND;
+        const u64 ts = seq_at((u64)s_t0[bl] + i);
+        const i64 rel = (i64)ts - (i64)((u64)(bf + bl) << 16);
+        blk_bnd[(u64)bf * ZENC_LOC_BND + x] = ts != ~0ull && rel < (1 << 30) ? (i32)rel : (i32)(1 << 30);
+    }
+    if (threadIdx.x >= nb) return;
+    const u32 b = bf + threadIdx.x;
+    const u64 B0 = (u64)b << 16, B1 = B0 + 65536, t0 = s_t0[threadIdx.x];
     bool ok = !(probed && (((b >> DIRECT_PROBE_BLOCKS_LOG) & (u32)(probed - 1)) == 0));
-    u64 ts[ZENC_LOC_BND];
-#pragma unroll
-    for (u32 i = 0; i < ZENC_LOC_BND; i++) ts[i] = t0 + i <= tiles ? t_seq[t0 + i] : ~0ull;
-#pragma unroll
-    for (u32 i = 0; i < ZENC_LOC_BND; i++) { const i64 rel = (i64)ts[i] - (i64)B0; blk_bnd[(u64)b * ZENC_LOC_BND + i] = ts[i] != ~0ull && rel < (1 << 30) ? (i32)rel : (i32)(1 << 30); }
     u32 acc[8] = { 0, 0, 0, 0, 0, 0, 0, 0 };
     bool end = false;
-#pragma unroll
     for (u32 i = 0; i < ZENC_LOC_BND - 1; i++) {
         if (!end && ok) {
-            if (t0 + i >= tiles || ts[i] >= B1) end = true;
-            else if (!(t_reg[t0 + i] & REG_ACGT)) ok = false;
+            const u64 t = t0 + i, j = t - w0;
+            const bool in = j < wn;
+            if (t >= tiles || seq_at(t) >= B1) end = true;
+            else if (!((in ? s_rel[j] : t_reg[t]) & REG_ACGT)) ok = false;
             else {
-                const uint4 h = *(const uint4 *)(t_hist + (t0 + i) * 16);
+                const uint4 h = in ? s_hist[j] : *(const uint4 *)(t_hist + t * 16);
                 acc[0] += h.x & 0x00FF00FFu; acc[1] += (h.x >> 8) & 0x00FF00FFu; acc[2] += h.y & 0x00FF00FFu; acc[3] += (h.y >> 8) & 0x00FF00FFu;
                 acc[4] += h.z & 0x00FF00FFu; acc[5] += (h.z >> 8) & 0x00FF00FFu; acc[6] += h.w & 0x00FF00FFu; acc[7] += (h.w >> 8) & 0x00FF00FFu;
             }
@@ -920,6 +949,15 @@
         ok = ns >= 1024 && h * (float)prefer_flat > 4.0f * (float)ns * (float)(prefer_flat - 1);
     }
     direct[b] = ok ? 1 : 0;
+    const u64 odd = __ballot(!ok);
+    if (threadIdx.x == 0) odd_cnt[blockIdx.x] = (u64)__popcll(odd);
+}
+__global__ __launch_bounds__(256) void k_odd_list(const u8 *direct, u32 nd, const u64 *pre, u32 *list)
+{
+    const u32 g = blockIdx.x * 4 + (threadIdx.x >> 6), lane = threadIdx.x & 63, b = g * DV_BLOCKS + lane;
+    const bool odd = b < nd && !direct[b];
+    const u64 bal = __ballot(odd);
+    if (odd) list[pre[g] + (u64)__popcll(bal & ((1ull << lane) - 1))] = b;
 }
 __global__ __launch_bounds__(256) void k_case_gather(const u8 *direct, u32 nd, const u32 *blk_t0, const i32 *blk_bnd, const u8 *locc, const u8 *t_lower, u64 *casebits)
 {
@@ -2796,6 +2834,7 @@
         O.unexpected = d_unexp; O.longest = d_unexp + 3 * 257; O.strict_first = o->strict ? d_unexp + 3 * 257 + 1 : nullptr; O.lead = d_unexp + 3 * 257 + 2;
         O.t_seq = t_seq; O.t_ids = t_ids; O.t_cmt = t_cmt; O.t_rec = t_rec; O.t_tail = t_tail; O.tile_eol = t_eol; O.t_reg = t_reg; O.irr_list = S.fourbit ? irr_list : nullptr;
         O.direct = nullptr; O.nd = 0; O.loc_mode = 0; O.sparse_list = nullptr; O.n_sparse = nullptr;
+        u64 *odd_cnt = nullptr;
         if (S.fourbit) {
             const u64 n_seqb = (T + 1) / 2;
             const char *ed = e_ed, *epr = e_epr;
@@ -2807,7 +2846,15 @@
                 const bool use_loc = fused && !(e_op && e_op[0] == '3' && !S.no_case);
                 i32 *blk_bnd = use_loc ? arena_new<i32>(c, (size_t)S.nd * ZENC_LOC_BND + 1) : nullptr;
                 if (use_loc && !blk_bnd) return NAF_GPU_ENOMEM;
-                if (use_loc) LAUNCH(c, "ennaf_direct_blocks", k_direct_verdict, cdiv(S.nd, 256), 256, 0, (const u64 *)t_seq, (const u32 *)t_reg, (const u8 *)t_hist, tiles, S.nd, prefer_flat, (epr && epr[0] == '0') ? 0 : (int)zenc_probe_every(n_seqb), (const u32 *)blk_t0, S.direct, blk_bnd);
+                if (use_loc) {
+                    const u32 nwg = cdiv(S.nd, DV_BLOCKS);
+                    odd_cnt = arena_new<u64>(c, (size_t)nwg + 2); u32 *odd_list = arena_new<u32>(c, (size_t)S.nd + 1);
+                    if (!odd_cnt || !odd_list) return NAF_GPU_ENOMEM;
+                    LAUNCH(c, "ennaf_direct_blocks", k_direct_verdict, nwg, 256, 0, (const u64 *)t_seq, (const u32 *)t_reg, (const u8 *)t_hist, tiles, S.nd, prefer_flat, (epr && epr[0] == '0') ? 0 : (int)zenc_probe_every(n_seqb), (const u32 *)blk_t0, S.direct, blk_bnd, odd_cnt);
+                    if ((rc = scan_exclusive_u64(c, odd_cnt, nwg, odd_cnt + nwg + 1))) return rc;
+                    LAUNCH(c, "ennaf_odd_list", k_odd_list, cdiv(nwg, 4), 256, 0, (const u8 *)S.direct, S.nd, (const u64 *)odd_cnt, odd_list);
+                    S.dloc.odd_list = odd_list; odd_cnt += nwg + 1;
+                }
                 else LAUNCH(c, "ennaf_direct_blocks", k_direct_blocks, cdiv(S.nd, 4), 256, 0, d_text, (const u64 *)t_seq, (const u32 *)t_reg, tiles, S.nd, prefer_flat, (epr && epr[0] == '0') ? 0 : (int)zenc_probe_every(n_seqb), S.direct, (const u32 *)blk_t0, blk_bnd);
                 O.direct = S.direct; O.nd = S.nd;
                 if (use_loc) {
@@ -2829,6 +2876,11 @@
             if ((rc = ennaf_scatter4(c, S.sc4, S.packed, S.casebits))) return rc;
         } else LAUNCH(c, "ennaf_scatter", k_enc_scatter<false>, tiles, 256, 0, P, (const i64 *)t_eol, (const i64 *)t_sp, O);
         std::vector<u64> hu(NU);
+        if (S.dloc.odd_list) {
+            u64 n_odd = 0;
+            if ((rc = ctx_readback2(c, hu.data(), d_unexp, NU * 8, &n_odd, odd_cnt, 8))) return rc;
+            S.dloc.n_odd = (u32)n_odd;
+        } else
         if ((rc = ctx_readback(c, hu.data(), d_unexp, NU * 8))) return rc;
         const u64 sk = hu[3 * 257 + 1];
         if (o->strict && sk != ~0ull) {
diff --git a/naf_amd/csrc/scan.hip b/naf_amd/csrc/scan.hip
--- a/naf_amd/csrc/scan.hip
+++ b/naf_amd/csrc/scan.hip
@@ -122,6 +122,29 @@
     for (size_t k = lo; k < hi; k++) { const T v = vals[k]; vals[k] = run; run = Op::template f<T>(run, v); }
     if (S.tot[blockIdx.x] && threadIdx.x == 0) *S.tot[blockIdx.x] = tot;
 }
+#define SCAN_MID (16 * SCAN_SMALL)
+template <typename T, typename Op>
+__global__ __launch_bounds__(SCAN_THREADS) void k_scan_mid_multi(ScanSet<T> S, size_t n)
+{
+    __shared__ T lds[2][4];
+    T *vals = S.sums[blockIdx.x];
+    T run = Op::template id<T>();
+    for (size_t c0 = 0; c0 < n; c0 += SCAN_TILE) {
+        const size_t base = c0 + threadIdx.x;
+        T v[SCAN_ITEMS];
+#pragma unroll
+        for (int i = 0; i < SCAN_ITEMS; i++) { size_t k = base + (size_t)i * SCAN_THREADS; v[i] = k < n ? vals[k] : Op::template id<T>(); }
+#pragma unroll
+        for (int i = 0; i < SCAN_ITEMS; i++) {
+            T pre, tot;
+            T wi = wg_scan1<T, Op>(v[i], &pre, &tot, lds[i & 1]);
+            size_t k = base + (size_t)i * SCAN_THREADS;
+            if (k < n) vals[k] = Op::template f<T>(run, Op::template f<T>(pre, wave_shift_up1<T, Op>(wi)));
+            run = Op::template f<T>(run, tot);
+        }
+    }
+    if (S.tot[blockIdx.x] && threadIdx.x == 0) *S.tot[blockIdx.x] = run;
+}
 template <typename T, typename Op, bool EXCL>
 __global__ __launch_bounds__(SCAN_THREADS) void k_scan_tile_apply_multi(ScanSet<T> S, size_t n)
 {
@@ -146,7 +169,7 @@
 static int scan_multi(naf_gpu_ctx *c, T *const *arrs, int k, size_t n, T *const *totals)
 {
     const size_t ntiles = (n + SCAN_TILE - 1) / SCAN_TILE;
-    if (k < 2 || k > SCAN_MULTI_MAX || n <= SCAN_SMALL || ntiles > SCAN_SMALL) {
+    if (k < 2 || k > SCAN_MULTI_MAX || n <= SCAN_SMALL || ntiles > SCAN_MID) {
         for (int i = 0; i < k; i++) { int rc = scan_rec<T, Op, EXCL>(c, arrs[i], n, totals ? totals[i] : (T *)nullptr); if (rc) return rc; }
         return 0;
     }
@@ -156,7 +179,8 @@
         S.sums[i] = arena_new<T>(c, ntiles + 1); if (!S.sums[i]) return ctx_fail(c, NAF_GPU_ENOMEM, "scan scratch");
     }
     LAUNCH(c, "scan_reduce", (k_scan_tile_reduce_multi<T, Op>), dim3((unsigned)ntiles, (unsigned)k), SCAN_THREADS, 0, S, n);
-    LAUNCH(c, "scan_small", (k_scan_small_multi<T, Op>), (unsigned)k, SCAN_THREADS, 0, S, ntiles);
+    if (ntiles <= SCAN_SMALL) LAUNCH(c, "scan_small", (k_scan_small_multi<T, Op>), (unsigned)k, SCAN_THREADS, 0, S, ntiles);
+    else LAUNCH(c, "scan_small", (k_scan_mid_multi<T, Op>), (unsigned)k, SCAN_THREADS, 0, S, ntiles);
     LAUNCH(c, "scan_apply", (k_scan_tile_apply_multi<T, Op, EXCL>), dim3((unsigned)ntiles, (unsigned)k), SCAN_THREADS, 0, S, n);
     return 0;
 }
diff --git a/naf_amd/csrc/zstd_enc.hip b/naf_amd/csrc/zstd_enc.hip
--- a/naf_amd/csrc/zstd_enc.hip
+++ b/naf_amd/csrc/zstd_enc.hip
@@ -33,13 +33,15 @@
 __host__ __device__ static inline u64 zenc_block_lo(u64 n, u32 nblk, u32 b) { u64 q = n / nblk, r = n % nblk; return (u64)b * q + (b < r ? b : r); }
 
 #define ZENC_FLATSCAN_WAVES 4
-__global__ __launch_bounds__(64 * ZENC_FLATSCAN_WAVES) void k_zenc_flat_scan(const u8 *src, u64 n, u32 nblk, ZEncPlan *plan, u16 *codes, u8 *trees, u64 *csize, u8 *done, u32 min_gain, u32 prefer_flat, ZFlat16 f16, const u8 *planned, const u8 *direct)
+__global__ __launch_bounds__(64 * ZENC_FLATSCAN_WAVES) void k_zenc_flat_scan(const u8 *src, u64 n, u32 nblk, ZEncPlan *plan, u16 *codes, u8 *trees, u64 *csize, u8 *done, u32 min_gain, u32 prefer_flat, ZFlat16 f16, const u8 *planned, const u8 *direct,
+                                                                               const u32 *list, u32 n_list)
 {
     __shared__ u32 bins[ZENC_FLATSCAN_WAVES][64];
     const u32 wv = threadIdx.x >> 6, lane = threadIdx.x & 63;
-    for (u32 bq = blockIdx.x; bq * ZENC_FLATSCAN_WAVES < nblk; bq += gridDim.x) {
-    const u32 b = bq * ZENC_FLATSCAN_WAVES + wv;
-    if (planned && bq * ZENC_FLATSCAN_WAVES + ZENC_FLATSCAN_WAVES <= nblk && *(const u32 *)(planned + bq * ZENC_FLATSCAN_WAVES) == 0x01010101u) continue;
+    for (u32 bq = blockIdx.x; bq * ZENC_FLATSCAN_WAVES < (list ? n_list : nblk); bq += gridDim.x) {
+    const u32 at = bq * ZENC_FLATSCAN_WAVES + wv;
+    const u32 b = !list ? at : at < n_list ? list[at] : nblk;
+    if (!list && planned && bq * ZENC_FLATSCAN_WAVES + ZENC_FLATSCAN_WAVES <= nblk && *(const u32 *)(planned + bq * ZENC_FLATSCAN_WAVES) == 0x01010101u) continue;
     bins[wv][lane] = 0;
     __syncthreads();
     bool ok = b < nblk;
@@ -99,6 +101,7 @@
                 const u32 hn = sym >> 4, ln = sym & 15u, rank = 4 * ((hn >> 1) - (hn >> 3)) + ((ln >> 1) - (ln >> 3));
                 codes[(u64)b * 256 + sym] = is16 ? (u16)(rank | (4u << 12)) : (u16)0;
             }
+            if (!dir || !planned)
             for (u32 k = lane; k < p.tree_bytes; k += 64) trees[(u64)b * ZENC_TREE_SLOT + k] = f16.tree[k];
         }
     }
@@ -106,19 +109,20 @@
     }
 }
 
-__global__ void k_zenc_direct_plans(const u8 *direct, u32 nblk, ZEncPlan pd, ZFlat16 f16, ZEncPlan *plan, u8 *trees, u64 *csize, u8 *done)
+__global__ void k_zenc_direct_plans(const u8 *direct, u32 nblk, ZEncPlan pd, ZFlat16 f16, ZEncPlan *plan, u8 *dtree, u64 *csize, u8 *done)
 {
     const u32 b = blockIdx.x * blockDim.x + threadIdx.x;
+    if (b == 0) for (u32 k = 0; k < pd.tree_bytes; k++) dtree[k] = f16.tree[k];
     if (b >= nblk || !direct[b]) return;
     plan[b] = pd; if (csize) csize[b] = pd.csize; done[b] = 1;
-    for (u32 k = 0; k < pd.tree_bytes; k++) trees[(u64)b * ZENC_TREE_SLOT + k] = f16.tree[k];
 }
 
 __global__ __launch_bounds__(256) void k_zenc_plan(const u8 *src, u64 n, u32 nblk, ZEncPlan *plan, u16 *codes, u8 *trees, u64 *csize, const u32 *blk_len, u64 slot, ZTreeCache *cache, u32 sample_stride, u32 try_fse, u32 min_gain, u32 maxbits, u32 prefer_flat, const u8 *done, u8 *wt_defer,
-                                                    u32 *fhist = nullptr, const ZEncPlan *fplan = nullptr, const u16 *fcodes = nullptr, const u32 *fratio = nullptr, u32 long_last = 0)
+                                                    u32 *fhist = nullptr, const ZEncPlan *fplan = nullptr, const u16 *fcodes = nullptr, const u32 *fratio = nullptr, u32 long_last = 0,
+                                                    const u32 *list = nullptr)
 {
     __shared__ u32 hist[ZENC_HCOPIES * 1024];
-    u32 b = sample_stride ? blockIdx.x * sample_stride : blockIdx.x;
+    u32 b = list ? list[blockIdx.x] : sample_stride ? blockIdx.x * sample_stride : blockIdx.x;
     if (done && done[b]) return;
     u64 lo = zenc_block_lo(n, nblk, b), hi = zenc_block_lo(n, nblk, b + 1);
     if (blk_len) { lo = (u64)b * slot; hi = lo + blk_len[b]; }
@@ -524,11 +528,12 @@
 
 struct ZTreeLane { FseWS fse; u8 tmp[160]; u8 w[256]; u32 odd; };
 static_assert((sizeof(ZTreeLane) / 4) % 2 == 1, "odd word stride: the lanes' workspaces start in different LDS banks");
-__global__ __launch_bounds__(64) void k_zenc_tree(u32 nblk, ZEncPlan *plan, u8 *trees, u64 *csize, const u8 *wt_defer, u32 min_gain)
+__global__ __launch_bounds__(64) void k_zenc_tree(u32 nblk, ZEncPlan *plan, u8 *trees, u64 *csize, const u8 *wt_defer, u32 min_gain, const u32 *list, u32 n_list)
 {
     __builtin_amdgcn_s_setprio(3);
     extern __shared__ __attribute__((aligned(16))) u8 tree_lds[];
-    const u32 b = blockIdx.x * 64 + threadIdx.x;
+    const u32 at = blockIdx.x * 64 + threadIdx.x;
+    const u32 b = !list ? at : at < n_list ? list[at] : nblk;
     const bool pending = b < nblk && (plan[b].pad & 0x80u);
     if (!__ballot(pending)) return;
     if (!pending) return;
@@ -1045,7 +1050,7 @@
 }
 
 struct ZWriteLz { const u8 *mode; const ZEncPlan *plan1; const u16 *codes1; const u8 *trees1; LzBufs B; u32 not_last; u32 wave_general; u32 frame_split; };
-struct ZencJob { const u8 *src; size_t n; u32 nblk, frame_wlog; ZEncPlan *plan; u16 *codes; u8 *trees; u64 *offs; u64 hdr; int with_magic, empty; ZWriteLz L; bool direct; u32 block_bytes; ZencLoc dloc; u64 known_total; int have_total, own_sync; };
+struct ZencJob { const u8 *src; size_t n; u32 nblk, frame_wlog; ZEncPlan *plan; u16 *codes; u8 *trees; u64 *offs; u64 hdr; int with_magic, empty; ZWriteLz L; bool direct; u8 *dtree; u32 block_bytes; ZencLoc dloc; u64 known_total; int have_total, own_sync; };
 template <bool FRAME>
 __global__ __launch_bounds__(64) void k_zenc_write(const u8 *src, u64 n, u32 nblk, const ZEncPlan *plan, const u16 *codes_g, const u8 *trees,
                                                     const u64 *offs, u8 *dst, u64 frame_hdr, ZWriteLz L)
@@ -1216,7 +1221,7 @@
     }
 }
 
-__global__ __launch_bounds__(256) void k_zenc_write_direct(const u8 *src, u32 nblk, const ZEncPlan *plan, const u8 *trees, const u64 *offs, u8 *dst, u64 frame_hdr, u32 not_last)
+__global__ __launch_bounds__(256) void k_zenc_write_direct(const u8 *src, u32 nblk, const ZEncPlan *plan, const u8 *trees, const u64 *offs, u8 *dst, u64 frame_hdr, u32 not_last, const u8 *dtree)
 {
     const u32 b = blockIdx.x, q = threadIdx.x >> 6, lane = threadIdx.x & 63;
     const ZEncPlan p = plan[b];
@@ -1224,7 +1229,7 @@
     const u32 o = 3 + p.lhdr + p.tree_bytes + 6 + (q > 0 ? p.ssz[0] : 0u) + (q > 1 ? p.ssz[1] : 0u) + (q > 2 ? p.ssz[2] : 0u);
     const uint4 *in = (const uint4 *)(src + ((u64)b << 15) + 4096u * q);
     u8 *out = dst + frame_hdr + offs[b], *so = out + o;
-    if (threadIdx.x == 255) { zenc_write_block_prefix(out, p, trees + (u64)b * ZENC_TREE_SLOT, b + 1 == nblk && !not_last, 0); out[p.csize - 1] = 0; }
+    if (threadIdx.x == 255) { zenc_write_block_prefix(out, p, dtree ? dtree : trees + (u64)b * ZENC_TREE_SLOT, b + 1 == nblk && !not_last, 0); out[p.csize - 1] = 0; }
     uint4 v[4];
 #pragma unroll
     for (u32 r = 0; r < 4; r++) v[r] = in[r * 64 + lane];
@@ -1234,7 +1239,7 @@
 }
 
 __device__ __forceinline__ u32 nibble_rev32(u32 x) { const u32 r = __builtin_bswap32(x); return ((r & 0x0F0F0F0Fu) << 4) | ((r >> 4) & 0x0F0F0F0Fu); }
-__global__ __launch_bounds__(256) void k_zenc_write_direct_loc(ZencLoc D, u32 nblk, const ZEncPlan *plan, const u8 *trees, const u64 *offs, u8 *dst, u64 frame_hdr, u32 not_last)
+__global__ __launch_bounds__(256) void k_zenc_write_direct_loc(ZencLoc D, u32 nblk, const ZEncPlan *plan, const u8 *trees, const u64 *offs, u8 *dst, u64 frame_hdr, u32 not_last, const u8 *dtree)
 {
     __shared__ i32 s_bnd[4][ZENC_LOC_BND];
     const u32 b = blockIdx.x, q = threadIdx.x >> 6, lane = threadIdx.x & 63;
@@ -1265,7 +1270,7 @@
     }
     const u32 o = 3 + p.lhdr + p.tree_bytes + 6 + (q > 0 ? p.ssz[0] : 0u) + (q > 1 ? p.ssz[1] : 0u) + (q > 2 ? p.ssz[2] : 0u);
     u8 *out = dst + frame_hdr + offs[b], *so = out + o;
-    if (threadIdx.x == 255) { zenc_write_block_prefix(out, p, trees + (u64)b * ZENC_TREE_SLOT, b + 1 == nblk && !not_last, 0); out[p.csize - 1] = 0; }
+    if (threadIdx.x == 255) { zenc_write_block_prefix(out, p, dtree ? dtree : trees + (u64)b * ZENC_TREE_SLOT, b + 1 == nblk && !not_last, 0); out[p.csize - 1] = 0; }
     uint4 v[4];
 #pragma unroll
     for (u32 r = 0; r < 4; r++) {
@@ -1446,6 +1451,7 @@
     const u8 *done; u8 *wt_defer;
     u32 *fhist; const ZEncPlan *fplan; const u16 *fcodes; const u32 *fratio;
     u32 long_last;
+    const u32 *list;
 };
 static PlanCall plan_call(const char *name, u32 grid) { PlanCall p; memset(&p, 0, sizeof p); p.name = name; p.grid = grid; return p; }
 static PlanCall plan_call_blocks(const ZencFrame &F, const char *name, u32 grid)
@@ -1458,11 +1464,11 @@
 static void launch_plan(const ZencFrame &F, const PlanCall &p)
 {
     LAUNCH(F.c, p.name, k_zenc_plan, p.grid, 256, 0, p.src, p.n, p.nblk, p.plan, p.codes, p.trees, p.csize, p.blk_len, p.slot, p.cache, p.sample_stride, F.O.try_fse, p.min_gain, F.O.maxbits, p.prefer_flat,
-           p.done, p.wt_defer, p.fhist, p.fplan, p.fcodes, p.fratio, p.long_last);
-}
-static void launch_tree(naf_gpu_ctx *c, u32 nblk, ZEncPlan *plan, u8 *trees, u64 *csize, const u8 *wt_defer, u32 min_gain)
-{
-    LAUNCH(c, "zenc_tree", k_zenc_tree, cdiv(nblk, 64), 64, 64 * sizeof(ZTreeLane), nblk, plan, trees, csize, wt_defer, min_gain);
+           p.done, p.wt_defer, p.fhist, p.fplan, p.fcodes, p.fratio, p.long_last, p.list);
+}
+static void launch_tree(naf_gpu_ctx *c, u32 nblk, ZEncPlan *plan, u8 *trees, u64 *csize, const u8 *wt_defer, u32 min_gain, const u32 *list = nullptr, u32 n_list = 0)
+{
+    LAUNCH(c, "zenc_tree", k_zenc_tree, cdiv(list ? n_list : nblk, 64), 64, 64 * sizeof(ZTreeLane), nblk, plan, trees, csize, wt_defer, min_gain, list, n_list);
 }
 static int zenc_done_map(ZencFrame &F, bool zeroed)
 {
@@ -1485,6 +1491,11 @@
     return 0;
 }
 
+static bool zenc_by_list(const ZencFrame &F)
+{
+    const ZencLoc *D = F.dloc;
+    return F.direct && F.J->dtree && D && D->odd_list && D->n_odd <= F.nblk / 2 && !(ctx_opt(F.c, "ODD_LIST") && ctx_opt(F.c, "ODD_LIST")[0] == '0');
+}
 static int flat_blocks(ZencFrame &F)
 {
     naf_gpu_ctx *c = F.c; const u32 nblk = F.nblk; const u8 *direct = F.direct;
@@ -1498,11 +1509,16 @@
         for (u32 k = 0; k < 4; k++) pd.ssz[k] = (perq * 4 + 8) >> 3;
         zenc_plan_finish(pd, bn, 4, zenc_flat16().tb, F.O.min_gain);
         if (pd.kind == ZK_HUF) {
+            F.J->dtree = (u8 *)arena_alloc(c, ZENC_TREE_SLOT); if (!F.J->dtree) return NAF_GPU_ENOMEM;
             pd.pad = 2; dplans = true;
-            LAUNCH(c, "zenc_direct_plans", k_zenc_direct_plans, cdiv(nblk, 256), 256, 0, direct, nblk, pd, zenc_flat16(), F.plan, F.trees, F.offs, F.done);
-        }
-    }
-    LAUNCH(c, "zenc_flat_scan", k_zenc_flat_scan, (dplans && cdiv(nblk, ZENC_FLATSCAN_WAVES) > 16384u) ? 16384u : cdiv(nblk, ZENC_FLATSCAN_WAVES), 64 * ZENC_FLATSCAN_WAVES, 0, F.src, (u64)F.n, nblk, F.plan, F.codes, F.trees, F.offs, F.done, F.O.min_gain, F.O.prefer_flat, zenc_flat16(), dplans ? direct : (const u8 *)nullptr, direct);
+            LAUNCH(c, "zenc_direct_plans", k_zenc_direct_plans, cdiv(nblk, 256), 256, 0, direct, nblk, pd, zenc_flat16(), F.plan, F.J->dtree, F.offs, F.done);
+        }
+    }
+    const bool by_list = zenc_by_list(F);
+    const u32 nwork = by_list ? F.dloc->n_odd : nblk;
+    if (!nwork) return 0;
+    LAUNCH(c, "zenc_flat_scan", k_zenc_flat_scan, (dplans && cdiv(nwork, ZENC_FLATSCAN_WAVES) > 16384u) ? 16384u : cdiv(nwork, ZENC_FLATSCAN_WAVES), 64 * ZENC_FLATSCAN_WAVES, 0, F.src, (u64)F.n, nblk, F.plan, F.codes, F.trees, F.offs, F.done, F.O.min_gain, F.O.prefer_flat, zenc_flat16(), dplans ? direct : (const u8 *)nullptr, direct,
+           by_list ? F.dloc->odd_list : (const u32 *)nullptr, nwork);
     return 0;
 }
 
@@ -1569,10 +1585,14 @@
 static int plan_blocks(ZencFrame &F)
 {
     F.wt_defer = (F.nblk >= 256 && F.O.tree_defer) ? (u8 *)arena_alloc(F.c, (size_t)F.nblk * 256) : nullptr;
-    PlanCall p = plan_call_blocks(F, "zenc_plan", F.nblk);
+    const ZencLoc *D = F.dloc;
+    const bool by_list = zenc_by_list(F);
+    if (by_list && !D->n_odd) return 0;
+    PlanCall p = plan_call_blocks(F, "zenc_plan", by_list ? D->n_odd : F.nblk);
     p.cache = F.cache; p.wt_defer = F.wt_defer; p.fplan = F.fplan; p.fcodes = F.fcodes; p.fratio = F.fhist ? F.fhist + 257 : nullptr; p.long_last = F.O.long_last;
+    if (by_list) p.list = D->odd_list;
     launch_plan(F, p);
-    if (F.wt_defer) launch_tree(F.c, F.nblk, F.plan, F.trees, F.offs, F.wt_defer, F.O.min_gain);
+    if (F.wt_defer) launch_tree(F.c, F.nblk, F.plan, F.trees, F.offs, F.wt_defer, F.O.min_gain, p.list, by_list ? D->n_odd : 0u);
     return 0;
 }
 
@@ -1708,8 +1728,8 @@
 static int write_direct(naf_gpu_ctx *c, const ZencJob *J, u8 *d_dst)
 {
     const u32 nblk = J->nblk;
-    if (J->direct && J->dloc.loc) LAUNCH(c, "zenc_write_direct", k_zenc_write_direct_loc, nblk, 256, 0, J->dloc, nblk, (const ZEncPlan *)J->plan, (const u8 *)J->trees, (const u64 *)J->offs, d_dst, J->hdr, J->L.not_last);
-    else if (J->direct) LAUNCH(c, "zenc_write_direct", k_zenc_write_direct, nblk, 256, 0, J->src, nblk, (const ZEncPlan *)J->plan, (const u8 *)J->trees, (const u64 *)J->offs, d_dst, J->hdr, J->L.not_last);
+    if (J->direct && J->dloc.loc) LAUNCH(c, "zenc_write_direct", k_zenc_write_direct_loc, nblk, 256, 0, J->dloc, nblk, (const ZEncPlan *)J->plan, (const u8 *)J->trees, (const u64 *)J->offs, d_dst, J->hdr, J->L.not_last, (const u8 *)J->dtree);
+    else if (J->direct) LAUNCH(c, "zenc_write_direct", k_zenc_write_direct, nblk, 256, 0, J->src, nblk, (const ZEncPlan *)J->plan, (const u8 *)J->trees, (const u64 *)J->offs, d_dst, J->hdr, J->L.not_last, (const u8 *)J->dtree);
     return 0;
 }
 static naf_gpu_ctx *beside_stream(naf_gpu_ctx *c, const ZencJob *J)
```

After: 4340 GB/s. About the same (-0.9%).
